# virajmehta/vae-training

Hardware: AMD Instinct MI355X
Metric: ELBO train-step samples/sec (higher is better)
Workload: dtype f32; 1 GPU; M: linear-padding dd3 pad9 (D=12) L=20 linear enc/dec -tdv eps=-1 lr=1e-3 (seed_linpadding_expts.sh:1); batch_per_gpu=65536, global_batch=65536, data_dim=12, latent_dim=20, params=533, parallelism=dp1, grad_exchange=none, launch=direct library call x2395 steps (arguments marshalled once), input_batches=48

## Files before the change

### include/vaek.h

```cpp
#ifndef VAEK_H
#define VAEK_H

#include <stddef.h>
#include <stdint.h>

#ifdef __cplusplus
extern "C" {
#endif

#define VAEK_VERSION 100
#define VAEK_MAX_HIDDEN 8

typedef enum vaek_status {
    VAEK_OK = 0,
    VAEK_ERR_INVALID = -1,
    VAEK_ERR_HIP = -2,
    VAEK_ERR_NO_DEVICE = -3,
    VAEK_ERR_WORKSPACE = -4,
    VAEK_ERR_COMM = -5
} vaek_status;

enum { VAEK_ACT_NONE = 0, VAEK_ACT_RELU = 1 };

enum { VAEK_F32 = 0, VAEK_BF16 = 1 };

typedef struct vaek_config {
    int32_t struct_size;
    int32_t batch;
    int32_t data_dim;
    int32_t latent_dim;
    int32_t n_enc_hidden;
    int32_t enc_hidden[VAEK_MAX_HIDDEN];
    int32_t n_dec_hidden;
    int32_t dec_hidden[VAEK_MAX_HIDDEN];
    int32_t sigmoid_decoder;
    int32_t tunable_eps;
    float   eps_cli;
    int32_t dtype;
    int32_t device;
    int32_t world;
    int32_t rank;
    int64_t global_batch;
    int32_t force_generic;
    int32_t reserved[7];
} vaek_config;

typedef struct vaek_ctx vaek_ctx;

int vaek_version(void);
const char* vaek_last_error(void);

int vaek_ctx_create(const vaek_config* cfg, vaek_ctx** out);
int vaek_ctx_destroy(vaek_ctx* ctx);
int vaek_param_count(const vaek_ctx* ctx, int64_t* P);
int vaek_grad_len(const vaek_ctx* ctx, int64_t* n);
int vaek_leaf_count(const vaek_ctx* ctx, int32_t* n_leaves);
int vaek_leaf_info(const vaek_ctx* ctx, int32_t leaf, char* name, int32_t name_cap,
                   int64_t* offset, int32_t* rows, int32_t* cols);
int vaek_workspace_bytes(const vaek_ctx* ctx, size_t* bytes);
int vaek_uses_fused_path(const vaek_ctx* ctx, int32_t* fused);
int vaek_train_step_path(const vaek_ctx* ctx, char* name, int32_t cap);

int vaek_dense_fwd(vaek_ctx* ctx, const float* x, const float* w, const float* b, float* y,
                   int32_t rows, int32_t n_in, int32_t n_out, int32_t act, void* stream);
int vaek_dense_bwd_dx(vaek_ctx* ctx, const float* dy, const float* w, const float* x_post, float* dx,
                      int32_t rows, int32_t n_in, int32_t n_out, int32_t act, int32_t accumulate, void* stream);
int vaek_dense_bwd_dw(vaek_ctx* ctx, const float* x, const float* dy, float* dwb,
                      int32_t rows, int32_t n_in, int32_t n_out, void* workspace, void* stream);
int vaek_elbo_fwd_bwd(vaek_ctx* ctx, const float* x, const float* x_hat_lin, const float* x_hat_sig,
                      const float* z2, const float* mu, const float* logvar_e, float eps,
                      float* d_lin, float* d_sig, float* out4, int32_t rows, int32_t data_dim,
                      int32_t latent_dim, int64_t batch_total, void* workspace, void* stream);
int vaek_elbo_fwd_bwd_dev(vaek_ctx* ctx, const float* x, const float* x_hat_lin, const float* x_hat_sig,
                          const float* z2, const float* mu, const float* logvar_e, const float* eps_param_dev, float eps_scale,
                          float* d_lin, float* d_sig, float* out4, int32_t rows, int32_t data_dim,
                          int32_t latent_dim, int64_t batch_total, void* workspace, void* stream);
int vaek_adam_step(vaek_ctx* ctx, float* params, const float* grads, float* m, float* v, int64_t n,
                   float lr, int32_t step, const int32_t* step_dev, float grad_scale, void* stream);

int vaek_train_step(vaek_ctx* ctx, float* params, float* grads, float* m, float* v, int32_t* step_dev,
                    const float* x, const float* z1, const float* z2, float lr,
                    void* workspace, void* stream);
int vaek_train_step_grads_only(vaek_ctx* ctx, const float* params, float* grads, int32_t* step_dev,
                               const float* x, const float* z1, const float* z2,
                               void* workspace, void* stream);
int vaek_train_step_apply(vaek_ctx* ctx, float* params, const float* grads, float* m, float* v,
                          const int32_t* step_dev, float lr, void* stream);
int vaek_bucket_count(const vaek_ctx* ctx, int32_t* n);
int vaek_bucket_info(const vaek_ctx* ctx, int32_t i, int64_t* offset, int64_t* count);
int vaek_train_step_grads_bucketed(vaek_ctx* ctx, const float* params, float* grads, int32_t* step_dev,
                                   const float* x, const float* z1, const float* z2, void* const* ready_events,
                                   void* workspace, void* stream);
int vaek_loss_eval(vaek_ctx* ctx, const float* params, const float* x, const float* z1, const float* z2,
                   float* out4, void* workspace, void* stream);
int vaek_forward(vaek_ctx* ctx, const float* params, const float* x, const float* z1, const float* z2,
                 int32_t sampling, float eps, float* x_hat, float* mu_out, int32_t rows,
                 void* workspace, void* stream);

int vaek_comm_buffer_bytes(const vaek_ctx* ctx, size_t* bytes);
int vaek_comm_create(vaek_ctx* ctx, uint8_t handle_out[64]);
int vaek_comm_init(vaek_ctx* ctx, const uint8_t* all_handles );
int vaek_comm_destroy(vaek_ctx* ctx);
int vaek_comm_allreduce(vaek_ctx* ctx, float* buf, int64_t n, void* stream);
int vaek_comm_status(vaek_ctx* ctx, int32_t* timed_out);

int vaek_make_batch(vaek_ctx* ctx, int32_t kind, const float* A, int32_t dd, int32_t did, int32_t pad, float var_added,
                    float* x, float* z1, float* z2, int32_t rows, int64_t row0, uint64_t seed,
                    const int32_t* step_dev, uint32_t step_host, uint32_t tag, void* stream);
int vaek_make_batch_next(vaek_ctx* ctx, int32_t kind, const float* A, int32_t dd, int32_t did, int32_t pad, float var_added,
                         float* x, float* z1, float* z2, int32_t rows, int64_t row0, uint64_t seed,
                         int32_t* counter , int32_t which, uint32_t tag, void* stream);
int vaek_train_step_gen(vaek_ctx* ctx, float* params, float* grads, float* m, float* v, int32_t* step_dev, const float* x,
                        const float* z1, const float* z2, float lr, void* workspace, int32_t kind, const float* A, int32_t dd,
                        int32_t did, int32_t pad, float var_added, float* x_next, float* z1_next, float* z2_next, int64_t row0,
                        uint64_t seed, int32_t* counter, int32_t which, uint32_t tag, void* stream);
int vaek_supports_train_steps(const vaek_ctx* ctx, int32_t* yes);
int vaek_train_steps(vaek_ctx* ctx, float* params, float* grads, float* m, float* v, int32_t* step_dev,
                     const float* const* xs, const float* const* z1s, const float* const* z2s, int32_t n_steps, float lr,
                     void* workspace, void* stream);
int vaek_train_steps_status(vaek_ctx* ctx, void* workspace, int32_t* gave_up);
int vaek_supports_train_steps_gen(const vaek_ctx* ctx, int32_t kind, int32_t* yes);
int vaek_train_steps_moment_len(const vaek_ctx* ctx, int64_t* len);
int vaek_train_steps_moments(vaek_ctx* ctx, const float* x, const float* z1, const float* z2, double* M, void* workspace, void* stream);
int vaek_train_steps_update(vaek_ctx* ctx, float* params, float* grads, float* m, float* v, int32_t* step_dev, const double* M, float lr,
                            void* workspace, void* stream);
int vaek_train_steps_gen(vaek_ctx* ctx, float* params, float* grads, float* m, float* v, int32_t* step_dev, int32_t kind, const float* A,
                         int32_t dd, int32_t did, int32_t pad, float var_added, int64_t row0, uint64_t seed, uint32_t tag, int32_t n_steps,
                         float lr, void* workspace, void* stream);
int vaek_supports_train_loop_gen(const vaek_ctx* ctx, int32_t kind, int32_t* yes);
int vaek_train_loop_gen(vaek_ctx* ctx, float* params, float* grads, float* m, float* v, int32_t* step_dev, int32_t kind, const float* A,
                        int32_t dd, int32_t did, int32_t pad, float var_added, int64_t row0, uint64_t seed, uint32_t tag, int32_t n_steps,
                        float lr, void* workspace, void* stream);
int vaek_train_loop_steps_per_launch(void);
typedef struct vaek_replicas {
    int32_t struct_size;
    int32_t n;
    int64_t state_stride;
    int64_t grads_stride;
    const uint64_t* seeds;
    const float* lrs;
    int64_t a_stride;
    float* loss_hist;
    int64_t loss_hist_cap;
} vaek_replicas;
int vaek_train_loop_max_replicas(void);
int vaek_train_loop_replicas_workspace_bytes(const vaek_ctx* ctx, int32_t n, size_t* bytes);
int vaek_train_loop_gen_replicas(vaek_ctx* ctx, float* params, float* grads, float* m, float* v, int32_t* step_dev,
                                 const vaek_replicas* rep, int32_t kind, const float* A, int32_t dd, int32_t did, int32_t pad,
                                 float var_added, int64_t row0, uint32_t tag, int32_t n_steps, float lr, void* workspace, void* stream);
typedef struct vaek_trajectory {
    int32_t struct_size;
    int32_t every;
    float*  buf;
    int64_t cap;
    int64_t record_stride;
    int64_t replica_stride;
} vaek_trajectory;
int vaek_trajectory_record_len(const vaek_ctx* ctx, int64_t* floats);
int vaek_train_loop_gen_traj(vaek_ctx* ctx, float* params, float* grads, float* m, float* v, int32_t* step_dev, int32_t kind, const float* A,
                             int32_t dd, int32_t did, int32_t pad, float var_added, int64_t row0, uint64_t seed, uint32_t tag, int32_t n_steps,
                             float lr, void* workspace, void* stream, const vaek_trajectory* traj);
int vaek_train_loop_gen_replicas_traj(vaek_ctx* ctx, float* params, float* grads, float* m, float* v, int32_t* step_dev,
                                      const vaek_replicas* rep, int32_t kind, const float* A, int32_t dd, int32_t did, int32_t pad,
                                      float var_added, int64_t row0, uint32_t tag, int32_t n_steps, float lr, void* workspace, void* stream,
                                      const vaek_trajectory* traj);
int vaek_supports_train_step_replicas(const vaek_ctx* ctx, int32_t* yes);
int vaek_train_step_max_replicas(void);
int vaek_train_step_replicas_workspace_bytes(const vaek_ctx* ctx, int32_t n, size_t* bytes);
int vaek_train_step_gen_replicas(vaek_ctx* ctx, float* params, float* grads, float* m, float* v, int32_t* step_dev,
                                 const vaek_replicas* rep, const float* x, const float* z1, const float* z2, float lr, void* workspace,
                                 int32_t kind, const float* A, int32_t dd, int32_t did, int32_t pad, float var_added, float* x_next,
                                 float* z1_next, float* z2_next, int64_t row0, int32_t* counter, int32_t which, uint32_t tag,
                                 void* stream);
int vaek_conv2d_forward_workspace(int32_t batch, int32_t height, int32_t width, int32_t c_in, int32_t c_out, int32_t transposed, size_t* bytes);
int vaek_conv2d_forward(const float* x, const float* w, const float* bias, const float* mask, float* y, int32_t batch, int32_t height,
                        int32_t width, int32_t c_in, int32_t c_out, int32_t relu, void* workspace, const void* x_bf16, void* y_bf16,
                        void* stream);
int vaek_to_bf16(const float* src, void* dst_bf16, int64_t n, void* stream);
int vaek_conv2d_transpose_forward(const float* y, const float* w, const float* bias, const float* mask, float* out, int32_t batch,
                                  int32_t height, int32_t width, int32_t c_in, int32_t c_out, int32_t relu, void* workspace,
                                  const void* y_bf16, void* out_bf16, void* stream);
int vaek_conv2d_weight_grad_workspace(int32_t batch, int32_t height, int32_t width, int32_t c_in, int32_t c_out, size_t* bytes);
int vaek_conv2d_weight_grad(const float* x, const float* dy, float* dw, float* dbias, void* workspace, int32_t batch, int32_t height,
                            int32_t width, int32_t c_in, int32_t c_out, const void* x_bf16, const void* dy_bf16, void* stream);
int vaek_conv2d_bias_grad(const float* dy, float* dbias, void* workspace, int64_t pixels, int32_t c, void* stream);
int vaek_conv2d_bias_grad_bf16(const void* dy_bf16, float* dbias, void* workspace, int64_t pixels, int32_t c, void* stream);
int vaek_dense_fwd_reparam(vaek_ctx* ctx, const float* x, const float* w, const float* b, float* mu, float* samples, const float* z1,
                           const float* logvar_e, int32_t rows, int32_t n_in, int32_t n_out, void* stream);
int vaek_reparam_bwd(vaek_ctx* ctx, float* d_samples, const float* mu, const float* z1, const float* logvar_e, float* d_logvar_e,
                     int32_t rows, int32_t latent_dim, int64_t batch_total, void* workspace, void* stream);
int vaek_rng_fill(vaek_ctx* ctx, float* normals, uint32_t* bits, int64_t n, uint64_t seed, uint32_t step, uint32_t tag,
                  void* stream);
int vaek_set_loss_history(vaek_ctx* ctx, float* buf, int64_t cap);

int vaek_microbench_copy(vaek_ctx* ctx, const void* src, void* dst, int64_t bytes, void* stream);
int vaek_microbench_mfma(vaek_ctx* ctx, int32_t kind, int32_t iters, int32_t waves_per_simd, float* scratch,
                         double* flops_out, void* stream);

int vaek_microbench_launch(vaek_ctx* ctx, int32_t kind, int32_t blocks, int32_t n, const int32_t* p, int32_t* out, void* stream);

int vaek_profile_begin(vaek_ctx* ctx, int32_t max_records);
int vaek_profile_report(vaek_ctx* ctx, char* buf, size_t cap);

#ifdef __cplusplus
}
#endif
#endif
```

### vae_training_amd/_lib.py

```python
from __future__ import annotations

import ctypes as C
import os

_HERE = os.path.dirname(os.path.abspath(__file__))
LIB_PATH = os.environ.get("VAEK_LIB_PATH") or os.path.join(_HERE, "csrc", "libvaek.so")
VAEK_MAX_HIDDEN = 8
VAEK_F32, VAEK_BF16 = 0, 1
VAEK_ACT_NONE, VAEK_ACT_RELU = 0, 1


class VaekError(RuntimeError):
    def __init__(self, code, msg):
        super().__init__(f"libvaek error {code}: {msg}")
        self.code = code


class VaekConfig(C.Structure):
    _fields_ = [
        ("struct_size", C.c_int32), ("batch", C.c_int32), ("data_dim", C.c_int32), ("latent_dim", C.c_int32),
        ("n_enc_hidden", C.c_int32), ("enc_hidden", C.c_int32 * VAEK_MAX_HIDDEN),
        ("n_dec_hidden", C.c_int32), ("dec_hidden", C.c_int32 * VAEK_MAX_HIDDEN),
        ("sigmoid_decoder", C.c_int32), ("tunable_eps", C.c_int32), ("eps_cli", C.c_float),
        ("dtype", C.c_int32), ("device", C.c_int32), ("world", C.c_int32), ("rank", C.c_int32),
        ("global_batch", C.c_int64), ("force_generic", C.c_int32), ("reserved", C.c_int32 * 7),
    ]


class VaekReplicas(C.Structure):
    _fields_ = [
        ("struct_size", C.c_int32), ("n", C.c_int32), ("state_stride", C.c_int64), ("grads_stride", C.c_int64),
        ("seeds", C.c_void_p), ("lrs", C.c_void_p), ("a_stride", C.c_int64), ("loss_hist", C.c_void_p), ("loss_hist_cap", C.c_int64),
    ]


class VaekTrajectory(C.Structure):
    _fields_ = [
        ("struct_size", C.c_int32), ("every", C.c_int32), ("buf", C.c_void_p), ("cap", C.c_int64), ("record_stride", C.c_int64),
        ("replica_stride", C.c_int64),
    ]


def trajectory_slot(t, every, cap):
    if t < 1 or t % every:
        return None
    return (t // every - 1) % cap


_vp, _i32, _i64, _f32 = C.c_void_p, C.c_int32, C.c_int64, C.c_float

SIGNATURES = {
    "vaek_version": (C.c_int, []),
    "vaek_last_error": (C.c_char_p, []),
    "vaek_ctx_create": (C.c_int, [C.POINTER(VaekConfig), C.POINTER(_vp)]),
    "vaek_ctx_destroy": (C.c_int, [_vp]),
    "vaek_param_count": (C.c_int, [_vp, C.POINTER(_i64)]),
    "vaek_grad_len": (C.c_int, [_vp, C.POINTER(_i64)]),
    "vaek_leaf_count": (C.c_int, [_vp, C.POINTER(_i32)]),
    "vaek_leaf_info": (C.c_int, [_vp, _i32, C.c_char_p, _i32, C.POINTER(_i64), C.POINTER(_i32), C.POINTER(_i32)]),
    "vaek_workspace_bytes": (C.c_int, [_vp, C.POINTER(C.c_size_t)]),
    "vaek_uses_fused_path": (C.c_int, [_vp, C.POINTER(_i32)]),
    "vaek_train_step_path": (C.c_int, [_vp, C.c_char_p, _i32]),
    "vaek_dense_fwd": (C.c_int, [_vp, _vp, _vp, _vp, _vp, _i32, _i32, _i32, _i32, _vp]),
    "vaek_dense_bwd_dx": (C.c_int, [_vp, _vp, _vp, _vp, _vp, _i32, _i32, _i32, _i32, _i32, _vp]),
    "vaek_dense_bwd_dw": (C.c_int, [_vp, _vp, _vp, _vp, _i32, _i32, _i32, _vp, _vp]),
    "vaek_elbo_fwd_bwd": (C.c_int, [_vp, _vp, _vp, _vp, _vp, _vp, _vp, _f32, _vp, _vp, _vp, _i32, _i32, _i32, _i64, _vp, _vp]),
    "vaek_elbo_fwd_bwd_dev": (C.c_int, [_vp, _vp, _vp, _vp, _vp, _vp, _vp, _vp, _f32, _vp, _vp, _vp, _i32, _i32, _i32, _i64, _vp, _vp]),
    "vaek_adam_step": (C.c_int, [_vp, _vp, _vp, _vp, _vp, _i64, _f32, _i32, _vp, _f32, _vp]),
    "vaek_train_step": (C.c_int, [_vp, _vp, _vp, _vp, _vp, _vp, _vp, _vp, _vp, _f32, _vp, _vp]),
    "vaek_train_step_grads_only": (C.c_int, [_vp, _vp, _vp, _vp, _vp, _vp, _vp, _vp, _vp]),
    "vaek_train_step_apply": (C.c_int, [_vp, _vp, _vp, _vp, _vp, _vp, _f32, _vp]),
    "vaek_bucket_count": (C.c_int, [_vp, C.POINTER(_i32)]),
    "vaek_bucket_info": (C.c_int, [_vp, _i32, C.POINTER(_i64), C.POINTER(_i64)]),
    "vaek_train_step_grads_bucketed": (C.c_int, [_vp, _vp, _vp, _vp, _vp, _vp, _vp, _vp, _vp, _vp]),
    "vaek_loss_eval": (C.c_int, [_vp, _vp, _vp, _vp, _vp, _vp, _vp, _vp]),
    "vaek_forward": (C.c_int, [_vp, _vp, _vp, _vp, _vp, _i32, _f32, _vp, _vp, _i32, _vp, _vp]),
    "vaek_comm_buffer_bytes": (C.c_int, [_vp, C.POINTER(C.c_size_t)]),
    "vaek_comm_create": (C.c_int, [_vp, _vp]),
    "vaek_comm_init": (C.c_int, [_vp, _vp]),
    "vaek_comm_status": (C.c_int, [_vp, C.POINTER(_i32)]),
    "vaek_comm_destroy": (C.c_int, [_vp]),
    "vaek_comm_allreduce": (C.c_int, [_vp, _vp, _i64, _vp]),
    "vaek_make_batch": (C.c_int, [_vp, _i32, _vp, _i32, _i32, _i32, _f32, _vp, _vp, _vp, _i32, _i64, C.c_uint64, _vp,
                                  C.c_uint32, C.c_uint32, _vp]),
    "vaek_make_batch_next": (C.c_int, [_vp, _i32, _vp, _i32, _i32, _i32, _f32, _vp, _vp, _vp, _i32, _i64, C.c_uint64, _vp,
                                       _i32, C.c_uint32, _vp]),
    "vaek_train_step_gen": (C.c_int, [_vp, _vp, _vp, _vp, _vp, _vp, _vp, _vp, _vp, _f32, _vp, _i32, _vp, _i32, _i32, _i32, _f32,
                                      _vp, _vp, _vp, _i64, C.c_uint64, _vp, _i32, C.c_uint32, _vp]),
    "vaek_supports_train_steps": (C.c_int, [_vp, C.POINTER(_i32)]),
    "vaek_train_steps": (C.c_int, [_vp, _vp, _vp, _vp, _vp, _vp, _vp, _vp, _vp, _i32, _f32, _vp, _vp]),
    "vaek_train_steps_status": (C.c_int, [_vp, _vp, C.POINTER(_i32)]),
    "vaek_supports_train_steps_gen": (C.c_int, [_vp, _i32, C.POINTER(_i32)]),
    "vaek_train_steps_moment_len": (C.c_int, [_vp, C.POINTER(_i64)]),
    "vaek_train_steps_moments": (C.c_int, [_vp, _vp, _vp, _vp, _vp, _vp, _vp]),
    "vaek_train_steps_update": (C.c_int, [_vp, _vp, _vp, _vp, _vp, _vp, _vp, _f32, _vp, _vp]),
    "vaek_train_steps_gen": (C.c_int, [_vp, _vp, _vp, _vp, _vp, _vp, _i32, _vp, _i32, _i32, _i32, _f32, C.c_int64, C.c_uint64, C.c_uint32, _i32,
                                       _f32, _vp, _vp]),
    "vaek_supports_train_loop_gen": (C.c_int, [_vp, _i32, C.POINTER(_i32)]),
    "vaek_train_loop_gen": (C.c_int, [_vp, _vp, _vp, _vp, _vp, _vp, _i32, _vp, _i32, _i32, _i32, _f32, C.c_int64, C.c_uint64, C.c_uint32, _i32,
                                      _f32, _vp, _vp]),
    "vaek_train_loop_steps_per_launch": (C.c_int, []),
    "vaek_train_loop_max_replicas": (C.c_int, []),
    "vaek_train_loop_replicas_workspace_bytes": (C.c_int, [_vp, _i32, C.POINTER(C.c_size_t)]),
    "vaek_train_loop_gen_replicas": (C.c_int, [_vp, _vp, _vp, _vp, _vp, _vp, C.POINTER(VaekReplicas), _i32, _vp, _i32, _i32, _i32, _f32,
                                               C.c_int64, C.c_uint32, _i32, _f32, _vp, _vp]),
    "vaek_trajectory_record_len": (C.c_int, [_vp, C.POINTER(_i64)]),
    "vaek_train_loop_gen_traj": (C.c_int, [_vp, _vp, _vp, _vp, _vp, _vp, _i32, _vp, _i32, _i32, _i32, _f32, C.c_int64, C.c_uint64, C.c_uint32, _i32,
                                           _f32, _vp, _vp, C.POINTER(VaekTrajectory)]),
    "vaek_train_loop_gen_replicas_traj": (C.c_int, [_vp, _vp, _vp, _vp, _vp, _vp, C.POINTER(VaekReplicas), _i32, _vp, _i32, _i32, _i32, _f32,
                                                    C.c_int64, C.c_uint32, _i32, _f32, _vp, _vp, C.POINTER(VaekTrajectory)]),
    "vaek_supports_train_step_replicas": (C.c_int, [_vp, C.POINTER(_i32)]),
    "vaek_train_step_max_replicas": (C.c_int, []),
    "vaek_train_step_replicas_workspace_bytes": (C.c_int, [_vp, _i32, C.POINTER(C.c_size_t)]),
    "vaek_train_step_gen_replicas": (C.c_int, [_vp, _vp, _vp, _vp, _vp, _vp, C.POINTER(VaekReplicas), _vp, _vp, _vp, _f32, _vp, _i32, _vp,
                                               _i32, _i32, _i32, _f32, _vp, _vp, _vp, _i64, _vp, _i32, C.c_uint32, _vp]),
    "vaek_conv2d_forward": (C.c_int, [_vp, _vp, _vp, _vp, _vp, _i32, _i32, _i32, _i32, _i32, _i32, _vp, _vp, _vp, _vp]),
    "vaek_to_bf16": (C.c_int, [_vp, _vp, C.c_int64, _vp]),
    "vaek_conv2d_forward_workspace": (C.c_int, [_i32, _i32, _i32, _i32, _i32, _i32, C.POINTER(C.c_size_t)]),
    "vaek_conv2d_bias_grad": (C.c_int, [_vp, _vp, _vp, C.c_int64, _i32, _vp]),
    "vaek_conv2d_bias_grad_bf16": (C.c_int, [_vp, _vp, _vp, C.c_int64, _i32, _vp]),
    "vaek_dense_fwd_reparam": (C.c_int, [_vp, _vp, _vp, _vp, _vp, _vp, _vp, _vp, _i32, _i32, _i32, _vp]),
    "vaek_reparam_bwd": (C.c_int, [_vp, _vp, _vp, _vp, _vp, _vp, _i32, _i32, C.c_int64, _vp, _vp]),
    "vaek_conv2d_transpose_forward": (C.c_int, [_vp, _vp, _vp, _vp, _vp, _i32, _i32, _i32, _i32, _i32, _i32, _vp, _vp, _vp, _vp]),
    "vaek_conv2d_weight_grad_workspace": (C.c_int, [_i32, _i32, _i32, _i32, _i32, C.POINTER(C.c_size_t)]),
    "vaek_conv2d_weight_grad": (C.c_int, [_vp, _vp, _vp, _vp, _vp, _i32, _i32, _i32, _i32, _i32, _vp, _vp, _vp]),
    "vaek_rng_fill": (C.c_int, [_vp, _vp, _vp, _i64, C.c_uint64, C.c_uint32, C.c_uint32, _vp]),
    "vaek_set_loss_history": (C.c_int, [_vp, _vp, _i64]),
    "vaek_microbench_copy": (C.c_int, [_vp, _vp, _vp, _i64, _vp]),
    "vaek_microbench_launch": (C.c_int, [_vp, _i32, _i32, _i32, _vp, _vp, _vp]),
    "vaek_microbench_mfma": (C.c_int, [_vp, _i32, _i32, _i32, _vp, C.POINTER(C.c_double), _vp]),
    "vaek_profile_begin": (C.c_int, [_vp, _i32]),
    "vaek_profile_report": (C.c_int, [_vp, C.c_char_p, C.c_size_t]),
}

_lib = None


def load():
    global _lib
    if _lib is not None:
        return _lib
    if not os.path.exists(LIB_PATH):
        raise RuntimeError(
            f"{LIB_PATH} is missing: build it with `make -C {os.path.dirname(LIB_PATH)}` or "
            "`python -c 'import __graft_entry__ as g; g.build()'`. vae_training_amd has no CPU/PyTorch fallback.")
    import torch
    lib = C.CDLL(LIB_PATH)
    for name, (res, args) in SIGNATURES.items():
        fn = getattr(lib, name)
        fn.restype, fn.argtypes = res, args
    _lib = lib
    return lib


def check(rc):
    if rc != 0:
        raise VaekError(rc, load().vaek_last_error().decode("utf-8", "replace"))
```

### vae_training_amd/csrc/api.hip

```cpp
#include <stdarg.h>
#include <string.h>

#include <algorithm>
#include <new>
#include <utility>

#include "vaek_internal.h"

namespace vaek {

static thread_local char g_err[512] = "";
thread_local Profiler* g_prof = nullptr;
void set_error(const char* fmt, ...) {
    va_list ap;
    va_start(ap, fmt);
    vsnprintf(g_err, sizeof(g_err), fmt, ap);
    va_end(ap);
}

static size_t align_up(size_t v, size_t a) { return (v + a - 1) / a * a; }
constexpr int kElboBlockSplits = 512;

static void add_net(vaek_ctx* c, Net& net, const char* name, int fan_in, const int* hidden, int n_hidden, int last) {
    int k = fan_in;
// ... 836 lines not shown
        return VAEK_ERR_INVALID;
    }
    if (rep->n < 1 || rep->n > resident_max_replicas()) {
        set_error("%s: %d replicas, need 1 .. %d (vaek_train_loop_max_replicas)", who, rep->n, resident_max_replicas());
        return VAEK_ERR_INVALID;
    }
    if (rep->state_stride < ctx->P || rep->grads_stride < ctx->P + kExtra) {
        set_error("%s: state_stride %lld < P = %lld or grads_stride %lld < grad_len = %lld", who, (long long)rep->state_stride,
                  (long long)ctx->P, (long long)rep->grads_stride, (long long)(ctx->P + kExtra));
        return VAEK_ERR_INVALID;
    }
    if (!rep->seeds) { set_error("%s: seeds is NULL", who); return VAEK_ERR_INVALID; }
    if (rep->a_stride < 0) { set_error("%s: a_stride %lld < 0", who, (long long)rep->a_stride); return VAEK_ERR_INVALID; }
    if (rep->loss_hist && rep->loss_hist_cap < 1) {
        set_error("%s: loss_hist given with loss_hist_cap %lld < 1", who, (long long)rep->loss_hist_cap);
        return VAEK_ERR_INVALID;
    }
    const size_t ws_bytes = resident_replicas_workspace_bytes(ctx, rep->n);
    if (ws_bytes && (!workspace || (reinterpret_cast<uintptr_t>(workspace) & 15))) {
        set_error("%s: this context stages its batches in memory: workspace must be a 16-byte aligned device "
                  "pointer of vaek_train_loop_replicas_workspace_bytes() = %zu bytes", who, ws_bytes);
        return VAEK_ERR_INVALID;
    }
    TrajArgs tj{};
    if (traj) { const int trc = check_trajectory(who, ctx, traj, true, &tj); if (trc) return trc; }
    BatchArgs gen;
    float* dummy = params;
    int rc = make_batch_args(ctx, kind, A, dd, did, pad, var_added, dummy, dummy, dummy, ctx->B, row0, 0, step_dev, 0, nullptr, 0, tag, &gen);
    if (rc) return rc;
    gen.x = gen.z1 = gen.z2 = nullptr;
    if (n_steps == 0) return VAEK_OK;
    return resident_train_loop_replicas(ctx, params, grads, m, v, step_dev, gen, rep->n, rep->state_stride, rep->grads_stride,
                                        reinterpret_cast<const unsigned long long*>(rep->seeds), rep->lrs, rep->a_stride, rep->loss_hist,
                                        rep->loss_hist_cap, n_steps, lr, workspace, (hipStream_t)stream, traj ? &tj : nullptr);
}

int vaek_train_loop_gen_replicas(vaek_ctx* ctx, float* params, float* grads, float* m, float* v, int32_t* step_dev,
                                 const vaek_replicas* rep, int32_t kind, const float* A, int32_t dd, int32_t did, int32_t pad,
                                 float var_added, int64_t row0, uint32_t tag, int32_t n_steps, float lr, void* workspace, void* stream) {
    return train_loop_gen_replicas_impl("vaek_train_loop_gen_replicas", ctx, params, grads, m, v, step_dev, rep, kind, A, dd, did, pad, var_added,
                                        row0, tag, n_steps, lr, workspace, stream, nullptr);
}

int vaek_train_loop_gen_replicas_traj(vaek_ctx* ctx, float* params, float* grads, float* m, float* v, int32_t* step_dev,
                                      const vaek_replicas* rep, int32_t kind, const float* A, int32_t dd, int32_t did, int32_t pad,
                                      float var_added, int64_t row0, uint32_t tag, int32_t n_steps, float lr, void* workspace, void* stream,
                                      const vaek_trajectory* traj) {
    return train_loop_gen_replicas_impl(traj ? "vaek_train_loop_gen_replicas_traj" : "vaek_train_loop_gen_replicas", ctx, params, grads, m, v,
                                        step_dev, rep, kind, A, dd, did, pad, var_added, row0, tag, n_steps, lr, workspace, stream, traj);
}

int vaek_train_loop_gen_traj(vaek_ctx* ctx, float* params, float* grads, float* m, float* v, int32_t* step_dev, int32_t kind, const float* A,
                             int32_t dd, int32_t did, int32_t pad, float var_added, int64_t row0, uint64_t seed, uint32_t tag, int32_t n_steps,
                             float lr, void* workspace, void* stream, const vaek_trajectory* traj) {
    if (!traj) return vaek_train_loop_gen(ctx, params, grads, m, v, step_dev, kind, A, dd, did, pad, var_added, row0, seed, tag, n_steps, lr,
                                          workspace, stream);
    ProfBind pb(ctx);
    if (!ctx || !params || !grads || !m || !v || !step_dev || n_steps < 0) { set_error("vaek_train_loop_gen_traj: invalid argument"); return VAEK_ERR_INVALID; }
    if (!ctx->resident) {
        set_error("vaek_train_loop_gen_traj: needs a context vaek_train_loop_gen covers (see vaek_supports_train_loop_gen)");
        return VAEK_ERR_INVALID;
    }
    TrajArgs tj{};
    int rc = check_trajectory("vaek_train_loop_gen_traj", ctx, traj, false, &tj);
    if (rc) return rc;
    if ((rc = check_ws(ctx, workspace))) return rc;
    BatchArgs gen;
    float* dummy = reinterpret_cast<float*>(workspace);
    if ((rc = make_batch_args(ctx, kind, A, dd, did, pad, var_added, dummy, dummy, dummy, ctx->B, row0, seed, step_dev, 0, nullptr, 0, tag, &gen))) return rc;
    gen.x = gen.z1 = gen.z2 = nullptr;
    if (n_steps == 0) return VAEK_OK;
    return resident_train_loop(ctx, params, grads, m, v, step_dev, gen, n_steps, lr, workspace, (hipStream_t)stream, &tj);
}

int vaek_supports_train_step_replicas(const vaek_ctx* ctx, int32_t* yes) {
    if (!ctx || !yes) { set_error("null argument"); return VAEK_ERR_INVALID; }
    *yes = ctx->mlp3 && ctx->cfg.world == 1 ? 1 : 0;
    return VAEK_OK;
}

int vaek_train_step_max_replicas(void) { return mlp3_max_replicas(); }

int vaek_train_step_replicas_workspace_bytes(const vaek_ctx* ctx, int32_t n, size_t* bytes) {
    if (!ctx || !bytes || n < 1 || n > mlp3_max_replicas()) {
        set_error("vaek_train_step_replicas_workspace_bytes: null argument, or n outside 1 .. %d", mlp3_max_replicas());
        return VAEK_ERR_INVALID;
    }
    *bytes = ctx->mlp3 && ctx->cfg.world == 1 ? mlp3_replicas_workspace_bytes(ctx, n) : 0;
    return VAEK_OK;
}

int vaek_train_step_gen_replicas(vaek_ctx* ctx, float* params, float* grads, float* m, float* v, int32_t* step_dev,
                                 const vaek_replicas* rep, const float* x, const float* z1, const float* z2, float lr, void* workspace,
                                 int32_t kind, const float* A, int32_t dd, int32_t did, int32_t pad, float var_added, float* x_next,
                                 float* z1_next, float* z2_next, int64_t row0, int32_t* counter, int32_t which, uint32_t tag, void* stream) {
    ProfBind pb(ctx);
    const char* const fn = "vaek_train_step_gen_replicas";
    if (!ctx || !params || !grads || !m || !v || !step_dev || !rep || !x || !z1 || !z2) {
        set_error("%s: null argument", fn);
        return VAEK_ERR_INVALID;
    }
    if (rep->struct_size != (int32_t)sizeof(vaek_replicas)) {
        set_error("%s: vaek_replicas.struct_size %d != %d (header / library mismatch)", fn, rep->struct_size, (int)sizeof(vaek_replicas));
        return VAEK_ERR_INVALID;
    }
    if (!ctx->mlp3 || ctx->cfg.world != 1) {
        set_error("%s: needs a single-GPU context whose train step path is \"mlp3\" (see vaek_supports_train_step_replicas)", fn);
        return VAEK_ERR_INVALID;
    }
    if (rep->n < 1 || rep->n > mlp3_max_replicas()) {
        set_error("%s: %d replicas, need 1 .. %d (vaek_train_step_max_replicas)", fn, rep->n, mlp3_max_replicas());
        return VAEK_ERR_INVALID;
    }
    if (rep->state_stride < ctx->P || rep->state_stride % 4 != 0) {
        set_error("%s: state_stride %lld must be >= P = %lld and a multiple of 4", fn, (long long)rep->state_stride, (long long)ctx->P);
        return VAEK_ERR_INVALID;
    }
    if (rep->grads_stride < ctx->P + kExtra) {
        set_error("%s: grads_stride %lld < grad_len = %lld", fn, (long long)rep->grads_stride, (long long)(ctx->P + kExtra));
        return VAEK_ERR_INVALID;
    }
    if (rep->loss_hist && rep->loss_hist_cap < 1) {
        set_error("%s: loss_hist given with loss_hist_cap %lld < 1", fn, (long long)rep->loss_hist_cap);
        return VAEK_ERR_INVALID;
    }
    if (rep->a_stride < 0) { set_error("%s: a_stride %lld < 0", fn, (long long)rep->a_stride); return VAEK_ERR_INVALID; }
    if (dd > 16 || did > 16) { set_error("%s: dd %d or did %d > 16", fn, dd, did); return VAEK_ERR_INVALID; }
    const int n_next = (x_next ? 1 : 0) + (z1_next ? 1 : 0) + (z2_next ? 1 : 0);
    if (n_next != 0 && n_next != 3) {
        set_error("%s: x_next, z1_next and z2_next must be all NULL (no draw) or all given", fn);
        return VAEK_ERR_INVALID;
    }
    if (!workspace || (reinterpret_cast<uintptr_t>(workspace) & 15)) {
        set_error("%s: workspace must be a 16-byte aligned device pointer of vaek_train_step_replicas_workspace_bytes() = %zu bytes", fn,
                  mlp3_replicas_workspace_bytes(ctx, rep->n));
        return VAEK_ERR_INVALID;
    }
    BatchArgs gen;
    if (n_next) {
        if (!rep->seeds || !counter) { set_error("%s: the drawing form needs seeds and counter", fn); return VAEK_ERR_INVALID; }
        if (x_next == x || z1_next == z1 || z2_next == z2) {
            set_error("%s: the next batch must not alias the current one", fn);
            return VAEK_ERR_INVALID;
        }
        int rc = make_batch_args(ctx, kind, A, dd, did, pad, var_added, x_next, z1_next, z2_next, ctx->B, row0, 0, nullptr, 0, counter, which,
                                 tag, &gen);
        if (rc) return rc;
    }
    return mlp3_train_step_replicas(ctx, params, grads, m, v, step_dev, x, z1, z2, lr, workspace, (hipStream_t)stream, n_next ? &gen : nullptr,
                                    rep->n, rep->state_stride, rep->grads_stride, reinterpret_cast<const unsigned long long*>(rep->seeds),
                                    rep->lrs, rep->a_stride, rep->loss_hist, rep->loss_hist_cap);
}

int vaek_train_steps_moment_len(const vaek_ctx* ctx, int64_t* len) {
    if (!ctx || !len) { set_error("null argument"); return VAEK_ERR_INVALID; }
    *len = ctx->lin.NO;
    return VAEK_OK;
}

int vaek_train_steps_moments(vaek_ctx* ctx, const float* x, const float* z1, const float* z2, double* M, void* workspace, void* stream) {
    ProfBind pb(ctx);
    if (!ctx || !x || !z1 || !z2 || !M) { set_error("vaek_train_steps_moments: null argument"); return VAEK_ERR_INVALID; }
    if (!ctx->lin.ok) { set_error("vaek_train_steps_moments: not a float32 linear VAE with L + 2 D + 1 <= 64"); return VAEK_ERR_INVALID; }
    if ((reinterpret_cast<uintptr_t>(x) | reinterpret_cast<uintptr_t>(z1) | reinterpret_cast<uintptr_t>(z2)) & 15) {
        set_error("vaek_train_steps_moments: batch pointers must be 16-byte aligned");
        return VAEK_ERR_INVALID;
    }
    int rc = check_ws(ctx, workspace);
    if (rc) return rc;
    return lin_moments(ctx, x, z1, z2, M, workspace, (hipStream_t)stream);
}

int vaek_train_steps_update(vaek_ctx* ctx, float* params, float* grads, float* m, float* v, int32_t* step_dev, const double* M, float lr,
                            void* workspace, void* stream) {
    ProfBind pb(ctx);
    if (!ctx || !params || !grads || !m || !v || !step_dev || !M) { set_error("vaek_train_steps_update: null argument"); return VAEK_ERR_INVALID; }
    if (!ctx->lin.ok) { set_error("vaek_train_steps_update: not a float32 linear VAE with L + 2 D + 1 <= 64"); return VAEK_ERR_INVALID; }
    int rc = check_ws(ctx, workspace);
    if (rc) return rc;
    return lin_update(ctx, params, grads, m, v, step_dev, M, lr, (hipStream_t)stream);
}

int vaek_train_steps_status(vaek_ctx* ctx, void* workspace, int32_t* gave_up) {
    if (!ctx || !workspace || !gave_up) { set_error("null argument"); return VAEK_ERR_INVALID; }
    int g = 0;
    const int rc = lin_steps_status(ctx, workspace, &g);
    *gave_up = g;
    return rc;
}

static void bucket_list(const vaek_ctx* c, std::vector<std::pair<int64_t, int64_t>>& out) {
    out.clear();
    if (c->fused) { out.push_back({0, c->P + kExtra}); return; }
    for (const Net* net : {&c->dec, &c->sig, &c->enc})
        for (int i = (int)net->layers.size() - 1; i >= 0; --i) {
            const auto& l = net->layers[i];
            out.push_back({l.w_off, (int64_t)(l.n_in + 1) * l.n_out});
        }
    out.push_back({c->off_epsp, c->P + kExtra - c->off_epsp});
}

int vaek_bucket_count(const vaek_ctx* ctx, int32_t* n) {
    if (!ctx || !n) { set_error("null argument"); return VAEK_ERR_INVALID; }
    std::vector<std::pair<int64_t, int64_t>> b;
    bucket_list(ctx, b);
    *n = (int32_t)b.size();
    return VAEK_OK;
}

int vaek_bucket_info(const vaek_ctx* ctx, int32_t i, int64_t* offset, int64_t* count) {
    if (!ctx || !offset || !count) { set_error("null argument"); return VAEK_ERR_INVALID; }
    std::vector<std::pair<int64_t, int64_t>> b;
    bucket_list(ctx, b);
    if (i < 0 || i >= (int32_t)b.size()) { set_error("bucket index out of range"); return VAEK_ERR_INVALID; }
    *offset = b[i].first; *count = b[i].second;
    return VAEK_OK;
}

int vaek_train_step_grads_bucketed(vaek_ctx* ctx, const float* params, float* grads, int32_t* step_dev, const float* x,
                                   const float* z1, const float* z2, void* const* ready_events, void* workspace, void* stream) {
    ProfBind pb(ctx);
    if (!ctx || !params || !grads || !step_dev || !x || !z1 || !z2 || !ready_events) { set_error("vaek_train_step_grads_bucketed: null argument"); return VAEK_ERR_INVALID; }
    int rc = check_ws(ctx, workspace);
    if (rc) return rc;
    hipStream_t st = (hipStream_t)stream;
    if (ctx->fused) {
        if ((rc = whole_step(ctx, const_cast<float*>(params), grads, nullptr, nullptr, step_dev, x, z1, z2, 0.f, false, false,
                             workspace, st)))
            return rc;
        VAEK_HIP_CHECK(hipEventRecord((hipEvent_t)ready_events[0], st));
        return VAEK_OK;
    }
    BucketSink sink{grads, ready_events, 0};
    if ((rc = generic_grads(ctx, params, step_dev, x, z1, z2, workspace, st, &sink))) return rc;
    if ((rc = generic_finalize(ctx, params, grads, nullptr, nullptr, nullptr, nullptr, 0.f, workspace, st, ctx->off_epsp))) return rc;
    VAEK_HIP_CHECK(hipEventRecord((hipEvent_t)ready_events[sink.next], st));
    return VAEK_OK;
}

int vaek_loss_eval(vaek_ctx* ctx, const float* params, const float* x, const float* z1, const float* z2, float* out4,
                   void* workspace, void* stream) {
    ProfBind pb(ctx);
    if (!ctx || !params || !x || !z1 || !z2 || !out4) { set_error("vaek_loss_eval: null argument"); return VAEK_ERR_INVALID; }
    int rc = check_ws(ctx, workspace);
    if (rc) return rc;
    hipStream_t st = (hipStream_t)stream;
    vaek_ctx* c = ctx;
    const bool sig = c->cfg.sigmoid_decoder != 0;
    if ((rc = convert_weights(c, params, workspace, st))) return rc;
    if ((rc = net_forward(c, c->enc, params, x, workspace, c->B, true, z1, st))) return rc;
    const float* samples = at<float>(workspace, c->ws_samples);
    if ((rc = net_forward(c, c->dec, params, samples, workspace, c->B, false, nullptr, st))) return rc;
    if (sig && (rc = net_forward(c, c->sig, params, samples, workspace, c->B, false, nullptr, st))) return rc;
    ElboArgs e{};
    e.x = x; e.y_lin = at<float>(workspace, c->dec.act_off.back());
    e.y_sig = sig ? at<float>(workspace, c->sig.act_off.back()) : nullptr;
    e.z2 = z2; e.mu = at<float>(workspace, c->enc.act_off.back());
    e.eps_param = c->off_eps >= 0 ? params + c->off_eps : nullptr; e.eps_cli = c->cfg.eps_cli;
    e.partial = at<float>(workspace, c->ws_epart);
    e.rows = c->B; e.D = c->D; e.L = c->L; e.S = c->Se; e.rows_per_split = c->rows_per_esplit;
    e.inv_bt = (float)(1.0 / (double)c->B);
    if ((rc = launch_elbo(e, st))) return rc;
    return launch_eval_out4(e.partial, c->Se, params, c->off_epsp, c->off_eps, c->L, c->D, c->cfg.eps_cli, (float)c->B,
                            e.inv_bt, out4, st);
}

int vaek_forward(vaek_ctx* ctx, const float* params, const float* x, const float* z1, const float* z2,
                 int32_t sampling, float eps, float* x_hat, float* mu_out, int32_t rows, void* workspace, void* stream) {
    ProfBind pb(ctx);
    if (!ctx || !params || !z1 || !z2 || !x_hat || (!sampling && !x) || rows <= 0) { set_error("vaek_forward: invalid argument"); return VAEK_ERR_INVALID; }
    if (rows > ctx->B) { set_error("vaek_forward: rows %d exceed this context's batch %d", rows, ctx->B); return VAEK_ERR_WORKSPACE; }
    int rc = check_ws(ctx, workspace);
    if (rc) return rc;
    hipStream_t st = (hipStream_t)stream;
    vaek_ctx* c = ctx;
    const bool sig = c->cfg.sigmoid_decoder != 0;
    const float* samples = z1;
    if ((rc = convert_weights(c, params, workspace, st))) return rc;
    if (!sampling) {
        if ((rc = net_forward(c, c->enc, params, x, workspace, rows, true, z1, st))) return rc;
        samples = at<float>(workspace, c->ws_samples);
        if (mu_out)
            VAEK_HIP_CHECK(hipMemcpyAsync(mu_out, at<float>(workspace, c->enc.act_off.back()),
                                          (size_t)rows * c->L * sizeof(float), hipMemcpyDeviceToDevice, st));
    } else if (mu_out) {
        VAEK_HIP_CHECK(hipMemsetAsync(mu_out, 0, (size_t)rows * c->L * sizeof(float), st));
    }
    if ((rc = net_forward(c, c->dec, params, samples, workspace, rows, false, nullptr, st))) return rc;
    if (sig && (rc = net_forward(c, c->sig, params, samples, workspace, rows, false, nullptr, st))) return rc;
    const float* eps_param = (!sampling && c->off_eps >= 0) ? params + c->off_eps : nullptr;
    const float eps_val = sampling ? eps : c->cfg.eps_cli;
    return launch_add_noise(at<float>(workspace, c->dec.act_off.back()),
                            sig ? at<float>(workspace, c->sig.act_off.back()) : nullptr, z2, eps_param, eps_val, x_hat,
                            (int64_t)rows * c->D, st);
}

int vaek_debug_set_stamps(vaek_ctx* ctx, unsigned long long* buf) {
    if (!ctx) return VAEK_ERR_INVALID;
    ctx->dbg_stamps = buf;
    return VAEK_OK;
}

int vaek_profile_begin(vaek_ctx* ctx, int32_t max_records) {
    if (!ctx || max_records <= 0) { set_error("vaek_profile_begin: invalid argument"); return VAEK_ERR_INVALID; }
    Profiler& p = ctx->prof;
    while ((int)p.ev.size() < 2 * max_records) {
// ... 40 lines not shown
```

### vae_training_amd/csrc/linear_moments.hip

```cpp
#include <stdlib.h>

#include <type_traits>

#include "comm_dev.h"
#include "rng_dev.h"
#include "vaek_internal.h"

namespace vaek {

using f32x4 = __attribute__((ext_vector_type(4))) float;
using d2 = __attribute__((ext_vector_type(2))) double;
typedef __attribute__((address_space(3))) void lds_void_t;
typedef const __attribute__((address_space(1))) void glb_void_t;

constexpr int LNT = 512, LNW = LNT / 64;
constexpr int kLinMaxPersist = 64;
constexpr int kLinCarry = 2, kLinSlots = kLinMaxPersist + kLinCarry;
struct LinWindow { int first, count; };
struct LinWindows { LinWindow stream, reduce, update; };
constexpr LinWindows lin_windows(int K, int j) {
    const int s0 = kLinMaxPersist * j, s1 = s0 + kLinMaxPersist < K ? s0 + kLinMaxPersist : K;
    const bool last = s1 == K;
    const int r0 = s0 >= 1 ? s0 - 1 : 0, u0 = s0 >= 2 ? s0 - 2 : 0;
    return LinWindows{{s0, s1 - s0}, {r0, (last ? K : s1 - 1) - r0}, {u0, (last ? K : s1 - 2) - u0}};
}
constexpr int lin_launches(int K) { return (K + kLinMaxPersist - 1) / kLinMaxPersist; }
constexpr bool lin_windows_ok(int K) {
    int s = 0, r = 0, u = 0;
    for (int j = 0; j < lin_launches(K); ++j) {
        const LinWindows w = lin_windows(K, j);
        if (w.stream.first != s || w.reduce.first != r || w.update.first != u) return false;
        if (w.stream.count < 1 || w.stream.count > kLinMaxPersist || w.reduce.count < 1 || w.update.count < 1) return false;
        s += w.stream.count; r += w.reduce.count; u += w.update.count;
        if (r > s || u > r || s - w.update.first > kLinSlots) return false;
    }
    return s == K && r == K && u == K;
}
static_assert(lin_windows_ok(1) && lin_windows_ok(2) && lin_windows_ok(64) && lin_windows_ok(65) && lin_windows_ok(66) && lin_windows_ok(128) &&
              lin_windows_ok(129) && lin_windows_ok(130) && lin_windows_ok(960), "launch windows of a vaek_train_steps call");
static_assert(lin_windows(64, 0).update.count == 64 && lin_windows(130, 1).update.first == 62 && lin_windows(130, 1).reduce.first == 63 &&
              lin_windows(130, 2).update.count == 4, "launch windows of a vaek_train_steps call");
constexpr int kLinReduceSets = 1;
constexpr int kLinReduceWgs = 24;

constexpr int kLinCommBanks = 4;
struct LinComm { unsigned long long* peer[kMaxWorld]; int world, rank, ng2; };

constexpr int kLinShards = 8, kLinShardStride = 32;
struct LinPtrs { const float* x[64]; const float* z1[64]; const float* z2[64]; };
struct LinArgs {
    int has_update, n_reduce, n_stream;
    int B, D, L, ntiles, T;
    const float* x; const float* z1; const float* z2; float* partial_out;
    const float* partial_in; double* M_out;
    const double* M_in;
    int persistent, n_steps, sets;
    int n_red, n_str, slot_upd, slot_red, slot_str;
    int d_red, d_str;
    float* partial_base; double* M_base;
    unsigned* cnt_stream; unsigned* cnt_reduce; unsigned* status;
    float* params; float* grads; float* m; float* v; int32_t* step_dev; float lr;
    float inv_bt, eps_cli, rows, rows_over_bt; int off_eps, P;
    float* loss_hist; long long loss_hist_cap;
    int stagger;
    LinComm comm;
};

#ifndef VAEK_LIN_ABL
#define VAEK_LIN_ABL 0
#endif
#ifdef VAEK_LIN_STAMPS
#ifdef VAEK_LIN_FOUR_BLOCK_TU
static __device__ unsigned long long* g_lin_stamp_buf = nullptr;
#else
__device__ unsigned long long* g_lin_stamp_buf = nullptr;
#endif
int lin_stamps_four(unsigned long long* buf);
#define LIN_STAMP(i)                                                                                         \
    do {                                                                                                     \
        if (VAEK_LIN_STAMPS == 2) break;          \
        __builtin_amdgcn_sched_barrier(0);                                                                   \
        unsigned long long _t;                                                                               \
        unsigned long long _r;                                                                               \
        asm volatile("s_waitcnt vmcnt(0) lgkmcnt(0)\n\ts_memtime %0\n\ts_memrealtime %1\n\ts_waitcnt lgkmcnt(0)" : "=s"(_t), "=s"(_r)::"memory"); \
        if (g_lin_stamp_buf && threadIdx.x == 0) { g_lin_stamp_buf[i] = _t; g_lin_stamp_buf[16 + (i)] = _r; } \
        __builtin_amdgcn_sched_barrier(0);                                                                   \
    } while (0)
#define LIN_NOW(v)                                                                                           \
    do {                                                                                                     \
        __builtin_amdgcn_sched_barrier(0);                                                                   \
        if (VAEK_LIN_STAMPS == 2) asm volatile("s_memrealtime %0\n\ts_waitcnt lgkmcnt(0)" : "=s"(v)::"memory");             \
        else asm volatile("s_waitcnt vmcnt(0) lgkmcnt(0)\n\ts_memrealtime %0\n\ts_waitcnt lgkmcnt(0)" : "=s"(v)::"memory"); \
        __builtin_amdgcn_sched_barrier(0);                                                                   \
    } while (0)
#define LIN_NOWQ(v)                                     \
    do {                                                                                                     \
        __builtin_amdgcn_sched_barrier(0);                                                                   \
        asm volatile("s_memrealtime %0\n\ts_waitcnt lgkmcnt(0)" : "=s"(v)::"memory");                        \
        __builtin_amdgcn_sched_barrier(0);                                                                   \
    } while (0)
#define LIN_PUT(i, v) do { if (g_lin_stamp_buf && threadIdx.x == 0) g_lin_stamp_buf[i] = (v); } while (0)
#define LIN_PUTMAX(i, v) do { if (g_lin_stamp_buf && threadIdx.x == 0) atomicMax(&g_lin_stamp_buf[i], (v)); } while (0)
#else
#define LIN_STAMP(i) do {} while (0)
#define LIN_NOW(v) do {} while (0)
#define LIN_NOWQ(v) do {} while (0)
#define LIN_PUT(i, v) do {} while (0)
#define LIN_PUTMAX(i, v) do {} while (0)
#endif

__device__ __forceinline__ void lin_glds16(const void* gsrc, void* lds_wave_base) {
    __builtin_amdgcn_global_load_lds((glb_void_t*)gsrc, (lds_void_t*)lds_wave_base, 16, 0, 0);
}
template <int N> __device__ __forceinline__ void lin_wait_vmcnt() { asm volatile("s_waitcnt vmcnt(%0)" ::"n"(N) : "memory"); }
__device__ __forceinline__ void lin_barrier() { asm volatile("s_waitcnt lgkmcnt(0)\n\ts_barrier" ::: "memory"); }
__device__ __forceinline__ void lin_wait_vmcnt_upto(int n) {
    switch (n) {
        case 1: lin_wait_vmcnt<1>(); break;   case 2: lin_wait_vmcnt<2>(); break;   case 3: lin_wait_vmcnt<3>(); break;
        case 4: lin_wait_vmcnt<4>(); break;   case 5: lin_wait_vmcnt<5>(); break;   case 6: lin_wait_vmcnt<6>(); break;
        case 7: lin_wait_vmcnt<7>(); break;   case 8: lin_wait_vmcnt<8>(); break;   case 9: lin_wait_vmcnt<9>(); break;
        case 10: lin_wait_vmcnt<10>(); break; case 11: lin_wait_vmcnt<11>(); break; case 12: lin_wait_vmcnt<12>(); break;
        case 13: lin_wait_vmcnt<13>(); break; case 14: lin_wait_vmcnt<14>(); break; case 15: lin_wait_vmcnt<15>(); break;
        case 16: lin_wait_vmcnt<16>(); break; case 17: lin_wait_vmcnt<17>(); break; case 18: lin_wait_vmcnt<18>(); break;
        case 19: lin_wait_vmcnt<19>(); break; case 20: lin_wait_vmcnt<20>(); break;
        default: lin_wait_vmcnt<0>(); break;
    }
}

__device__ __host__ constexpr int lin_blk(int NB, int b1, int b2) { return b1 * NB - b1 * (b1 - 1) / 2 + (b2 - b1); }

__device__ __forceinline__ void st_sc1(float* p, float v) { __hip_atomic_store(p, v, __ATOMIC_RELAXED, __HIP_MEMORY_SCOPE_AGENT); }
__device__ __forceinline__ void st_sc1(double* p, double v) { __hip_atomic_store(p, v, __ATOMIC_RELAXED, __HIP_MEMORY_SCOPE_AGENT); }
__device__ __forceinline__ float ld_sc1(const float* p) { return __hip_atomic_load(p, __ATOMIC_RELAXED, __HIP_MEMORY_SCOPE_AGENT); }
__device__ __forceinline__ double ld_sc1(const double* p) { return __hip_atomic_load(p, __ATOMIC_RELAXED, __HIP_MEMORY_SCOPE_AGENT); }

__device__ __forceinline__ void lin_wait_count(const unsigned* cnt, unsigned target, unsigned* status, unsigned tag) {
    if (threadIdx.x == 0) {
        unsigned spins = 0, seen;
        while ((seen = __hip_atomic_load(cnt, __ATOMIC_RELAXED, __HIP_MEMORY_SCOPE_AGENT)) < target) {
            __builtin_amdgcn_s_sleep(16);
            if ((++spins & 1023u) == 0) {
                if (__hip_atomic_load(status, __ATOMIC_RELAXED, __HIP_MEMORY_SCOPE_AGENT)) break;
                if (spins > (1u << 21)) {
                    unsigned expect = 0;
                    __hip_atomic_compare_exchange_strong(status, &expect, 0x80000000u | tag | (seen & 0xffffu), __ATOMIC_RELAXED,
                                                         __ATOMIC_RELAXED, __HIP_MEMORY_SCOPE_AGENT);
                    break;
                }
            }
        }
    }
    __syncthreads();
}

__device__ __forceinline__ void lin_wait_shards(const unsigned* cnt, unsigned target, unsigned* status, unsigned tag) {
    if (threadIdx.x == 0) {
        unsigned spins = 0, seen;
        for (;;) {
            unsigned v[kLinShards];
#pragma unroll
            for (int k = 0; k < kLinShards; ++k) v[k] = __hip_atomic_load(cnt + k * kLinShardStride, __ATOMIC_RELAXED, __HIP_MEMORY_SCOPE_AGENT);
            seen = 0;
#pragma unroll
            for (int k = 0; k < kLinShards; ++k) seen += v[k];
            if (seen >= target) break;
            __builtin_amdgcn_s_sleep(4);
            if ((++spins & 1023u) == 0) {
                if (__hip_atomic_load(status, __ATOMIC_RELAXED, __HIP_MEMORY_SCOPE_AGENT)) break;
                if (spins > (1u << 21)) {
                    unsigned expect = 0;
                    __hip_atomic_compare_exchange_strong(status, &expect, 0x80000000u | tag | (seen & 0xffffu), __ATOMIC_RELAXED,
                                                         __ATOMIC_RELAXED, __HIP_MEMORY_SCOPE_AGENT);
                    break;
                }
            }
        }
    }
    __syncthreads();
}

__device__ __forceinline__ double lin_sum_over_ranks(const LinComm& c, unsigned epoch, int o, double v, unsigned* status) {
    const unsigned long long bits = (unsigned long long)__double_as_longlong(v), tag = (unsigned long long)epoch << 32;
    const long long bank = (long long)(epoch & (kLinCommBanks - 1)) * c.world * c.ng2;
    for (int p = 0; p < c.world; ++p) {
        unsigned long long* q = c.peer[p] + bank + (long long)c.rank * c.ng2 + 2 * o;
        __hip_atomic_store(q, tag | (bits & 0xffffffffull), __ATOMIC_RELAXED, __HIP_MEMORY_SCOPE_SYSTEM);
        __hip_atomic_store(q + 1, tag | (bits >> 32), __ATOMIC_RELAXED, __HIP_MEMORY_SCOPE_SYSTEM);
    }
    const unsigned long long* own = c.peer[c.rank] + bank + 2 * o;
    double sum = 0.0;
    unsigned spins = 0;
    bool dead = false;
    for (int r = 0; r < c.world; ++r) {
        unsigned long long lo = 0, hi = 0;
        for (;;) {
            lo = __hip_atomic_load(own + (long long)r * c.ng2, __ATOMIC_RELAXED, __HIP_MEMORY_SCOPE_SYSTEM);
            hi = __hip_atomic_load(own + (long long)r * c.ng2 + 1, __ATOMIC_RELAXED, __HIP_MEMORY_SCOPE_SYSTEM);
            if (((unsigned)(lo >> 32) == epoch && (unsigned)(hi >> 32) == epoch) || dead) break;
            __builtin_amdgcn_s_sleep(8);
            if ((++spins & 1023u) == 0) {
                if (__hip_atomic_load(status, __ATOMIC_RELAXED, __HIP_MEMORY_SCOPE_AGENT)) dead = true;
                else if (spins > (1u << 21)) {
                    unsigned expect = 0;
                    __hip_atomic_compare_exchange_strong(status, &expect, 0x80000000u | (3u << 28) | ((unsigned)r << 16) | (epoch & 0xffffu),
                                                         __ATOMIC_RELAXED, __ATOMIC_RELAXED, __HIP_MEMORY_SCOPE_AGENT);
                    dead = true;
                }
            }
        }
        sum += __longlong_as_double((long long)((hi << 32) | (lo & 0xffffffffull)));
    }
    return sum;
}

struct LinTile {
    int nz1, nx, np, oX, oZ2, bytes;
    __device__ __host__ LinTile(int D, int L, int T) {
        nz1 = (L * 4 * T + 1023) >> 10; nx = (D * 4 * T + 1023) >> 10; np = nz1 + 2 * nx;
        oX = (nz1 << 10) + 80;
        oZ2 = oX + (nx << 10); bytes = (oZ2 + (nx << 10) + 255) & ~255;
    }
};

__device__ __forceinline__ void lin_issue_piece(const LinArgs& a, const LinTile& tl, const float* x, const float* z1, const float* z2,
                                                int tile, int p, char* slot, int lane) {
    const float* src; int cols, idx, lds_off;
    if (p < tl.nz1) { src = z1; cols = a.L; idx = p; lds_off = 0; }
    else if (p < tl.nz1 + tl.nx) { src = x; cols = a.D; idx = p - tl.nz1; lds_off = tl.oX; }
    else { src = z2; cols = a.D; idx = p - tl.nz1 - tl.nx; lds_off = tl.oZ2; }
    const long long tot = (long long)a.B * cols * 4, base = (long long)tile * a.T * cols * 4;
    const long long last = min(tot & ~15ll, base + (long long)a.T * cols * 4) - 16;
    long long off = base + idx * 1024 + lane * 16;
    off = off <= last ? off : last;
    lin_glds16(reinterpret_cast<const char*>(src) + off, slot + lds_off + idx * 1024);
}

struct LinTileSrc {
    const char *z1, *x, *z2; long long baseL, lastL, baseD, lastD; char* slot; bool on;
    __device__ __forceinline__ void prepare(const LinArgs& a, const float* px, const float* pz1, const float* pz2, int tile, char* slot_) {
        auto uni = [](const float* q) {
            const unsigned long long u = (unsigned long long)q;
            return reinterpret_cast<const char*>((unsigned long long)(unsigned)__builtin_amdgcn_readfirstlane((unsigned)u) |
                                                 ((unsigned long long)(unsigned)__builtin_amdgcn_readfirstlane((unsigned)(u >> 32)) << 32));
        };
        z1 = uni(pz1); x = uni(px); z2 = uni(pz2); slot = slot_; on = true;
        const long long rows = (long long)tile * a.T;
        const long long totL = (long long)a.B * a.L * 4, totD = (long long)a.B * a.D * 4;
        baseL = rows * a.L * 4; baseD = rows * a.D * 4;
        lastL = min(totL & ~15ll, baseL + (long long)a.T * a.L * 4) - 16;
        lastD = min(totD & ~15ll, baseD + (long long)a.T * a.D * 4) - 16;
    }
    __device__ __forceinline__ void issue(const LinTile& tl, int p, int lane) const {
        const char* src; long long base, last; int idx, lds_off;
        if (p < tl.nz1) { src = z1; base = baseL; last = lastL; idx = p; lds_off = 0; }
        else if (p < tl.nz1 + tl.nx) { src = x; base = baseD; last = lastD; idx = p - tl.nz1; lds_off = tl.oX; }
        else { src = z2; base = baseD; last = lastD; idx = p - tl.nz1 - tl.nx; lds_off = tl.oZ2; }
        long long off = base + idx * 1024 + lane * 16;
        off = off <= last ? off : last;
        lin_glds16(src + off, slot + lds_off + idx * 1024);
    }
#pragma clang diagnostic push
#pragma clang diagnostic ignored "-Winline-asm"
    __device__ __forceinline__ void issue_tile(const LinTile& tl, int lw, int NLW, int lane) const {
        auto region = [&](const char* src, long long base, long long last, int n, int lds_off) __attribute__((always_inline)) {
            const long long b2 = base <= last ? base : last;
            const char* sbase = src + b2;
            const unsigned lastrel = (unsigned)(last - b2), degenerate = base <= last ? 0xffffffffu : 0u;
            const unsigned m0_0 = (unsigned)(size_t)(lds_void_t*)(slot + lds_off);
            for (int idx = lw; idx < n; idx += NLW) {
                unsigned off = ((unsigned)idx * 1024u + (unsigned)lane * 16u) & degenerate;
                off = off <= lastrel ? off : lastrel;
                asm volatile("s_mov_b32 m0, %2\n\ts_nop 0\n\tglobal_load_lds_dwordx4 %0, %1" ::"v"(off), "s"(sbase), "s"(m0_0 + (unsigned)idx * 1024u) : "memory", "m0");
            }
        };
        region(z1, baseL, lastL, tl.nz1, 0);
        region(x, baseD, lastD, tl.nx, tl.oX);
        region(z2, baseD, lastD, tl.np - tl.nz1 - tl.nx, tl.oZ2);
    }
#pragma clang diagnostic pop
};

__device__ __forceinline__ void lin_fix_ragged(const LinArgs& a, const LinTile& tl, const float* x, const float* z1, const float* z2,
                                               int tile, char* slot, int t) {
    const int T = a.T;
    const long long row0 = (long long)tile * T;
    const int valid = (int)min((long long)T, (long long)a.B - row0), D = a.D, L = a.L;
    if (valid < T) {
        auto patch_tail = [&](const float* src, int cols, int lds_off) {
            const long long tot = (long long)a.B * cols * 4, full = tot & ~15ll, base = row0 * cols * 4;
            if (t < (int)((tot - full) / 4) && full >= base) reinterpret_cast<float*>(slot + lds_off)[(full - base) / 4 + t] = src[full / 4 + t];
        };
        patch_tail(z1, L, 0); patch_tail(x, D, tl.oX); patch_tail(z2, D, tl.oZ2);
        for (int e = valid * L + t; e < T * L; e += LNT) reinterpret_cast<float*>(slot)[e] = 0.f;
        for (int e = valid * D + t; e < T * D; e += LNT) { reinterpret_cast<float*>(slot + tl.oX)[e] = 0.f; reinterpret_cast<float*>(slot + tl.oZ2)[e] = 0.f; }
    }
    lin_barrier();
}
__device__ __forceinline__ void lin_write_vcol(float* v, int T, int valid, int t) {
    for (int r = t; r < T; r += LNT) v[r] = r < valid ? 1.f : 0.f;
}

__device__ __forceinline__ void st_sc1_x4(float* p, f32x4 v) {
    asm volatile("global_store_dwordx4 %0, %1, off sc1\n\ts_nop 1" ::"v"(p), "v"(v) : "memory");
}

constexpr int lin_scratch_bytes(int NB) { return LNW * (NB * (NB + 1) / 2) * 1024; }
constexpr int lin_ring_scratch_bytes(int NB) { return NB == 3 ? lin_scratch_bytes(NB) : lin_scratch_bytes(NB) / 2; }
constexpr int kLinCW = 4;
template <int NB, int JT, int CW, typename Hook>
__device__ __forceinline__ void lin_tile_products(const LinArgs& a, const LinTile& tl, const char* smem, int slot_off, int v_off, int c_off,
                                                  f32x4 (&acc)[NB * (NB + 1) / 2], int lane, int wave, Hook&& hook) {
    constexpr int NBLK = NB * (NB + 1) / 2;
    const int g = lane >> 4, D = a.D, L = a.L;
    int fb[NB], fs[NB];
#pragma unroll
    for (int u = 0; u < NB; ++u) {
        const int f = 16 * u + (lane & 15);
        if (f < L) { fb[u] = slot_off + f * 4; fs[u] = L * 4; }
        else if (f < L + D) { fb[u] = slot_off + tl.oX + (f - L) * 4; fs[u] = D * 4; }
        else if (f < L + 2 * D) { fb[u] = slot_off + tl.oZ2 + (f - L - D) * 4; fs[u] = D * 4; }
        else if (f == L + 2 * D) { fb[u] = v_off; fs[u] = 4; }
        else { fb[u] = c_off; fs[u] = 0; }
    }
#pragma unroll
    for (int k = 0; k < NBLK; ++k) acc[k] = f32x4{0.f, 0.f, 0.f, 0.f};
    const int J = JT ? JT : a.T / (4 * CW), wbase = (a.T / CW) * wave, jfull = J & ~3;
    auto products = [&](const float (&op)[NB]) __attribute__((always_inline)) {
        int k = 0;
#pragma unroll
        for (int b1 = 0; b1 < NB; ++b1)
#pragma unroll
            for (int b2 = b1; b2 < NB; ++b2, ++k) {
                if (VAEK_LIN_ABL & 2) acc[k][0] += op[b1] * op[b2];
                else acc[k] = __builtin_amdgcn_mfma_f32_16x16x4f32(op[b1], op[b2], acc[k], 0, 0, 0);
            }
    };
    if constexpr (JT > 0) {
        constexpr int JF = JT & ~3;
        int cur[NB], fs13[NB], tail[NB];
#pragma unroll
        for (int u = 0; u < NB; ++u) {
            cur[u] = fb[u] + (wbase + 4 * g) * fs[u]; fs13[u] = 13 * fs[u];
            tail[u] = fb[u] + (wbase + 4 * JF + (JT - JF) * g) * fs[u];
        }
        float op[JT][NB];
        auto fetch = [&](int j) __attribute__((always_inline)) {
#pragma unroll
            for (int u = 0; u < NB; ++u) {
                if (j == JF) cur[u] = tail[u];
                op[j][u] = *reinterpret_cast<const float*>(smem + cur[u]);
                cur[u] += (j < JF && (j & 3) == 3) ? fs13[u] : fs[u];
            }
        };
        fetch(0);
        if (JT > 1) fetch(1);
#pragma unroll
        for (int j = 0; j < JT; ++j) {
            if (j + 2 < JT) fetch(j + 2);
            hook(j);
            __builtin_amdgcn_sched_barrier(0);
            products(op[j]);
            __builtin_amdgcn_sched_barrier(0);
        }
    } else {
        float op[2][NB];
        auto fetch = [&](int set, int j) __attribute__((always_inline)) {
            const int sample = wbase + (j < jfull ? 16 * (j >> 2) + (j & 3) + 4 * g : 4 * jfull + (j - jfull) + (J - jfull) * g);
#pragma unroll
            for (int u = 0; u < NB; ++u) op[set][u] = *reinterpret_cast<const float*>(smem + fb[u] + sample * fs[u]);
        };
        fetch(0, 0);
        for (int j = 0; j < J; j += 2) {
            if (j + 1 < J) fetch(1, j + 1);
            hook(j);
            __builtin_amdgcn_sched_barrier(0);
            products(op[0]);
            __builtin_amdgcn_sched_barrier(0);
            if (j + 1 < J) {
                if (j + 2 < J) fetch(0, j + 2);
                hook(j + 1);
                __builtin_amdgcn_sched_barrier(0);
                products(op[1]);
                __builtin_amdgcn_sched_barrier(0);
            }
        }
    }
}

template <int NB, bool SC1, int CW>
__device__ __forceinline__ void lin_tile_combine(const f32x4 (&acc)[NB * (NB + 1) / 2], char* scratch, float* out, int t, int wave, int lane) {
    constexpr int NBLK = NB * (NB + 1) / 2;
    f32x4* scr = reinterpret_cast<f32x4*>(scratch);
    if (wave < CW) {
#pragma unroll
        for (int k = 0; k < NBLK; ++k) scr[(wave * NBLK + k) * 64 + lane] = acc[k];
    }
    lin_barrier();
    for (int q = t; q < NBLK * 64; q += LNT) {
        f32x4 sum = scr[q];
#pragma unroll
        for (int w = 1; w < CW; ++w) sum += scr[w * NBLK * 64 + q];
        if ((VAEK_LIN_ABL & 4) && sum[0] != 12345.f) continue;
        if (SC1) st_sc1_x4(out + 4 * q, sum); else *reinterpret_cast<f32x4*>(out + 4 * q) = sum;
    }
}
__device__ __forceinline__ void lin_img_coords(int e, int& blk, int& i, int& j) {
    blk = e >> 8; const int ln = (e >> 2) & 63; i = ((ln >> 4) << 2) + (e & 3); j = ln & 15;
}

template <bool SC1>
__device__ __forceinline__ void lin_reduce(const float* partial_in, double* M_out, int ntiles, char* smem, int rb, int no,
                                           const LinComm* cm = nullptr, unsigned epoch = 0, unsigned* status = nullptr) {
    double* sums = reinterpret_cast<double*>(smem);
    const int t = threadIdx.x, o = rb * 32 + (t & 31), rg = t >> 5;
    const int rpg = (ntiles + 15) / 16, r_lo = rg * rpg, r_hi = min(ntiles, r_lo + rpg);
    double s = 0.0;
    if (o < no)
        for (int r0 = r_lo; r0 < r_hi; r0 += 16) {
            float tv[16];
#pragma unroll
            for (int u = 0; u < 16; ++u) {
                const float* q = partial_in + (long long)min(r0 + u, r_hi - 1) * no + o;
                tv[u] = SC1 ? ld_sc1(q) : *q;
            }
#pragma unroll
            for (int u = 0; u < 16; ++u) s += r0 + u < r_hi ? (double)tv[u] : 0.0;
        }
    sums[rg * 32 + (t & 31)] = s;
    __syncthreads();
    if (t < 32 && o < no) {
        double tot = 0.0;
#pragma unroll
        for (int k = 0; k < 16; ++k) tot += sums[k * 32 + t];
        if (cm && cm->world > 1) tot = lin_sum_over_ranks(*cm, epoch, o, tot, status);
        if (SC1) st_sc1(M_out + o, tot); else M_out[o] = tot;
    }
}

__device__ __forceinline__ void lin_reduce_pair(const float* partial_in, double* M_out, int ntiles, char* smem, int rb0, int rb1, int no,
                                                const LinComm& cm, unsigned epoch, unsigned* status) {
    double* sums = reinterpret_cast<double*>(smem);
    const int t = threadIdx.x, q = t & 31, rg = t >> 5, o0 = rb0 * 32 + q, o1 = rb1 * 32 + q;
    const int rpg = (ntiles + 15) / 16, r_lo = rg * rpg, r_hi = min(ntiles, r_lo + rpg);
    double s0 = 0.0, s1 = 0.0;
    for (int r0 = r_lo; r0 < r_hi; r0 += 16) {
        float ta[16], tb[16];
#pragma unroll
        for (int u = 0; u < 16; ++u) {
            const float* row = partial_in + (long long)min(r0 + u, r_hi - 1) * no;
            ta[u] = ld_sc1(row + o0); tb[u] = ld_sc1(row + o1);
        }
#pragma unroll
        for (int u = 0; u < 16; ++u) { s0 += r0 + u < r_hi ? (double)ta[u] : 0.0; s1 += r0 + u < r_hi ? (double)tb[u] : 0.0; }
    }
    sums[rg * 32 + q] = s0; sums[512 + rg * 32 + q] = s1;
    __syncthreads();
    if (t < 64) {
        const int which = t >> 5;
        double tot = 0.0;
#pragma unroll
        for (int k = 0; k < 16; ++k) tot += sums[which * 512 + k * 32 + q];
        if (cm.world > 1) tot = lin_sum_over_ranks(cm, epoch, which ? o1 : o0, tot, status);
        st_sc1(M_out + (which ? o1 : o0), tot);
    }
}

constexpr int LKOUT = 4;
template <int NB, int DT, int LT>
struct LinUpd {
    static constexpr int NFP = 16 * NB, NBLK = NB * (NB + 1) / 2;
    int D, L, P, fone, off_be, off_wd, off_bd, off_epsp, off_eps;
    double *Mf, *SM, *P1, *G, *Wed, *Wdd, *bed, *bdd, *sd, *elv, *lvd, *dwd, *red, *epsv;
    float p[LKOUT], m[LKOUT], v[LKOUT];

    __device__ __forceinline__ void carve(const LinArgs& a, char* smem) {
        D = DT ? DT : a.D; L = LT ? LT : a.L; P = a.P; fone = L + 2 * D; off_eps = a.off_eps;
        off_be = D * L; off_wd = off_be + L; off_bd = off_wd + L * D; off_epsp = off_bd + D;
        Mf = reinterpret_cast<double*>(smem);
// ... 146 lines not shown
        LIN_STAMP(3);
        for (int e = t; e < L * NFP; e += LNT) {
            const int l = e / NFP, f = e % NFP;
            double s = 0.0;
#pragma unroll
            for (int d = 0; d < (DT ? DT : 32); ++d) if (DT || d < D) s += Wdd[l * D + d] * P1[d * NFP + f];
            G[e] = s;
        }
        for (int e = t; e < L * D; e += LNT) {
            const int l = e / D, d = e % D;
            double s = sd[l] * P1[d * NFP + l] + bed[l] * P1[d * NFP + fone];
#pragma unroll
            for (int dd = 0; dd < (DT ? DT : 32); ++dd) if (DT || dd < D) s += Wed[dd * L + l] * P1[d * NFP + L + dd];
            dwd[e] = s;
        }
        }
        __syncthreads();
        LIN_STAMP(4);
        double ssq = 0.0, musq = 0.0, z2r = 0.0, klc = 0.0;
        if constexpr (DT > 0 && LT > 0 && (DT % 2 == 0) && (LT % 2 == 0) && LT * (NFP / 2) <= LNT && LT * DT <= LNT / 2) {
            static_assert(DT * LT + LT + LT * DT + DT + LT + 1 + 3 <= LNT + 64, "wave 0 must own the scalar outputs");
            if (t < 64) {
                constexpr int NS = (LT * DT + 63) / 64, NM = (LT * (DT + 1) + 63) / 64;
                double wa[NS], da[NS], qw[NM], qs[NM], qd[NM], qm[NM];
#pragma unroll
                for (int j = 0; j < NS; ++j) { const int e = min(t + 64 * j, LT * DT - 1); wa[j] = Wdd[e]; da[j] = dwd[e]; }
#pragma unroll
                for (int j = 0; j < NM; ++j) {
                    const int e = min(t + 64 * j, LT * (DT + 1) - 1), l = e / (DT + 1), dd = e % (DT + 1), f = dd < DT ? LT + dd : fone;
                    qw[j] = dd < DT ? Wed[dd * LT + l] : bed[l]; qs[j] = SM[l * NFP + f]; qd[j] = sd[l]; qm[j] = Mf[l * NFP + f];
                }
                const int dq = min(t, DT - 1), lq = min(t, LT - 1);
                const double px = P1[dq * NFP + LT + dq], pz = P1[dq * NFP + LT + DT + dq], po = P1[dq * NFP + fone], bq = bdd[dq];
                const double lvq = lvd[lq], evq = elv[lq];
                __builtin_amdgcn_sched_barrier(0);
#pragma unroll
                for (int j = 0; j < NS; ++j) ssq += t + 64 * j < LT * DT ? wa[j] * da[j] : 0.0;
#pragma unroll
                for (int j = 0; j < NM; ++j) musq += t + 64 * j < LT * (DT + 1) ? qw[j] * (qs[j] - qd[j] * qm[j]) : 0.0;
                if (t < DT) { ssq += -px + sigma * pz + bq * po; z2r = pz; }
                if (t < LT) klc = 1.0 + lvq - evq;
#pragma unroll
                for (int o = 32; o > 0; o >>= 1) {
                    ssq += __shfl_xor(ssq, o, 64); musq += __shfl_xor(musq, o, 64);
                    z2r += __shfl_xor(z2r, o, 64); klc += __shfl_xor(klc, o, 64);
                }
            }
        } else {
        double p_ssq = 0.0, p_musq = 0.0, p_z2r = 0.0, p_klc = 0.0;
        for (int e = t; e < L * D; e += LNT) p_ssq += Wdd[e] * dwd[e];
        if (t < D) {
            p_ssq += -P1[t * NFP + L + t] + sigma * P1[t * NFP + L + D + t] + bdd[t] * P1[t * NFP + fone];
            p_z2r = P1[t * NFP + L + D + t];
        }
        for (int e = t; e < L * (D + 1); e += LNT) {
            const int l = e / (D + 1), dd = e % (D + 1);
            const int f = dd < D ? L + dd : fone;
            const double q = SM[l * NFP + f] - sd[l] * Mf[l * NFP + f];
            p_musq += (dd < D ? Wed[dd * L + l] : bed[l]) * q;
        }
        if (t < L) p_klc = 1.0 + lvd[t] - elv[t];
#pragma unroll
        for (int o = 32; o > 0; o >>= 1) {
            p_ssq += __shfl_xor(p_ssq, o, 64); p_musq += __shfl_xor(p_musq, o, 64);
            p_z2r += __shfl_xor(p_z2r, o, 64); p_klc += __shfl_xor(p_klc, o, 64);
        }
        if ((t & 63) == 0) { red[t >> 6] = p_ssq; red[LNW + (t >> 6)] = p_musq; red[2 * LNW + (t >> 6)] = p_z2r; red[3 * LNW + (t >> 6)] = p_klc; }
        __syncthreads();
#pragma unroll
        for (int w = 0; w < LNW; ++w) { ssq += red[w]; musq += red[LNW + w]; z2r += red[2 * LNW + w]; klc += red[3 * LNW + w]; }
        }
        LIN_STAMP(5);
        const double inv_bt = (double)a.inv_bt, rows = (double)a.rows, c0 = inv_var * inv_bt;
        const float bc1 = -expm1f((float)tstep * -0.10536051565782628f), bc2 = -expm1f((float)tstep * -0.0010005003335835335f);
#pragma unroll
        for (int k = 0; k < LKOUT; ++k) {
            const int idx = t + LNT * k;
            double gd = 0.0;
            if (idx < off_be) { const int d = idx / L, l = idx % L; gd = c0 * G[l * NFP + L + d] + (SM[l * NFP + L + d] - sd[l] * Mf[l * NFP + L + d]) * inv_bt; }
            else if (idx < off_wd) { const int l = idx - off_be; gd = c0 * G[l * NFP + fone] + (SM[l * NFP + fone] - sd[l] * Mf[l * NFP + fone]) * inv_bt; }
            else if (idx < off_bd) gd = c0 * dwd[idx - off_wd];
            else if (idx < off_epsp) gd = c0 * P1[(idx - off_bd) * NFP + fone];
            else if (idx < off_epsp + L) {
                const int l = idx - off_epsp;
                gd = 0.5 * sd[l] * c0 * G[l * NFP + l] - 0.5 * (1.0 - elv[l]) * (double)a.rows_over_bt;
            } else if (idx == off_eps) {
                gd = (double)a.eps_cli * (-0.5 * ssq * inv_var + 0.5 * rows * D + 0.5 * sigma * z2r * inv_var) * inv_bt;
            } else if (idx >= P && idx < P + 3) {
                const double dkl = (0.5 * musq - 0.5 * rows * klc) * inv_bt;
                const double mse = (0.5 * ssq * inv_var + 0.5 * rows * D * ((double)kLog2Pi + eps)) * inv_bt;
                gd = idx == P ? dkl + mse : (idx == P + 1 ? dkl : mse);
            }
            const float gf = (float)gd;
            gout[k] = gf;
            if (idx == P && a.loss_hist) a.loss_hist[(long long)(tstep - 1) % a.loss_hist_cap] = gf;
            if (idx < P) adam_apply_f(p[k], gf, m[k], v[k], a.lr, bc1, bc2);
        }
        LIN_STAMP(6);
    }
    __device__ __forceinline__ void store_state(const LinArgs& a, const float (&gout)[LKOUT], int tstep) {
        const int t = threadIdx.x;
#pragma unroll
        for (int k = 0; k < LKOUT; ++k) {
            const int idx = t + LNT * k;
            if (idx < P + kExtra) a.grads[idx] = gout[k];
            if (idx < P) { a.params[idx] = p[k]; a.m[idx] = m[k]; a.v[idx] = v[k]; }
        }
        if (t == 0) a.step_dev[0] = tstep;
    }
};

using d4 = __attribute__((ext_vector_type(4))) double;
template <int CTRL>
__device__ __forceinline__ double lin_dpp_add(double x) {
    const int lo = __builtin_amdgcn_update_dpp(0, __double2loint(x), CTRL, 0xf, 0xf, false);
    const int hi = __builtin_amdgcn_update_dpp(0, __double2hiint(x), CTRL, 0xf, 0xf, false);
    return x + __hiloint2double(hi, lo);
}
__device__ __forceinline__ double lin_wave_sum(double x) {
    x = lin_dpp_add<0xB1>(x);
    x = lin_dpp_add<0x4E>(x);
    x = lin_dpp_add<0x141>(x);
    x = lin_dpp_add<0x140>(x);
    double tot = 0.0;
#pragma unroll
    for (int r = 0; r < 4; ++r)
        tot += __hiloint2double(__builtin_amdgcn_readlane(__double2hiint(x), 16 * r), __builtin_amdgcn_readlane(__double2loint(x), 16 * r));
    return tot;
}
template <bool InLoop = false>
__device__ __forceinline__ double lin_exp(double x) {
    auto c = [](double v) __attribute__((always_inline)) { if constexpr (InLoop) asm volatile("" : "+s"(v)); return v; };
    const double k = rint(x * c(1.4426950408889634));
    double r = fma(-k, c(6.93147180369123816490e-01), x);
    r = fma(-k, c(1.90821492927058770002e-10), r);
    double p = c(1.0 / 6227020800.0);
    p = fma(p, r, c(1.0 / 479001600.0)); p = fma(p, r, c(1.0 / 39916800.0)); p = fma(p, r, c(1.0 / 3628800.0)); p = fma(p, r, c(1.0 / 362880.0));
    p = fma(p, r, c(1.0 / 40320.0)); p = fma(p, r, c(1.0 / 5040.0)); p = fma(p, r, c(1.0 / 720.0)); p = fma(p, r, c(1.0 / 120.0));
    p = fma(p, r, c(1.0 / 24.0)); p = fma(p, r, c(1.0 / 6.0)); p = fma(p, r, 0.5); p = fma(p, r, 1.0); p = fma(p, r, 1.0);
    return ldexp(p, (int)k);
}
__device__ __forceinline__ int lin_m_index(int NB, int r, int c) {
    const int br = r >> 4, bc = c >> 4;
    const int b1 = br <= bc ? br : bc, b2 = br <= bc ? bc : br, i = br <= bc ? (r & 15) : (c & 15), j = br <= bc ? (c & 15) : (r & 15);
    return lin_blk(NB, b1, b2) * 256 + (((i >> 2) * 16 + j) << 2) + (i & 3);
}
template <int NB, int DT, int LT>
struct LinUpdM {
    static constexpr int NFP = 16 * NB;
    static constexpr int KD = DT ? (DT + 3) / 4 : 4;
    static constexpr int RL1 = LT ? (LT > 16 ? (LT - 16 + 3) / 4 : 0) : 4;
    static constexpr int NM = 4 + RL1 + 2 * KD + 1;
    int D, L, P, fone, off_be, off_wd, off_bd, off_epsp, off_eps;
    double *Wed, *Wdd, *bed, *bdd, *sd, *elv, *lvd, *scal, *part, *P1s, *gq;
    float p[LKOUT], m[LKOUT], v[LKOUT];
    int mo[NM];

    static __host__ __device__ constexpr bool shape_ok(int D, int L) { return D <= 16 && L <= 32 && L + 2 * D + 1 <= NFP && NB == 3; }
    static __host__ size_t lds_bytes(int D, int L, int P) {
        return sizeof(double) * ((size_t)2 * D * L + 4 * L + D + 8 + 16 + 16 * NFP + (size_t)(P + kExtra + 7));
    }
    __device__ __forceinline__ void carve(const LinArgs& a, char* smem) {
        D = DT ? DT : a.D; L = LT ? LT : a.L; P = a.P; fone = L + 2 * D; off_eps = a.off_eps;
        off_be = D * L; off_wd = off_be + L; off_bd = off_wd + L * D; off_epsp = off_bd + D;
        Wed = reinterpret_cast<double*>(smem); Wdd = Wed + D * L; bed = Wdd + L * D; bdd = bed + L; sd = bdd + D; elv = sd + L; lvd = elv + L;
        scal = lvd + L; part = scal + 8; P1s = part + 16; gq = P1s + 16 * NFP;
    }
    __device__ __forceinline__ void load_state(const LinArgs& a) {
        const int t = threadIdx.x;
#pragma unroll
        for (int k = 0; k < LKOUT; ++k) {
            const int idx = min(t + LNT * k, P - 1);
            p[k] = a.params[idx]; m[k] = a.m[idx]; v[k] = a.v[idx];
        }
        if (off_eps < 0 && t == 0) { const double e = (double)a.eps_cli; scal[0] = e; scal[1] = lin_exp(0.5 * e); scal[2] = lin_exp(-e); }
        const int lane = t & 63, j = lane & 15, g = lane >> 4, f = min(16 * (t >> 6) + j, NFP - 1);
        int k = 0;
#pragma unroll
        for (int r = 0; r < 4; ++r) mo[k++] = lin_m_index(NB, g + 4 * r, f);
#pragma unroll
        for (int r = 0; r < RL1; ++r) mo[k++] = lin_m_index(NB, min(16 + g + 4 * r, NFP - 1), f);
#pragma unroll
        for (int r = 0; r < KD; ++r) mo[k++] = lin_m_index(NB, min(L + g + 4 * r, NFP - 1), f);
#pragma unroll
        for (int r = 0; r < KD; ++r) mo[k++] = lin_m_index(NB, min(L + D + g + 4 * r, NFP - 1), f);
        mo[k++] = lin_m_index(NB, fone, f);
    }
    __device__ __forceinline__ void fetch_M(const double* M_in, double (&r)[NM]) const {
#pragma unroll
        for (int k = 0; k < NM; ++k) r[k] = ld_sc1(M_in + mo[k]);
    }
    __device__ __forceinline__ void publish_params(const LinArgs& a) {
        const int t = threadIdx.x;
#pragma unroll
        for (int k = 0; k < LKOUT; ++k) {
            const int i = t + LNT * k;
            const double pv = (double)p[k];
            if (i < off_be) Wed[i] = pv;
            else if (i < off_wd) bed[i - off_be] = pv;
            else if (i < off_bd) Wdd[i - off_wd] = pv;
            else if (i < off_epsp) bdd[i - off_bd] = pv;
            else if (i < off_epsp + L || i == off_eps) {
                const bool is_eps = i == off_eps;
                const double e = is_eps ? pv * (double)a.eps_cli : pv, h = lin_exp(0.5 * e);
                if (is_eps) {
                    const double q = h * h;
                    double r = __builtin_amdgcn_rcp(q);
                    r = fma(fma(-q, r, 1.0), r, r); r = fma(fma(-q, r, 1.0), r, r);
                    scal[0] = e; scal[1] = h; scal[2] = r;
                }
                else { sd[i - off_epsp] = h; elv[i - off_epsp] = h * h; lvd[i - off_epsp] = pv; }
            }
        }
    }
    __device__ __forceinline__ void step(const LinArgs& a, int tstep, const double (&mreg)[NM], float (&gout)[LKOUT], const unsigned* next_cnt,
                                         unsigned per_set, const double* M_next, double (&mnext)[NM], bool& have_next) {
        const int t = threadIdx.x, wave = __builtin_amdgcn_readfirstlane(t >> 6), lane = t & 63, j = lane & 15, g = lane >> 4;
        LIN_STAMP(1);
        if (t == 64 * (NB + 2)) scal[4] = (next_cnt && __hip_atomic_load(next_cnt, __ATOMIC_RELAXED, __HIP_MEMORY_SCOPE_AGENT) >= per_set) ? 1.0 : 0.0;
        const double eps = scal[0], sigma = scal[1], inv_var = scal[2], inv_bt = (double)a.inv_bt, c0 = inv_var * inv_bt;
        d4 sm[2], p1;
        double musq_p = 0.0, ssq_p = 0.0, z2r_p = 0.0;
        const int f = 16 * wave + j;
        double awSMr[KD][2], awP1r[4 + (RL1 ? RL1 : 1)];
        auto awSM = [&](int kk, int lt) -> double& { return awSMr[kk][lt]; };
        auto awP1 = [&](int r) -> double& { return awP1r[r]; };
        if (wave < NB) {
#pragma unroll
            for (int kk = 0; kk < KD; ++kk)
#pragma unroll
                for (int lt = 0; lt < 2; ++lt) {
                    const int dd = 4 * kk + g, l = 16 * lt + j;
                    const double w1 = Wed[min(dd, D - 1) * L + min(l, L - 1)];
                    awSM(kk, lt) = (dd < D && l < L && (lt == 0 || RL1 > 0)) ? w1 : 0.0;
                }
#pragma unroll
            for (int r = 0; r < 4 + RL1; ++r) {
                const int l = (r < 4 ? 4 * r : 16 + 4 * (r - 4)) + g;
                const double w = Wdd[min(l, L - 1) * D + min(j, D - 1)];
                awP1(r) = (j < D && l < L) ? w : 0.0;
            }
        }
        __builtin_amdgcn_sched_barrier(0);
        if (wave < NB) {
            const double* Mz = mreg; const double* Mx = mreg + 4 + RL1; const double* Mz2 = Mx + KD; const double Mone = mreg[NM - 1];
#pragma unroll
            for (int lt = 0; lt < 2; ++lt)
#pragma unroll
                for (int r = 0; r < 4; ++r) {
                    const int l = 16 * lt + g + 4 * r;
                    const bool ok = l < L && (lt == 0 || r < RL1);
                    const double sv = sd[min(l, L - 1)], bv = bed[min(l, L - 1)];
                    const double slv = ok ? sv : 0.0, blv = ok ? bv : 0.0;
                    sm[lt][r] = (lt == 0 || r < RL1) ? slv * Mz[lt == 0 ? r : min(4 + r, 3 + RL1)] + blv * Mone : 0.0;
                }
#pragma unroll
            for (int kk = 0; kk < KD; ++kk) {
#pragma unroll
                for (int lt = 0; lt < 2; ++lt) {
                    if (lt == 1 && RL1 == 0) continue;
                    sm[lt] = __builtin_amdgcn_mfma_f64_16x16x4f64(awSM(kk, lt), Mx[kk], sm[lt], 0, 0, 0);
                }
            }
#pragma unroll
            for (int r = 0; r < 4; ++r) {
                const int d = g + 4 * r;
                p1[r] = (r < KD && d < D) ? -Mx[min(r, KD - 1)] + sigma * Mz2[min(r, KD - 1)] + bdd[min(d, D - 1)] * Mone : 0.0;
            }
#pragma unroll
            for (int r = 0; r < 4; ++r) p1 = __builtin_amdgcn_mfma_f64_16x16x4f64(awP1(r), sm[0][r], p1, 0, 0, 0);
#pragma unroll
            for (int r = 0; r < RL1; ++r) p1 = __builtin_amdgcn_mfma_f64_16x16x4f64(awP1(4 + r), sm[1][r], p1, 0, 0, 0);
#pragma unroll
            for (int r = 0; r < 4; ++r) P1s[(g + 4 * r) * NFP + f] = p1[r];
        } else if (wave == NB + 1) {
            const double kl = lane < L ? 1.0 + lvd[min(lane, L - 1)] - elv[min(lane, L - 1)] : 0.0;
            const double tot = lin_wave_sum(kl);
            if (lane == 0) {
                part[12] = tot;
                part[13] = (double)(-expm1f((float)tstep * -0.10536051565782628f)); part[14] = (double)(-expm1f((float)tstep * -0.0010005003335835335f));
            }
        }
        LIN_STAMP(2);
        __syncthreads();
        LIN_STAMP(3);
        have_next = scal[4] != 0.0;
        if (wave < NB) {
            if (have_next) fetch_M(M_next, mnext);
            double awGr[KD][2];
#pragma unroll
            for (int kk = 0; kk < KD; ++kk)
#pragma unroll
                for (int lt = 0; lt < 2; ++lt) {
                    const int dd = 4 * kk + g, l = 16 * lt + j;
                    const double w2 = Wdd[min(l, L - 1) * D + min(dd, D - 1)];
                    awGr[kk][lt] = (l < L && dd < D && (lt == 0 || RL1 > 0)) ? w2 : 0.0;
                }
            double sl[2][4], bl[2][4];
#pragma unroll
            for (int lt = 0; lt < 2; ++lt)
#pragma unroll
                for (int r = 0; r < 4; ++r) {
                    const int l = 16 * lt + g + 4 * r;
                    const bool ok = l < L && (lt == 0 || r < RL1);
                    const double sv = sd[min(l, L - 1)], bv = bed[min(l, L - 1)];
                    sl[lt][r] = ok ? sv : 0.0; bl[lt][r] = ok ? bv : 0.0;
                }
            __builtin_amdgcn_sched_barrier(0);
            d4 G[2];
            G[0] = d4{0.0, 0.0, 0.0, 0.0}; G[1] = d4{0.0, 0.0, 0.0, 0.0};
#pragma unroll
            for (int r = 0; r < KD; ++r) {
#pragma unroll
                for (int lt = 0; lt < 2; ++lt) {
                    if (lt == 1 && RL1 == 0) continue;
                    G[lt] = __builtin_amdgcn_mfma_f64_16x16x4f64(awGr[r][lt], p1[r], G[lt], 0, 0, 0);
                }
            }
            const double* Mz = mreg;
            const bool is_x = f >= L && f < L + D, is_z2 = f >= L + D && f < fone, is_one = f == fone, is_z1 = f < L;
            if (is_x || is_one) {
                const int base = is_x ? (f - L) * L : off_be;
#pragma unroll
                for (int lt = 0; lt < 2; ++lt)
#pragma unroll
                    for (int r = 0; r < 4; ++r) {
                        if (lt == 1 && r >= RL1) continue;
                        const int l = 16 * lt + g + 4 * r;
                        if (l < L) {
                            const double q = sm[lt][r] - sl[lt][r] * Mz[lt == 0 ? r : min(4 + r, 3 + RL1)];
                            gq[base + l] = c0 * G[lt][r] + q * inv_bt;
                            musq_p += (is_x ? Wed[base + l] : bl[lt][r]) * q;
                        }
                    }
            }
            if (is_one) {
#pragma unroll
                for (int r = 0; r < 4; ++r) {
                    const int d = g + 4 * r;
                    if (d < D) { gq[off_bd + d] = c0 * p1[r]; ssq_p += bdd[d] * p1[r]; }
                }
            }
            if (is_z1 && (j & 3) == g) {
                const int lt = f >> 4, r = j >> 2;
                double gll = 0.0;
#pragma unroll
                for (int q2 = 0; q2 < 2; ++q2)
#pragma unroll
                    for (int r2 = 0; r2 < 4; ++r2) gll = (q2 == lt && r2 == r) ? G[q2][r2] : gll;
                gq[off_epsp + f] = 0.5 * sd[f] * c0 * gll - 0.5 * (1.0 - elv[f]) * (double)a.rows_over_bt;
            }
            if (is_x || is_z2) {
                const int d = is_x ? f - L : f - L - D;
                if ((d & 3) == g) {
                    double pd = 0.0;
#pragma unroll
                    for (int r2 = 0; r2 < 4; ++r2) pd = (r2 == (d >> 2)) ? p1[r2] : pd;
                    if (is_x) ssq_p -= pd; else { ssq_p += sigma * pd; z2r_p += pd; }
                }
            }
            musq_p = lin_wave_sum(musq_p); ssq_p = lin_wave_sum(ssq_p); z2r_p = lin_wave_sum(z2r_p);
            if (lane == 0) { part[3 * wave] = ssq_p; part[3 * wave + 1] = musq_p; part[3 * wave + 2] = z2r_p; }
        } else if (wave == NB) {
            d4 C[2];
            double wsum = 0.0, avk[KD], p1l[2][4], p1o[4], dw_sr[2], dw_br[2], dw_wr[KD][2], dw_dr[2][4];
            auto dw_s = [&](int ct) -> double& { return dw_sr[ct]; };
            auto dw_b = [&](int ct) -> double& { return dw_br[ct]; };
            auto dw_w = [&](int kk, int ct) -> double& { return dw_wr[kk][ct]; };
            auto dw_d = [&](int ct, int r) -> double& { return dw_dr[ct][r]; };
#pragma unroll
            for (int ct = 0; ct < 2; ++ct) {
                const int l = 16 * ct + j, lc = min(l, L - 1);
                const double s_l = sd[lc], b_l = bed[lc];
                dw_s(ct) = l < L ? s_l : 0.0; dw_b(ct) = l < L ? b_l : 0.0;
#pragma unroll
                for (int kk = 0; kk < KD; ++kk) {
                    const int dd = 4 * kk + g;
                    const double w = Wed[min(dd, D - 1) * L + lc];
                    dw_w(kk, ct) = (dd < D && l < L) ? w : 0.0;
                }
#pragma unroll
                for (int r = 0; r < 4; ++r) dw_d(ct, r) = Wdd[lc * D + min(g + 4 * r, D - 1)];
            }
#pragma unroll
            for (int kk = 0; kk < KD; ++kk) avk[kk] = P1s[j * NFP + min(L + 4 * kk + g, NFP - 1)];
#pragma unroll
            for (int r = 0; r < 4; ++r) {
                p1o[r] = P1s[(g + 4 * r) * NFP + fone];
#pragma unroll
                for (int ct = 0; ct < 2; ++ct) p1l[ct][r] = P1s[(g + 4 * r) * NFP + min(16 * ct + j, L - 1)];
            }
            __builtin_amdgcn_sched_barrier(0);
#pragma unroll
            for (int ct = 0; ct < 2; ++ct) {
                if (ct == 1 && RL1 == 0) continue;
                const int l = 16 * ct + j;
#pragma unroll
                for (int r = 0; r < 4; ++r) C[ct][r] = dw_s(ct) * p1l[ct][r] + dw_b(ct) * p1o[r];
#pragma unroll
                for (int kk = 0; kk < KD; ++kk) C[ct] = __builtin_amdgcn_mfma_f64_16x16x4f64(avk[kk], dw_w(kk, ct), C[ct], 0, 0, 0);
#pragma unroll
                for (int r = 0; r < 4; ++r) {
                    const int d = g + 4 * r;
                    if (l < L && d < D) { gq[off_wd + l * D + d] = c0 * C[ct][r]; wsum += dw_d(ct, r) * C[ct][r]; }
                }
            }
            wsum = lin_wave_sum(wsum);
            if (lane == 0) part[9] = wsum;
        }
        LIN_STAMP(4);
        __syncthreads();
        LIN_STAMP(5);
        const double rows = (double)a.rows;
        const float bc1 = (float)part[13], bc2 = (float)part[14];
#pragma unroll
        for (int k = 0; k < LKOUT; ++k) {
            const int idx = t + LNT * k;
            if (LNT * k >= P + 3) break;
            double gd = 0.0;
            if (idx < P && idx != off_eps) gd = gq[idx];
            else if (idx == off_eps || (idx >= P && idx < P + 3)) {
                const double ssq = part[0] + part[3] + part[6] + part[9], musq = part[1] + part[4] + part[7], z2r = part[2] + part[5] + part[8], klc = part[12];
                if (idx == off_eps) gd = (double)a.eps_cli * (-0.5 * ssq * inv_var + 0.5 * rows * D + 0.5 * sigma * z2r * inv_var) * inv_bt;
                else {
                    const double dkl = (0.5 * musq - 0.5 * rows * klc) * inv_bt;
                    const double mse = (0.5 * ssq * inv_var + 0.5 * rows * D * ((double)kLog2Pi + eps)) * inv_bt;
                    gd = idx == P ? dkl + mse : (idx == P + 1 ? dkl : mse);
                }
            }
            const float gf = (float)gd;
            gout[k] = gf;
            if (idx == P && a.loss_hist) a.loss_hist[(long long)(tstep - 1) % a.loss_hist_cap] = gf;
            if (idx < P) adam_apply_f(p[k], gf, m[k], v[k], a.lr, bc1, bc2);
        }
        LIN_STAMP(6);
    }
    __device__ __forceinline__ void store_state(const LinArgs& a, const float (&gout)[LKOUT], int tstep) {
        const int t = threadIdx.x;
#pragma unroll
        for (int k = 0; k < LKOUT; ++k) {
            const int idx = t + LNT * k;
            if (idx < P + kExtra) a.grads[idx] = gout[k];
            if (idx < P) { a.params[idx] = p[k]; a.m[idx] = m[k]; a.v[idx] = v[k]; }
        }
        if (t == 0) a.step_dev[0] = tstep;
    }
};

template <int NB, int DT, int LT>
struct LinUpdMG {
    static constexpr int NFP = 16 * NB;
    static constexpr int KD = DT ? (DT + 3) / 4 : (NB == 3 ? 4 : 8);
    static constexpr int RL1 = LT ? (LT > 16 ? (LT - 16 + 3) / 4 : 0) : 4;
    static constexpr int NM = 4 + RL1 + 2 * KD + 1;
    static constexpr int PT = KD > 4 ? 2 : 1;
    static constexpr int NPART = NB == 3 ? 16 : 20;
    static constexpr bool PREFETCH = NB == 3;
    int D, L, P, fone, off_be, off_wd, off_bd, off_epsp, off_eps;
    double *Wed, *Wdd, *bed, *bdd, *sd, *elv, *lvd, *scal, *part, *P1s, *gq;
    float* pmv;
    __device__ __forceinline__ float& pk(int k) const { return pmv[k * LNT + threadIdx.x]; }
    __device__ __forceinline__ float& mk(int k) const { return pmv[(LKOUT + k) * LNT + threadIdx.x]; }
    __device__ __forceinline__ float& vk(int k) const { return pmv[(2 * LKOUT + k) * LNT + threadIdx.x]; }
    int* mos;

    static __host__ __device__ constexpr bool shape_ok(int D, int L) {
        return NB == 3 ? D <= 16 && L <= 32 && L + 2 * D + 1 <= NFP : NB == 4 && L <= 32 && L + 2 * D + 1 <= NFP && D <= 4 * KD;
    }
    static __host__ size_t lds_bytes(int D, int L, int P) {
        return sizeof(double) * ((size_t)2 * D * L + 4 * L + D + 8 + NPART + 16 * PT * NFP + (size_t)(P + kExtra + 7)) + sizeof(int) * NM * 64 * NB + sizeof(float) * 3 * LKOUT * LNT;
    }
    __device__ __forceinline__ void carve(const LinArgs& a, char* smem) {
        D = DT ? DT : a.D; L = LT ? LT : a.L; P = a.P; fone = L + 2 * D; off_eps = a.off_eps;
        off_be = D * L; off_wd = off_be + L; off_bd = off_wd + L * D; off_epsp = off_bd + D;
        Wed = reinterpret_cast<double*>(smem); Wdd = Wed + D * L; bed = Wdd + L * D; bdd = bed + L; sd = bdd + D; elv = sd + L; lvd = elv + L;
        scal = lvd + L; part = scal + 8; P1s = part + NPART; gq = P1s + 16 * PT * NFP; mos = reinterpret_cast<int*>(gq + P + kExtra + 7);
        pmv = reinterpret_cast<float*>(smem + sizeof(double) * (size_t)(gq + P + kExtra + 7 - Wed) + sizeof(int) * NM * 64 * NB);
    }
    __device__ __forceinline__ void load_state(const LinArgs& a) {
        const int t = threadIdx.x;
#pragma unroll
        for (int k = 0; k < LKOUT; ++k) {
            const int idx = min(t + LNT * k, P - 1);
            pk(k) = a.params[idx]; mk(k) = a.m[idx]; vk(k) = a.v[idx];
        }
        if (off_eps < 0 && t == 0) { const double e = (double)a.eps_cli; scal[0] = e; scal[1] = lin_exp<true>(0.5 * e); scal[2] = lin_exp<true>(-e); }
        if (t < 64 * NB) {
            const int lane = t & 63, j = lane & 15, g = lane >> 4, f = 16 * (t >> 6) + j;
            int k = 0;
            auto put = [&](int row) { mos[(k++) * 64 * NB + t] = lin_m_index(NB, row, f); };
#pragma unroll
            for (int r = 0; r < 4; ++r) put(g + 4 * r);
#pragma unroll
            for (int r = 0; r < RL1; ++r) put(min(16 + g + 4 * r, NFP - 1));
#pragma unroll
            for (int r = 0; r < KD; ++r) put(min(L + g + 4 * r, NFP - 1));
#pragma unroll
            for (int r = 0; r < KD; ++r) put(min(L + D + g + 4 * r, NFP - 1));
            put(fone);
        }
    }
    __device__ __forceinline__ void fetch_M(const double* M_in, double (&r)[NM]) const {
        const int* mt = mos + threadIdx.x;
        int o[NM];
#pragma unroll
        for (int k = 0; k < NM; ++k) o[k] = mt[k * 64 * NB];
#pragma unroll
        for (int k = 0; k < NM; ++k) r[k] = ld_sc1(M_in + o[k]);
    }
    __device__ __forceinline__ void publish_params(const LinArgs& a) {
        int t = threadIdx.x;
        if constexpr (NB == 4) asm volatile("" : "+v"(t));
#pragma unroll
        for (int k = 0; k < LKOUT; ++k) {
            const int i = t + LNT * k;
            const double pv = (double)pk(k);
            if (i < off_be) Wed[i] = pv;
            else if (i < off_wd) bed[i - off_be] = pv;
            else if (i < off_bd) Wdd[i - off_wd] = pv;
            else if (i < off_epsp) bdd[i - off_bd] = pv;
            else if (i < off_epsp + L || i == off_eps) {
                const bool is_eps = i == off_eps;
                const double e = is_eps ? pv * (double)a.eps_cli : pv, h = lin_exp<true>(0.5 * e);
                if (is_eps) {
                    const double q = h * h;
                    double r = __builtin_amdgcn_rcp(q);
                    r = fma(fma(-q, r, 1.0), r, r); r = fma(fma(-q, r, 1.0), r, r);
                    scal[0] = e; scal[1] = h; scal[2] = r;
                }
                else { sd[i - off_epsp] = h; elv[i - off_epsp] = h * h; lvd[i - off_epsp] = pv; }
            }
        }
    }
    __device__ __forceinline__ void step(const LinArgs& a, int tstep, const double (&mreg)[NM], float (&gout)[LKOUT], const unsigned* next_cnt,
                                         unsigned per_set, const double* M_next, double (&mnext)[NM], bool& have_next) {
        int t = threadIdx.x;
        if constexpr (NB == 4) asm volatile("" : "+v"(t));
        const int wave = __builtin_amdgcn_readfirstlane(t >> 6), lane = t & 63, j = lane & 15, g = lane >> 4;
        LIN_STAMP(1);
        if (PREFETCH && t == 64 * (NB + 2)) scal[4] = (next_cnt && __hip_atomic_load(next_cnt, __ATOMIC_RELAXED, __HIP_MEMORY_SCOPE_AGENT) >= per_set) ? 1.0 : 0.0;
        const double eps = scal[0], sigma = scal[1], inv_var = scal[2], inv_bt = (double)a.inv_bt, c0 = inv_var * inv_bt;
        d4 sm[2], p1;
        [[maybe_unused]] d4 p1b;
        auto p1row = [&](int r) -> double { return r < 4 ? p1[r & 3] : p1b[r & 3]; };
        double musq_p = 0.0, ssq_p = 0.0, z2r_p = 0.0;
        const int f = 16 * wave + j;
        double awSMr[KD][2], awP1r[PT][4 + (RL1 ? RL1 : 1)];
        auto awSM = [&](int kk, int lt) -> double& { return awSMr[kk][lt]; };
        auto awP1 = [&](int r) -> double& { return awP1r[0][r]; };
        if (wave < NB) {
#pragma unroll
            for (int kk = 0; kk < KD; ++kk)
#pragma unroll
                for (int lt = 0; lt < 2; ++lt) {
                    const int dd = 4 * kk + g, l = 16 * lt + j;
                    const double w1 = Wed[min(dd, D - 1) * L + min(l, L - 1)];
                    awSM(kk, lt) = (dd < D && l < L && (lt == 0 || RL1 > 0)) ? w1 : 0.0;
                }
#pragma unroll
            for (int r = 0; r < 4 + RL1; ++r) {
                const int l = (r < 4 ? 4 * r : 16 + 4 * (r - 4)) + g;
                const double w = Wdd[min(l, L - 1) * D + min(j, D - 1)];
                awP1(r) = (j < D && l < L) ? w : 0.0;
            }
        }
        __builtin_amdgcn_sched_barrier(0);
        if (wave < NB) {
            const double* Mz = mreg; const double* Mx = mreg + 4 + RL1; const double* Mz2 = Mx + KD; const double Mone = mreg[NM - 1];
#pragma unroll
            for (int lt = 0; lt < 2; ++lt)
#pragma unroll
                for (int r = 0; r < 4; ++r) {
                    const int l = 16 * lt + g + 4 * r;
                    const bool ok = l < L && (lt == 0 || r < RL1);
                    const double sv = sd[min(l, L - 1)], bv = bed[min(l, L - 1)];
                    const double slv = ok ? sv : 0.0, blv = ok ? bv : 0.0;
                    sm[lt][r] = (lt == 0 || r < RL1) ? slv * Mz[lt == 0 ? r : min(4 + r, 3 + RL1)] + blv * Mone : 0.0;
                }
#pragma unroll
            for (int kk = 0; kk < KD; ++kk) {
#pragma unroll
                for (int lt = 0; lt < 2; ++lt) {
                    if (lt == 1 && RL1 == 0) continue;
                    sm[lt] = __builtin_amdgcn_mfma_f64_16x16x4f64(awSM(kk, lt), Mx[kk], sm[lt], 0, 0, 0);
                }
            }
#pragma unroll
            for (int r = 0; r < 4; ++r) {
                const int d = g + 4 * r;
                p1[r] = (r < KD && d < D) ? -Mx[min(r, KD - 1)] + sigma * Mz2[min(r, KD - 1)] + bdd[min(d, D - 1)] * Mone : 0.0;
            }
#pragma unroll
            for (int r = 0; r < 4; ++r) p1 = __builtin_amdgcn_mfma_f64_16x16x4f64(awP1(r), sm[0][r], p1, 0, 0, 0);
#pragma unroll
            for (int r = 0; r < RL1; ++r) p1 = __builtin_amdgcn_mfma_f64_16x16x4f64(awP1(4 + r), sm[1][r], p1, 0, 0, 0);
#pragma unroll
            for (int r = 0; r < 4; ++r) P1s[(g + 4 * r) * NFP + f] = p1[r];
// ... 111 lines not shown
        } else if (wave == NB) {
            double wsum = 0.0;
#pragma unroll
            for (int dt = 0; dt < PT; ++dt) {
                d4 C[2];
                double avk[KD], p1l[2][4], p1o[4], dw_sr[2], dw_br[2], dw_wr[KD][2], dw_dr[2][4];
                auto dw_s = [&](int ct) -> double& { return dw_sr[ct]; };
                auto dw_b = [&](int ct) -> double& { return dw_br[ct]; };
                auto dw_w = [&](int kk, int ct) -> double& { return dw_wr[kk][ct]; };
                auto dw_d = [&](int ct, int r) -> double& { return dw_dr[ct][r]; };
                const int d0 = 16 * dt;
#pragma unroll
                for (int ct = 0; ct < 2; ++ct) {
                    const int l = 16 * ct + j, lc = min(l, L - 1);
                    const double s_l = sd[lc], b_l = bed[lc];
                    dw_s(ct) = l < L ? s_l : 0.0; dw_b(ct) = l < L ? b_l : 0.0;
#pragma unroll
                    for (int kk = 0; kk < KD; ++kk) {
                        const int dd = 4 * kk + g;
                        const double w = Wed[min(dd, D - 1) * L + lc];
                        dw_w(kk, ct) = (dd < D && l < L) ? w : 0.0;
                    }
#pragma unroll
                    for (int r = 0; r < 4; ++r) dw_d(ct, r) = Wdd[lc * D + min(d0 + g + 4 * r, D - 1)];
                }
#pragma unroll
                for (int kk = 0; kk < KD; ++kk) avk[kk] = P1s[(d0 + j) * NFP + min(L + 4 * kk + g, NFP - 1)];
#pragma unroll
                for (int r = 0; r < 4; ++r) {
                    p1o[r] = P1s[(d0 + g + 4 * r) * NFP + fone];
#pragma unroll
                    for (int ct = 0; ct < 2; ++ct) p1l[ct][r] = P1s[(d0 + g + 4 * r) * NFP + min(16 * ct + j, L - 1)];
                }
                __builtin_amdgcn_sched_barrier(0);
#pragma unroll
                for (int ct = 0; ct < 2; ++ct) {
                    if (ct == 1 && RL1 == 0) continue;
                    const int l = 16 * ct + j;
#pragma unroll
                    for (int r = 0; r < 4; ++r) C[ct][r] = dw_s(ct) * p1l[ct][r] + dw_b(ct) * p1o[r];
#pragma unroll
                    for (int kk = 0; kk < KD; ++kk) C[ct] = __builtin_amdgcn_mfma_f64_16x16x4f64(avk[kk], dw_w(kk, ct), C[ct], 0, 0, 0);
#pragma unroll
                    for (int r = 0; r < 4; ++r) {
                        const int d = d0 + g + 4 * r;
                        if (l < L && d < D) { gq[off_wd + l * D + d] = c0 * C[ct][r]; wsum += dw_d(ct, r) * C[ct][r]; }
                    }
                }
            }
            wsum = lin_wave_sum(wsum);
            if (lane == 0) part[3 * NB] = wsum;
        }
        LIN_STAMP(4);
        __syncthreads();
        LIN_STAMP(5);
        const double rows = (double)a.rows;
        const float bc1 = (float)part[3 * NB + 4], bc2 = (float)part[3 * NB + 5];
#pragma unroll
        for (int k = 0; k < LKOUT; ++k) {
            const int idx = t + LNT * k;
            if (LNT * k >= P + 3) break;
            double gd = 0.0;
            if (idx < P && idx != off_eps) gd = gq[idx];
            else if (idx == off_eps || (idx >= P && idx < P + 3)) {
                double ssq = part[0], musq = part[1], z2r = part[2];
#pragma unroll
                for (int w = 1; w < NB; ++w) { ssq += part[3 * w]; musq += part[3 * w + 1]; z2r += part[3 * w + 2]; }
                ssq += part[3 * NB];
                const double klc = part[3 * NB + 3];
                if (idx == off_eps) gd = (double)a.eps_cli * (-0.5 * ssq * inv_var + 0.5 * rows * D + 0.5 * sigma * z2r * inv_var) * inv_bt;
                else {
                    const double dkl = (0.5 * musq - 0.5 * rows * klc) * inv_bt;
                    const double mse = (0.5 * ssq * inv_var + 0.5 * rows * D * ((double)kLog2Pi + eps)) * inv_bt;
                    gd = idx == P ? dkl + mse : (idx == P + 1 ? dkl : mse);
                }
            }
            const float gf = (float)gd;
            gout[k] = gf;
            if (idx == P && a.loss_hist) a.loss_hist[(long long)(tstep - 1) % a.loss_hist_cap] = gf;
            if (idx < P) adam_apply_f(pk(k), gf, mk(k), vk(k), a.lr, bc1, bc2);
        }
        LIN_STAMP(6);
    }
    __device__ __forceinline__ void store_state(const LinArgs& a, const float (&gout)[LKOUT], int tstep) {
        const int t = threadIdx.x;
#pragma unroll
        for (int k = 0; k < LKOUT; ++k) {
            const int idx = t + LNT * k;
            if (idx < P + kExtra) a.grads[idx] = gout[k];
            if (idx < P) { a.params[idx] = pk(k); a.m[idx] = mk(k); a.v[idx] = vk(k); }
        }
        if (t == 0) a.step_dev[0] = tstep;
    }
};

template <int NB, int DT, int LT>
using LinUpdMFor = std::conditional_t<NB == 3, LinUpdM<NB, DT, LT>, LinUpdMG<NB, DT, LT>>;

template <int NB, int DT, int LT>
__global__ __launch_bounds__(LNT) void lin_step_kernel(const LinArgs a) {
    extern __shared__ __attribute__((aligned(16))) char lin_smem[];
    const int b = blockIdx.x, t = threadIdx.x;
    constexpr int NO = NB * (NB + 1) / 2 * 256;
    if (b < a.has_update) {
        LinUpd<NB, DT, LT> u;
        u.carve(a, lin_smem);
        LIN_STAMP(0);
        const int tstep = a.step_dev[0] + 1;
        u.load_state(a);
        u.publish_params();
        u.template expand_M<false>(a.M_in);
        __syncthreads();
        float g[LKOUT];
        u.step(a, tstep, g);
        u.store_state(a, g, tstep);
        LIN_STAMP(7);
    } else if (b < a.has_update + a.n_reduce) {
        lin_reduce<false>(a.partial_in, a.M_out, a.ntiles, lin_smem, b - a.has_update, NO);
    } else {
        const int tile = b - a.has_update - a.n_reduce;
        const int wave = __builtin_amdgcn_readfirstlane(t >> 6), lane = t & 63;
        const LinTile tl(a.D, a.L, a.T);
        const int stride = max(tl.bytes, lin_scratch_bytes(NB)), v_off = stride, c_off = v_off + 4 * a.T;
        for (int p = wave; p < tl.np; p += LNW) lin_issue_piece(a, tl, a.x, a.z1, a.z2, tile, p, lin_smem, lane);
        lin_write_vcol(reinterpret_cast<float*>(lin_smem + v_off), a.T, (int)min((long long)a.T, (long long)a.B - (long long)tile * a.T), t);
        if (t == 0) *reinterpret_cast<float*>(lin_smem + c_off) = 0.f;
        lin_wait_vmcnt<0>();
        lin_barrier();
        lin_fix_ragged(a, tl, a.x, a.z1, a.z2, tile, lin_smem, t);
        f32x4 acc[NB * (NB + 1) / 2];
        lin_tile_products<NB, 0, LNW>(a, tl, lin_smem, 0, v_off, c_off, acc, lane, wave, [](int) {});
        lin_barrier();
        lin_tile_combine<NB, false, LNW>(acc, lin_smem, a.partial_out + (long long)tile * NO, t, wave, lane);
    }
}

template <int NB, int DT, int LT, int JT, bool GEN>
__global__ __launch_bounds__(LNT, 2) void lin_persist_kernel(const LinArgs a, const std::conditional_t<GEN, BatchArgs, LinPtrs> src) {
    extern __shared__ __attribute__((aligned(16))) char lin_smem[];
    const int b = blockIdx.x, t = threadIdx.x, N = a.n_steps;
    constexpr int NO = NB * (NB + 1) / 2 * 256;
    const int per_set = a.n_reduce / a.sets;
    if (b < a.has_update) {
        LinUpdMFor<NB, DT, LT> u;
        u.carve(a, lin_smem);
        int tstep = a.step_dev[0];
        u.load_state(a);
        float g[LKOUT];
#pragma unroll
        for (int k = 0; k < LKOUT; ++k) g[k] = 0.f;
        constexpr int NM = LinUpdMFor<NB, DT, LT>::NM;
        double mreg[NM], mnext[NM];
        bool have_next = false;
        LIN_STAMP(10);
        int sl = a.slot_upd;
        for (int n = 0; n < N; ++n) {
            const int sl_next = sl + 1 == kLinSlots ? 0 : sl + 1;
            LIN_STAMP(0);
            u.publish_params(a);
            LIN_STAMP(9);
            if (!have_next) {
                lin_wait_count(a.cnt_reduce + sl, (unsigned)per_set, a.status, (1u << 28) | ((unsigned)n << 16));
                if (t < 64 * NB) u.fetch_M(a.M_base + (long long)sl * NO, mreg);
            } else {
                __syncthreads();
#pragma unroll
                for (int k = 0; k < NM; ++k) mreg[k] = mnext[k];
            }
            LIN_STAMP(8);
            ++tstep;
            u.step(a, tstep, mreg, g, n + 1 < N ? a.cnt_reduce + sl_next : nullptr, (unsigned)per_set, a.M_base + (long long)sl_next * NO, mnext, have_next);
            LIN_STAMP(7);
            { [[maybe_unused]] unsigned long long te = 0; LIN_NOWQ(te); LIN_PUT(64 + n, te); }
            sl = sl_next;
        }
        u.store_state(a, g, tstep);
        for (int k = t; k < N * kLinShards; k += LNT) {
            int s = a.slot_upd + k / kLinShards;
            s = s >= kLinSlots ? s - kLinSlots : s;
            __hip_atomic_store(a.cnt_stream + (s * kLinShards + k % kLinShards) * kLinShardStride, 0u, __ATOMIC_RELAXED, __HIP_MEMORY_SCOPE_AGENT);
        }
        for (int k = t; k < N; k += LNT) {
            int s = a.slot_upd + k;
            s = s >= kLinSlots ? s - kLinSlots : s;
            __hip_atomic_store(a.cnt_reduce + s, 0u, __ATOMIC_RELAXED, __HIP_MEMORY_SCOPE_AGENT);
        }
    } else if (b < a.has_update + a.n_reduce) {
        const int rb = b - a.has_update, set = rb / per_set, ro = rb % per_set;
        const int tstep0 = a.step_dev[0];
        [[maybe_unused]] unsigned long long r0 = 0, r1 = 0, r2 = 0, racc_w = 0, racc_r = 0;
        int sl = a.slot_red + set;
        sl = sl >= kLinSlots ? sl - kLinSlots : sl;
        for (int n = set; n < a.n_red; n += a.sets, sl = sl + a.sets >= kLinSlots ? sl + a.sets - kLinSlots : sl + a.sets) {
            LIN_NOWQ(r0);
            lin_wait_shards(a.cnt_stream + sl * kLinShards * kLinShardStride, (unsigned)a.ntiles, a.status, (2u << 28) | ((unsigned)n << 16));
            LIN_NOWQ(r1);
            for (int sub = ro; sub < NO / 32; sub += 2 * per_set) {
                if (sub != ro) __syncthreads();
                const float* pin = a.partial_base + (long long)sl * a.ntiles * NO;
                const unsigned epoch = (unsigned)(tstep0 + a.d_red + n + 1);
                if (sub + per_set < NO / 32)
                    lin_reduce_pair(pin, a.M_base + (long long)sl * NO, a.ntiles, lin_smem, sub, sub + per_set, NO, a.comm, epoch, a.status);
                else lin_reduce<true>(pin, a.M_base + (long long)sl * NO, a.ntiles, lin_smem, sub, NO, &a.comm, epoch, a.status);
            }
            lin_wait_vmcnt<0>();
            __syncthreads();
            LIN_NOWQ(r2);
            racc_w += r1 - r0; racc_r += r2 - r1;
            if (rb == 5) { LIN_PUT(40, racc_w); LIN_PUT(41, racc_r); }
            if (rb == 5 && n < 3) { LIN_PUT(56 + 2 * n, r1); LIN_PUT(57 + 2 * n, r2); }
            if (t == 0) __hip_atomic_fetch_add(a.cnt_reduce + sl, 1u, __ATOMIC_RELAXED, __HIP_MEMORY_SCOPE_AGENT);
            { [[maybe_unused]] unsigned long long te = 0; LIN_NOW(te); LIN_PUTMAX(136 + n, te); }
        }
    } else {
        const int sid = b - a.has_update - a.n_reduce, S = a.n_stream;
        { [[maybe_unused]] unsigned long long te = 0; LIN_NOWQ(te); if (sid == 0) LIN_PUT(50, te); if (sid == S / 2) LIN_PUT(51, te); if (sid == S - 1) LIN_PUT(52, te); }
        const int wave = __builtin_amdgcn_readfirstlane(t >> 6), lane = t & 63;
        const LinTile tl(a.D, a.L, a.T);
        const int stride = max(tl.bytes, lin_ring_scratch_bytes(NB));
        const int v_off = 3 * stride, vr_off = v_off + 4 * a.T, c_off = vr_off + 4 * a.T;
        const float** tab = reinterpret_cast<const float**>(lin_smem + c_off + 16);
        if constexpr (!GEN) {
            if (t < 3 * kLinMaxPersist) {
                const int which = t / kLinMaxPersist, n = t % kLinMaxPersist;
                tab[t] = n < a.n_str ? (which == 0 ? src.x : which == 1 ? src.z1 : src.z2)[n] : nullptr;
            }
        }
        [[maybe_unused]] float* const Amat = reinterpret_cast<float*>(lin_smem + c_off + 16);
        if constexpr (GEN) {
            if (src.kind == 0 && t < src.dd * src.did) Amat[t] = src.A[t];
        }
        const int valid_last = a.B - (a.ntiles - 1) * a.T;
        lin_write_vcol(reinterpret_cast<float*>(lin_smem + v_off), a.T, a.T, t);
        lin_write_vcol(reinterpret_cast<float*>(lin_smem + vr_off), a.T, valid_last, t);
        if (t == 0) { *reinterpret_cast<float*>(lin_smem + c_off) = 0.f; *reinterpret_cast<unsigned*>(lin_smem + c_off + 8) = 0u; }
        __syncthreads();
        const int per_batch = sid < a.ntiles ? (a.ntiles - sid + S - 1) / S : 0, items = a.n_str * per_batch;
        const bool loader = wave >= kLinCW;
        const int lw = wave - kLinCW;
        constexpr int NLW = LNW - kLinCW;
        auto share = [&](int n) { return lw < n ? (n - lw + NLW - 1) / NLW : 0; };
        const int npw = (GEN || !loader) ? 0 : share(tl.nz1) + share(tl.nx) + share(tl.np - tl.nz1 - tl.nx);
        const int sw = wave < (NO / 4 + 63) / 64 ? 1 : 0;
        struct Pos {
            int idx, n, r, slot, bs;
            __device__ __forceinline__ void advance(int per_batch) {
                ++idx; slot = slot == 2 ? 0 : slot + 1;
                if (++r == per_batch) { r = 0; ++n; bs = bs == kLinSlots - 1 ? 0 : bs + 1; }
            }
        };
        auto pos_tile = [&](const Pos& q) { return sid + q.r * S; };
        Pos p_cur{0, 0, 0, 0, a.slot_str}, p_load{0, 0, 0, 0, a.slot_str}, p_sig{0, 0, 0, 0, a.slot_str};
        LinTileSrc nxt;
        nxt.on = false;
        auto prepare = [&]() __attribute__((always_inline)) {
            if constexpr (!GEN) {
                nxt.on = false;
                if (p_load.idx < items) {
                    const int n = p_load.n;
                    nxt.prepare(a, tab[n], tab[kLinMaxPersist + n], tab[2 * kLinMaxPersist + n], pos_tile(p_load), lin_smem + p_load.slot * stride);
                }
                p_load.advance(per_batch);
            }
        };
        auto issue_pieces = [&]() __attribute__((always_inline)) {
            if constexpr (!GEN) { if (!(VAEK_LIN_ABL & 8) && nxt.on) nxt.issue_tile(tl, lw, NLW, lane); }
        };
        constexpr int GT = NLW * 64;
        [[maybe_unused]] const int gD = DT ? DT : a.D, gL = LT ? LT : a.L, nzb = (gL + gD + 3) / 4;
        [[maybe_unused]] const int nlat = a.T * nzb, xr = (a.T + GT - 1) / GT, npair = nlat / (2 * GT), rem = nlat - 2 * GT * npair;
        [[maybe_unused]] const int gen_rounds = xr + npair + (rem + GT - 1) / GT;
        [[maybe_unused]] const unsigned step0 = (unsigned)(a.step_dev[0] + a.d_str);
        [[maybe_unused]] int g_kind = 0, g_dd = 0, g_did = 0; [[maybe_unused]] float g_noise = 0.f; [[maybe_unused]] unsigned g_tag = 0;
        if constexpr (GEN) { g_kind = src.kind; g_dd = src.dd; g_did = src.did; g_noise = src.noise_std; g_tag = src.tag; }
        auto gen_round = [&](const Pos& q, int k, int gt) __attribute__((always_inline)) {
            if constexpr (GEN) {
                if (q.idx < items && k < gen_rounds) {
                    const uint2 key = make_uint2((unsigned)src.seed, (unsigned)(src.seed >> 32));
                    const long long row_lo = (long long)pos_tile(q) * a.T;
                    const unsigned step = step0 + (unsigned)q.n;
                    char* slot = lin_smem + q.slot * stride;
                    auto put = [&](int z, const float (&n4)[4]) __attribute__((always_inline)) {
                        const int r = z / nzb, q = z - r * nzb, c0 = 4 * q;
                        const bool live = row_lo + r < a.B;
                        const f32x4 v4 = live ? f32x4{n4[0], n4[1], n4[2], n4[3]} : f32x4{0.f, 0.f, 0.f, 0.f};
                        float* z1r = reinterpret_cast<float*>(slot) + r * gL;
                        float* z2r = reinterpret_cast<float*>(slot + tl.oZ2) + r * gD;
                        if (c0 + 3 < gL && gL % 4 == 0) *reinterpret_cast<f32x4*>(z1r + c0) = v4;
                        else if (c0 >= gL && (c0 - gL) + 3 < gD && gD % 4 == 0 && gL % 4 == 0) *reinterpret_cast<f32x4*>(z2r + (c0 - gL)) = v4;
                        else {
#pragma unroll
                            for (int c = 0; c < 4; ++c) {
                                if (c0 + c < gL) z1r[c0 + c] = v4[c];
                                else if (c0 + c < gL + gD) z2r[c0 + c - gL] = v4[c];
                            }
                        }
                    };
                    auto draw = [&](int z, float (&n4)[4]) __attribute__((always_inline)) {
                        const int r = z / nzb;
                        latent_block(src, step, src.row0 + row_lo + r, key, z - r * nzb, n4);
                    };
                    if (k >= xr && k < xr + npair) {
                        const int za = 2 * GT * (k - xr) + gt;
                        float na[4], nb[4];
                        draw(za, na); draw(za + GT, nb);
                        put(za, na); put(za + GT, nb);
                    } else if (k >= xr + npair) {
                        const int z = 2 * GT * npair + GT * (k - xr - npair) + gt;
                        if (z < nlat) {
                            float n4[4];
                            draw(z, n4);
                            put(z, n4);
                        }
                    } else {
                        const int row = gt + GT * k;
                        if (row < a.T) {
                            const long long lrow = row_lo + row, grow = src.row0 + lrow;
                            const bool live = lrow < a.B;
                            float nrm[16];
                            dataset_normals(src, step, grow, key, nrm);
                            float* xr_ = reinterpret_cast<float*>(slot + tl.oX) + row * gD;
                            float inv = 0.f;
                            if (g_kind == 2) {
                                float nsq = 0.f;
#pragma unroll
                                for (int d = 0; d < 16; ++d) if (d < g_dd) nsq = fmaf(nrm[d], nrm[d], nsq);
                                inv = 1.f / sqrtf(nsq);
                            }
                            for (int c0 = 0; c0 < gD; c0 += 4) {
                                float o[4] = {0.f, 0.f, 0.f, 0.f};
                                if (c0 < g_dd) {
#pragma unroll
                                    for (int c = 0; c < 4; ++c) {
                                        const int d = c0 + c;
                                        float v = 0.f;
                                        if (d < g_dd) {
                                            if (g_kind == 0) {
#pragma unroll
                                                for (int kk = 0; kk < 16; ++kk) if (kk < g_did) v = fmaf(Amat[d * g_did + kk], nrm[kk], v);
                                            } else {
#pragma unroll
                                                for (int kk = 0; kk < 16; ++kk) v = (kk == d) ? nrm[kk] : v;
                                                v *= inv;
                                            }
                                        }
                                        o[c] = v;
                                    }
                                }
                                if (g_kind == 0 && g_noise > 0.f) {
                                    float n4[4];
                                    normals4(philox4x32_10(make_uint4((unsigned)grow, (unsigned)((g_did + 3) / 4 + c0 / 4), step, g_tag), key), n4);
#pragma unroll
                                    for (int c = 0; c < 4; ++c) o[c] = fmaf(g_noise, n4[c], o[c]);
                                }
                                const f32x4 v4 = live ? f32x4{o[0], o[1], o[2], o[3]} : f32x4{0.f, 0.f, 0.f, 0.f};
                                if (gD % 4 == 0) *reinterpret_cast<f32x4*>(xr_ + c0) = v4;
                                else {
#pragma unroll
                                    for (int c = 0; c < 4; ++c) if (c0 + c < gD) xr_[c0 + c] = v4[c];
                                }
                            }
                        }
                    }
                }
            }
        };
        [[maybe_unused]] unsigned* const ticket = reinterpret_cast<unsigned*>(lin_smem + c_off + 8);
        auto gen_share = [&](const Pos& q0, const Pos& q1, int nitems) __attribute__((always_inline)) {
            if constexpr (GEN) {
                const unsigned units = (unsigned)gen_rounds * NLW, total = units * (unsigned)nitems;
#pragma unroll 1
                for (;;) {
                    unsigned u = 0;
                    if (lane == 0) u = __hip_atomic_fetch_add(ticket, 1u, __ATOMIC_RELAXED, __HIP_MEMORY_SCOPE_WORKGROUP);
                    u = (unsigned)__builtin_amdgcn_readfirstlane((int)u);
                    if (u >= total) break;
                    const bool second = u >= units;
                    const unsigned v = second ? u - units : u;
                    gen_round(second ? q1 : q0, (int)(v / NLW), (int)(v % NLW) * 64 + lane);
                }
            }
        };
        unsigned* const my_shard = a.cnt_stream + (b & (kLinShards - 1)) * kLinShardStride;
        auto signal = [&]() {
            if (t == 0) __hip_atomic_fetch_add(my_shard + p_sig.bs * kLinShards * kLinShardStride, 1u, __ATOMIC_RELAXED, __HIP_MEMORY_SCOPE_AGENT);
            p_sig.advance(per_batch);
        };
        if constexpr (GEN) {
            Pos q1 = p_load;
            q1.advance(per_batch);
            gen_share(p_load, q1, 2);
            p_load.advance(per_batch); p_load.advance(per_batch);
            lin_barrier();
            if (t == 0) *ticket = 0u;
        } else if (loader) {
            prepare();
            issue_pieces();
            prepare();
            issue_pieces();
        }
        [[maybe_unused]] unsigned long long s0 = 0, s1 = 0, s2 = 0, s3 = 0, s4 = 0, s5 = 0, s6 = 0, sacc_i = 0, sacc_l = 0, sacc_f = 0, sacc_m = 0, sacc_p = 0, sacc_b = 0;
        for (int i = 0; i < items; ++i) {
            LIN_NOWQ(s0);
            lin_wait_vmcnt_upto((i + 1 < items ? npw : 0) + (i >= 1 ? sw : 0));
            LIN_NOWQ(s1);
            lin_barrier();
            LIN_NOWQ(s2);
            if (i >= 3) signal();
            const int n = p_cur.n, tile = pos_tile(p_cur), slot_off = p_cur.slot * stride;
            char* slot = lin_smem + slot_off;
            const bool ragged = tile == a.ntiles - 1 && valid_last < a.T;
            if constexpr (!GEN) {
                if (ragged) lin_fix_ragged(a, tl, tab[n], tab[kLinMaxPersist + n], tab[2 * kLinMaxPersist + n], tile, slot, t);
            }
            LIN_NOWQ(s3);
            f32x4 acc[NB * (NB + 1) / 2];
            if (!loader) lin_tile_products<NB, JT, kLinCW>(a, tl, lin_smem, slot_off, ragged ? vr_off : v_off, c_off, acc, lane, wave, [](int) {});
            if constexpr (GEN) {
                gen_share(p_load, p_load, 1);
                p_load.advance(per_batch);
            } else if (loader && i > 0) {
                prepare();
                issue_pieces();
            }
            LIN_NOWQ(s5);
            lin_barrier();
            if constexpr (GEN) { if (t == 0) *ticket = 0u; }
            LIN_NOWQ(s6);
            lin_tile_combine<NB, true, kLinCW>(acc, slot, a.partial_base + ((long long)p_cur.bs * a.ntiles + tile) * NO, t, wave, lane);
            if (i == 0) {
                lin_wait_vmcnt<0>();
                lin_barrier();
                signal();
                if (sid == 0) { [[maybe_unused]] unsigned long long te = 0; LIN_NOWQ(te); LIN_PUT(53, te); }
                if constexpr (!GEN) {
                    if (loader) {
                        prepare();
                        issue_pieces();
                    }
                }
            }
            LIN_NOWQ(s4);
            if (i + 1 < items) { sacc_i += s1 - s0; sacc_l += s2 - s1; sacc_f += s3 - s2; sacc_m += s4 - s3; sacc_p += s5 - s3; sacc_b += s6 - s5; }
            if (sid == 7) { LIN_PUT(42, sacc_i); LIN_PUT(43, sacc_l); LIN_PUT(44, sacc_f); LIN_PUT(45, sacc_m); LIN_PUT(46, (unsigned long long)items); LIN_PUT(47, sacc_p); LIN_PUT(48, sacc_b); }
            p_cur.advance(per_batch);
        }
        lin_wait_vmcnt<0>();
        lin_barrier();
        if (items - 2 >= 1) signal();
        if (items - 1 >= 1) signal();
        { [[maybe_unused]] unsigned long long te = 0; LIN_NOWQ(te); LIN_PUTMAX(49, te); }
    }
}

constexpr unsigned kLinMagic = 0x4c494e33u;
#ifndef VAEK_LIN_FOUR_BLOCK_TU
__global__ void lin_init_kernel(unsigned* cnt, int n_words, unsigned* status) {
    for (int k = threadIdx.x; k < n_words; k += blockDim.x) cnt[k] = 0u;
    if (threadIdx.x == 0 && status[1] != kLinMagic) { status[0] = 0u; status[1] = kLinMagic; }
}
#endif

typedef void (*LinPersistKernel)(const LinArgs, const LinPtrs);
typedef void (*LinPersistGenKernel)(const LinArgs, const BatchArgs);
LinPersistKernel lin_persist_four(int which);
LinPersistGenKernel lin_persist_four_gen(int which);

#ifndef VAEK_LIN_FOUR_BLOCK_TU
constexpr size_t kLinMaxLds = 160 * 1024;
constexpr size_t kLinCntStreamBytes = (size_t)kLinSlots * kLinShards * kLinShardStride * 4, kLinCntBytes = kLinCntStreamBytes + 1024, kLinHeadBytes = kLinCntBytes + 256;
static_assert(kLinSlots * sizeof(unsigned) <= 1024, "cnt_reduce");

LinPlan lin_plan(const vaek_ctx* c) {
    LinPlan p{};
    const int D = c->D, L = c->L;
    p.ok = c->cfg.n_enc_hidden == 0 && c->cfg.n_dec_hidden == 0 && !c->cfg.sigmoid_decoder && c->cfg.dtype == VAEK_F32 &&
           L + 2 * D + 1 <= 64 && (long long)c->B * std::min(D, L) >= 8;
    if (!p.ok) return p;
    p.NB = (L + 2 * D + 1 + 15) / 16 <= 3 ? 3 : 4;
    p.NO = p.NB * (p.NB + 1) / 2 * 256;
    const auto slot_bytes = [&](int T) { return std::max((size_t)LinTile(D, L, T).bytes, (size_t)lin_scratch_bytes(p.NB)); };
    const auto ring_slot_bytes = [&](int T) { return std::max((size_t)LinTile(D, L, T).bytes, (size_t)lin_ring_scratch_bytes(p.NB)); };
    const auto ring_bytes = [&](int T) { return 3 * ring_slot_bytes(T) + 8 * (size_t)T + 16 + 3 * kLinMaxPersist * sizeof(void*) + 64; };
    const auto ksteps_ok = [&](int T) { return (LinTile(D, L, T).np + LNW - kLinCW - 1) / (LNW - kLinCW) <= 18; };
    const int smax = c->n_cu - 1 - kLinReduceSets * kLinReduceWgs;
    const bool upd_ok = p.NB == 3 ? LinUpdM<3, 0, 0>::shape_ok(D, L) : LinUpdMG<4, 0, 0>::shape_ok(D, L);
    p.T = 256;
    if (p.NB == 3) {
        if (smax >= 16 && c->B > 256 * smax) {
            const int T = 32 * (int)(((long long)c->B + 32ll * smax - 1) / (32ll * smax));
            if (T <= 512 && ksteps_ok(T) && ring_bytes(T) <= kLinMaxLds) p.T = T;
        }
    } else if (upd_ok && smax >= 16) {
        int T = 256;
        while (T > 32 && !(ksteps_ok(T) && ring_bytes(T) <= kLinMaxLds)) T -= 32;
        p.T = T;
    }
    p.ntiles = (c->B + p.T - 1) / p.T;
    const size_t upd = std::max(p.NB == 3 ? LinUpd<3, 0, 0>::lds_bytes(D, L) : LinUpd<4, 0, 0>::lds_bytes(D, L),
                                p.NB == 3 ? LinUpdM<3, 0, 0>::lds_bytes(D, L, (int)c->P) : LinUpdMG<4, 0, 0>::lds_bytes(D, L, (int)c->P));
    p.lds_step = std::max(slot_bytes(p.T) + 4 * (size_t)p.T + 16, std::max(upd, (size_t)2 * 16 * 32 * sizeof(double))) + 64;
    p.lds_persist = std::max(std::max(p.lds_step, ring_bytes(p.T)), (size_t)82 * 1024);
    p.persist = upd_ok && p.lds_persist <= kLinMaxLds && ksteps_ok(p.T) && smax >= 16;
    if (p.persist) {
        const int per = (p.ntiles + smax - 1) / smax;
        p.n_stream = (p.ntiles + per - 1) / per;
        p.n_reduce = kLinReduceSets * std::min(kLinReduceWgs, p.NO / 32);
    }
    p.which_persist = p.NB == 3 ? (D == 12 && L == 20 && p.T == 288 ? 0 : 1) : (D == 20 && L == 20 && p.T == 192 ? 3 : 2);
    p.which_step = D == 12 && L == 20 ? 2 : p.NB - 3;
    const int slots = p.persist ? kLinSlots : 2;
    p.M_off = kLinHeadBytes;
    p.partial_off = p.M_off + (size_t)slots * p.NO * sizeof(double) + 256;
    p.ws_bytes = (p.partial_off + (size_t)slots * p.ntiles * p.NO * sizeof(float) + 256 + 255) / 256 * 256;
    if (c->cfg.world > 1 && p.persist) p.comm_bytes = (size_t)kLinCommBanks * c->cfg.world * 2 * p.NO * sizeof(unsigned long long);
    return p;
}

bool lin_steps_supported(const vaek_ctx* c) {
    return c->lin.ok && (c->cfg.world == 1 || (c->lin.persist && c->comm.ready && c->comm.lin_bytes > 0));
}
bool lin_steps_gen_supported(const vaek_ctx* c, int kind) { return lin_steps_supported(c) && c->lin.persist && (kind == 0 || kind == 2); }

struct LinWs { float* partial; double* M; unsigned* cnt; unsigned* cnt_reduce; unsigned* status; };
static LinWs lin_ws(const vaek_ctx* c, void* ws) {
    char* base = static_cast<char*>(ws) + c->ws_lin;
    LinWs w;
    w.cnt = reinterpret_cast<unsigned*>(base); w.cnt_reduce = reinterpret_cast<unsigned*>(base + kLinCntStreamBytes);
    w.status = reinterpret_cast<unsigned*>(base + kLinCntBytes);
    w.M = reinterpret_cast<double*>(base + c->lin.M_off); w.partial = reinterpret_cast<float*>(base + c->lin.partial_off);
    return w;
}

typedef void (*LinStepKernel)(const LinArgs);
static const LinPersistKernel kLinPersist[] = {lin_persist_kernel<3, 12, 20, 18, false>, lin_persist_kernel<3, 0, 0, 0, false>,
                                                lin_persist_four(0), lin_persist_four(1)};
static const LinPersistGenKernel kLinPersistGen[] = {lin_persist_kernel<3, 12, 20, 18, true>, lin_persist_kernel<3, 0, 0, 0, true>,
                                                     lin_persist_four_gen(0), lin_persist_four_gen(1)};
static const LinStepKernel kLinStep[] = {lin_step_kernel<3, 0, 0>, lin_step_kernel<4, 0, 0>, lin_step_kernel<3, 12, 20>};
template <typename K, size_t N> static int lin_kernel(const K (&table)[N], int which, K* fn) {
    static thread_local PerDeviceOnce attr_set[N];
    if (attr_set[which].need()) {
        VAEK_HIP_CHECK(hipFuncSetAttribute((const void*)table[which], hipFuncAttributeMaxDynamicSharedMemorySize, (int)kLinMaxLds));
        attr_set[which].mark();
    }
    *fn = table[which];
    return VAEK_OK;
}

static void lin_fill_common(const vaek_ctx* c, LinArgs& a, float* params, float* grads, float* m, float* v, int32_t* step_dev, float lr) {
    a.B = c->B; a.D = c->D; a.L = c->L; a.T = c->lin.T; a.ntiles = c->lin.ntiles;
    a.params = params; a.grads = grads; a.m = m; a.v = v; a.step_dev = step_dev; a.lr = lr;
    const double rows = c->cfg.world > 1 ? (double)c->Bt : (double)c->B;
    a.inv_bt = (float)(1.0 / (double)c->Bt); a.eps_cli = c->cfg.eps_cli; a.rows = (float)rows;
    a.rows_over_bt = (float)(rows / (double)c->Bt); a.off_eps = (int)c->off_eps; a.P = (int)c->P;
    a.comm = LinComm{};
    a.comm.world = 1;
    if (c->cfg.world > 1 && c->comm.ready && c->comm.lin_bytes > 0) {
        a.comm.world = c->cfg.world; a.comm.rank = c->cfg.rank; a.comm.ng2 = 2 * c->lin.NO;
        for (int r = 0; r < c->cfg.world; ++r)
            a.comm.peer[r] = reinterpret_cast<unsigned long long*>(static_cast<char*>(c->comm.peers[r]) + c->comm.lin_off);
    }
    a.loss_hist = c->loss_hist; a.loss_hist_cap = c->loss_hist_cap;
    static const int stagger = getenv("VAEK_LIN_STAGGER") ? atoi(getenv("VAEK_LIN_STAGGER")) : 3;
    a.stagger = stagger;
}

static int lin_ensure_init(vaek_ctx* c, const LinWs& w, void* ws, hipStream_t st) {
    if (c->lin_ws_ready == ws) return VAEK_OK;
    hipStreamCaptureStatus cap = hipStreamCaptureStatusNone;
    VAEK_HIP_CHECK(hipStreamIsCapturing(st, &cap));
    hipLaunchKernelGGL(lin_init_kernel, dim3(1), dim3(1024), 0, st, w.cnt, (int)(kLinCntBytes / 4), w.status);
    VAEK_HIP_CHECK(hipGetLastError());
    c->lin_ws_issued = ws;
    c->lin_ws_ready = cap == hipStreamCaptureStatusNone ? ws : nullptr;
    return VAEK_OK;
}

static int lin_train_steps_impl(vaek_ctx* c, float* params, float* grads, float* m, float* v, int32_t* step_dev, const float* const* xs,
                                const float* const* z1s, const float* const* z2s, const BatchArgs* gen, int n_steps, float lr, void* ws, hipStream_t st) {
    const LinPlan& p = c->lin;
    const LinWs w = lin_ws(c, ws);
    static const char* env = getenv("VAEK_LIN_PERSIST");
    static const int roles = getenv("VAEK_LIN_ROLES") ? atoi(getenv("VAEK_LIN_ROLES")) : 7;
    const bool persistent = p.persist && (gen || c->cfg.world > 1 || !(env && atoi(env) == 0));
    if (gen && !persistent) { set_error("vaek_train_steps_gen: this context has no persistent form"); return VAEK_ERR_INVALID; }
    if (persistent) {
        LinPersistKernel fn = nullptr;
        LinPersistGenKernel fng = nullptr;
        if (int rc = gen ? lin_kernel(kLinPersistGen, p.which_persist, &fng) : lin_kernel(kLinPersist, p.which_persist, &fn)) return rc;
        if (int rc = lin_ensure_init(c, w, ws, st)) return rc;
        for (int j = 0; j < lin_launches(n_steps); ++j) {
            const LinWindows win = lin_windows(n_steps, j);
            const int s0 = win.stream.first, n = win.stream.count;
            LinArgs a{};
            lin_fill_common(c, a, params, grads, m, v, step_dev, lr);
            a.persistent = 1; a.n_steps = win.update.count; a.n_red = win.reduce.count; a.n_str = n;
            a.slot_upd = win.update.first % kLinSlots; a.slot_red = win.reduce.first % kLinSlots; a.slot_str = s0 % kLinSlots;
            a.d_red = win.reduce.first - win.update.first; a.d_str = s0 - win.update.first;
            a.sets = kLinReduceSets;
            a.has_update = 1; a.n_reduce = p.n_reduce; a.n_stream = p.n_stream;
            if (!(roles & 4)) a.has_update = 0;
            if (!(roles & 2)) { a.has_update = 0; a.n_reduce = 0; }
            if (!(roles & 1)) a.n_stream = 0;
            if (roles != 7) c->lin_ws_ready = nullptr;
            a.partial_base = w.partial; a.M_base = w.M;
            a.cnt_stream = w.cnt; a.cnt_reduce = w.cnt_reduce; a.status = w.status;
            const dim3 grid((unsigned)(a.has_update + a.n_reduce + a.n_stream));
            if (gen) {
                ProfScope ps("lin_moments_persistent_gen", st);
                launch_k(ps, fng, grid, dim3(LNT), p.lds_persist, st, a, *gen);
            } else {
                LinPtrs ptrs{};
                for (int i = 0; i < n; ++i) { ptrs.x[i] = xs[s0 + i]; ptrs.z1[i] = z1s[s0 + i]; ptrs.z2[i] = z2s[s0 + i]; }
                ProfScope ps("lin_moments_persistent", st);
                launch_k(ps, fn, grid, dim3(LNT), p.lds_persist, st, a, ptrs);
            }
        }
        VAEK_HIP_CHECK(hipGetLastError());
        return VAEK_OK;
    }
    LinStepKernel fn = nullptr;
    if (int rc = lin_kernel(kLinStep, p.which_step, &fn)) return rc;
    const size_t pstride = (size_t)p.ntiles * p.NO;
    for (int n = 0; n < n_steps + 2; ++n) {
        LinArgs a{};
        lin_fill_common(c, a, params, grads, m, v, step_dev, lr);
        a.has_update = (n >= 2 && (roles & 4)) ? 1 : 0;
        a.n_reduce = (n >= 1 && n <= n_steps && (roles & 2)) ? p.NO / 32 : 0;
        a.n_stream = (n < n_steps && (roles & 1)) ? p.ntiles : 0;
        if (a.has_update + a.n_reduce + a.n_stream == 0) continue;
        if (a.n_stream) { a.x = xs[n]; a.z1 = z1s[n]; a.z2 = z2s[n]; a.partial_out = w.partial + (n & 1) * pstride; }
        if (a.n_reduce) { a.partial_in = w.partial + ((n - 1) & 1) * pstride; a.M_out = w.M + ((n - 1) & 1) * p.NO; }
        a.M_in = w.M + (n & 1) * p.NO;
        ProfScope ps(a.n_stream ? "lin_moments_step" : "lin_moments_drain", st);
        launch_k(ps, fn, dim3((unsigned)(a.has_update + a.n_reduce + a.n_stream)), dim3(LNT), p.lds_step, st, a);
    }
    VAEK_HIP_CHECK(hipGetLastError());
    return VAEK_OK;
}

int lin_train_steps(vaek_ctx* c, float* params, float* grads, float* m, float* v, int32_t* step_dev, const float* const* xs,
                    const float* const* z1s, const float* const* z2s, int n_steps, float lr, void* ws, hipStream_t st) {
    return lin_train_steps_impl(c, params, grads, m, v, step_dev, xs, z1s, z2s, nullptr, n_steps, lr, ws, st);
}
int lin_train_steps_gen(vaek_ctx* c, float* params, float* grads, float* m, float* v, int32_t* step_dev, const BatchArgs& gen, int n_steps,
                        float lr, void* ws, hipStream_t st) {
    return lin_train_steps_impl(c, params, grads, m, v, step_dev, nullptr, nullptr, nullptr, &gen, n_steps, lr, ws, st);
}

int lin_moments(vaek_ctx* c, const float* x, const float* z1, const float* z2, double* M_out, void* ws, hipStream_t st) {
    const LinPlan& p = c->lin;
    LinStepKernel fn = nullptr;
    if (int rc = lin_kernel(kLinStep, p.which_step, &fn)) return rc;
    LinArgs a{};
    lin_fill_common(c, a, nullptr, nullptr, nullptr, nullptr, nullptr, 0.f);
    a.n_stream = p.ntiles; a.x = x; a.z1 = z1; a.z2 = z2; a.partial_out = lin_ws(c, ws).partial;
    { ProfScope ps("lin_moments_stream", st); launch_k(ps, fn, dim3((unsigned)p.ntiles), dim3(LNT), p.lds_step, st, a); }
    a.n_stream = 0; a.n_reduce = p.NO / 32; a.partial_in = a.partial_out; a.M_out = M_out;
    a.comm = LinComm{}; a.comm.world = 1;
    { ProfScope ps("lin_moments_reduce", st); launch_k(ps, fn, dim3((unsigned)a.n_reduce), dim3(LNT), p.lds_step, st, a); }
    VAEK_HIP_CHECK(hipGetLastError());
    return VAEK_OK;
}
int lin_update(vaek_ctx* c, float* params, float* grads, float* m, float* v, int32_t* step_dev, const double* M_in, float lr, hipStream_t st) {
    LinStepKernel fn = nullptr;
    if (int rc = lin_kernel(kLinStep, c->lin.which_step, &fn)) return rc;
    LinArgs a{};
    lin_fill_common(c, a, params, grads, m, v, step_dev, lr);
    a.has_update = 1; a.M_in = M_in;
    ProfScope ps("lin_moments_update", st);
    launch_k(ps, fn, dim3(1), dim3(LNT), c->lin.lds_step, st, a);
    VAEK_HIP_CHECK(hipGetLastError());
    return VAEK_OK;
}

int lin_steps_status(vaek_ctx* c, void* ws, int* gave_up) {
    *gave_up = 0;
    if (c->lin_ws_issued != ws) return VAEK_OK;
    const LinWs w = lin_ws(c, ws);
    unsigned s = 0;
    VAEK_HIP_CHECK(hipMemcpy(&s, w.status, sizeof(s), hipMemcpyDeviceToHost));
    *gave_up = (int)s;
    if (s) {
        VAEK_HIP_CHECK(hipMemset(w.status, 0, sizeof(unsigned)));
        c->lin_ws_ready = nullptr;
    }
    return VAEK_OK;
}

#endif

}

#if defined(VAEK_LIN_STAMPS) && !defined(VAEK_LIN_FOUR_BLOCK_TU)
extern "C" int vaek_debug_lin_stamps(unsigned long long* buf) {
    return hipMemcpyToSymbol(HIP_SYMBOL(vaek::g_lin_stamp_buf), &buf, sizeof(buf)) == hipSuccess ? vaek::lin_stamps_four(buf) : -2;
}
#endif
```

### vae_training_amd/csrc/vaek_internal.h

```cpp
#pragma once
#include <hip/hip_runtime.h>
#include <stdint.h>
#include <stdio.h>
#include <string>
#include <vector>

#include "../../include/vaek.h"

namespace vaek {

constexpr int kExtra = 4;
constexpr float kLog2Pi = 1.8378770664093453f;
constexpr float kAdamB1 = 0.9f, kAdamB2 = 0.999f, kAdamEps = 1e-8f;

void set_error(const char* fmt, ...);
#define VAEK_HIP_CHECK(expr)                                                              \
    do {                                                                                  \
        hipError_t _e = (expr);                                                           \
        if (_e != hipSuccess) {                                                           \
            vaek::set_error("%s failed: %s (%s:%d)", #expr, hipGetErrorString(_e), __FILE__, __LINE__); \
            return VAEK_ERR_HIP;                                                          \
        }                                                                                 \
    } while (0)

struct Leaf {
    std::string name;
    int64_t offset;
    int rows, cols;
};

enum class Kind : uint8_t {
    F32,
    BF16,
    FIRST_SK,
    FIRST16,
    HIDDEN16,
    LAST_SK,
    LAST16,
};
enum class Pos : uint8_t { FIRST, HIDDEN, LAST };

struct Layer {
    int n_in, n_out;
    int64_t w_off;
    bool relu;
    Kind kind = Kind::F32;
    int S, rows_per_split;
    int64_t w16_off = 0;
};

struct Net {
    std::vector<Layer> layers;
    std::vector<size_t> act_off;
};

struct Profiler {
    bool on = false;
    std::vector<hipEvent_t> ev;
    std::vector<const char*> label;
    int n = 0, cap = 0;
};
extern thread_local Profiler* g_prof;
struct ProfScope {
    int idx = -1;
    ProfScope(const char* label, hipStream_t) {
        Profiler* p = g_prof;
        if (p && p->on && p->n < p->cap) { idx = p->n++; p->label[idx] = label; }
    }
    hipEvent_t start() const { return g_prof->ev[2 * idx]; }
    hipEvent_t stop() const { return g_prof->ev[2 * idx + 1]; }
};
}
#include <hip/hip_ext.h>
namespace vaek {
template <typename K, typename... Args>
inline void launch_k(const ProfScope& ps, K kernel, dim3 grid, dim3 block, size_t shmem, hipStream_t st, Args... args) {
    if (ps.idx >= 0) hipExtLaunchKernelGGL(kernel, grid, block, shmem, st, ps.start(), ps.stop(), 0, args...);
    else hipLaunchKernelGGL(kernel, grid, block, shmem, st, args...);
}

struct Comm {
    bool ready = false;
    void* local = nullptr;
    size_t bytes = 0;
    int ng = 0;
    std::vector<void*> peers;
    uint32_t epoch = 0;
    size_t lin_off = 0, lin_bytes = 0;
};

struct LinPlan {
    bool ok = false;
    int NB = 0, NO = 0;
    int T = 0, ntiles = 0;
    bool persist = false;
    int n_stream = 0, n_reduce = 0;
    size_t lds_persist = 0, lds_step = 0;
    int which_persist = 0, which_step = 0;
    size_t M_off = 0, partial_off = 0, ws_bytes = 0;
    size_t comm_bytes = 0;
};

}

struct vaek_ctx {
    vaek_config cfg;
    int B, D, L;
    int64_t Bt;
    int64_t P;
    std::vector<vaek::Leaf> leaves;
    vaek::Net enc, dec, sig;
    int64_t off_epsp, off_eps;
    int S, rows_per_split, Se, rows_per_esplit;
    bool fused;
    bool mlp3 = false;
    bool resident = false;
    size_t ws_samples, ws_dsamp, ws_gbuf0, ws_gbuf1, ws_slabs, ws_epart, ws_epart_blk, ws_rpart, ws_eblk, ws_fused, ws_mlp3, ws_wb16, ws_sk16, ws_skpart, ws_lin, ws_lwd, ws_resident, ws_total;
    bool lwd = false; int lwd_rb = 0;
    int max_width;
    int n_cu;
    vaek::Comm comm;
    vaek::Profiler prof;
    unsigned long long* dbg_stamps = nullptr;
    float* loss_hist = nullptr;
    int64_t loss_hist_cap = 0;
    vaek::LinPlan lin;
    void* lin_ws_issued = nullptr;
    void* lin_ws_ready = nullptr;
};

namespace vaek {

struct ProfBind {
    explicit ProfBind(vaek_ctx* c) { g_prof = c ? &c->prof : nullptr; }
    ~ProfBind() { g_prof = nullptr; }
};

int launch_dense_fwd(const float* x, const float* w, const float* b, float* y, int rows, int n_in,
                     int n_out, bool relu, hipStream_t st);
int launch_dense_fwd_reparam(const float* x, const float* w, const float* b, float* mu, float* samples,
                             const float* z1, const float* lv, int rows, int n_in, int n_out, hipStream_t st);
int launch_dense_bwd_dx(const float* dy, const float* w, const float* x_post, float* dx, int rows,
                        int n_in, int n_out, bool relu, bool accumulate, hipStream_t st);
int launch_dense_bwd_dw(const float* x, const float* dy, float* slab0, int64_t slab_stride, int S,
                        int rows_per_split, int rows, int n_in, int n_out, hipStream_t st);

int launch_dense_fwd_bf16(const float* x, const float* w, const float* b, float* y, int rows, int n_in, int n_out,
                          bool relu, hipStream_t st);
int launch_dense_fwd_reparam_bf16(const float* x, const float* w, const float* b, float* mu, float* samples,
                                  const float* z1, const float* lv, int rows, int n_in, int n_out, hipStream_t st);
int launch_dense_bwd_dx_bf16(const float* dy, const float* w, const float* x_post, float* dx, int rows, int n_in,
                             int n_out, bool relu, bool accumulate, hipStream_t st);
int launch_dense_bwd_dw_bf16(const float* x, const float* dy, float* slab0, int64_t slab_stride, int S, int rows_per_split,
                             int rows, int n_in, int n_out, hipStream_t st);

int launch_dense_fwd_out16(const float* x, const float* w, const float* b, __bf16* y, int rows, int n_in, int n_out, bool relu,
                           hipStream_t st);
int launch_dense_fwd_in16(const __bf16* x, const float* w, const float* b, float* y, int rows, int n_in, int n_out, hipStream_t st);
int launch_dense_fwd_reparam_in16(const __bf16* x, const float* w, const float* b, float* mu, float* samples, const float* z1,
                                  const float* lv, int rows, int n_in, int n_out, hipStream_t st);
int launch_dense_fwd_elbo_in16(const __bf16* h, const float* w, const float* b, float* d_out, const float* x, const float* z2,
                               const float* eps_param, float eps_cli, float inv_bt, float* part, int rows, int n_in, int n_out,
                               int* bm, int* nbx, hipStream_t st);
int launch_dense_bwd_dx_out16(const float* dy, const float* w, const __bf16* x_post, __bf16* dx, int rows, int n_in, int n_out,
                              bool accumulate, hipStream_t st);
int launch_dense_bwd_dw_x16(const __bf16* x, const float* dy, float* slab0, int64_t slab_stride, int S, int rows_per_split,
                            int rows, int n_in, int n_out, hipStream_t st);
int launch_dense_bwd_dw_dy16(const float* x, const __bf16* dy, float* slab0, int64_t slab_stride, int S, int rows_per_split,
                             int rows, int n_in, int n_out, hipStream_t st);
int launch_dense_bwd_dx_in16(const __bf16* dy, const float* w, float* dx, int rows, int n_in, int n_out, bool accumulate,
                             hipStream_t st);
int launch_hs_fwd(const __bf16* x, const __bf16* wT, const float* b, __bf16* y, int rows, int n_in, int n_out, bool relu,
                  hipStream_t st);
int launch_hs_dx(const __bf16* dy, const __bf16* w16, const __bf16* x_post, __bf16* dx, int rows, int n_in, int n_out,
                 hipStream_t st);
int launch_hs_dw(const __bf16* x, const __bf16* dy, float* slab0, int64_t slab_stride, int S, int rows_per_split, int rows,
                 int n_in, int n_out, hipStream_t st);
int launch_cvt_weights(const float* params, __bf16* out, const int* K, const int* N, const int64_t* w_off, const int64_t* out_off,
                       int n, hipStream_t st);

bool sk_supported(int d, int H);
inline bool is_sk(Kind k) { return k == Kind::FIRST_SK || k == Kind::LAST_SK; }
inline int sk_d(const Layer& l) { return l.kind == Kind::FIRST_SK ? l.n_in : l.n_out; }
inline int sk_H(const Layer& l) { return l.kind == Kind::FIRST_SK ? l.n_out : l.n_in; }
bool sk_bwd_mfma_form(int rows, int H, int d, int S);
size_t sk_partial_bytes(int d, int H, int S);
int launch_sk_first_fwd(const float* x, const float* w, const float* b, __bf16* y, int rows, int d, int H, bool relu, hipStream_t st);
int launch_sk_last_fwd(const __bf16* h, const __bf16* wp, const float* b, float* y, int rows, int H, int d, hipStream_t st);
int launch_sk_last_fwd_reparam(const __bf16* h, const __bf16* wp, const float* b, float* mu, float* samples, const float* z1,
                               const float* lv, int rows, int H, int d, hipStream_t st);
int launch_sk_last_fwd_elbo(const __bf16* h, const __bf16* wp, const float* b, float* d_out, const float* x, const float* z2,
                            const float* eps_param, float eps_cli, float inv_bt, float* part, int rows, int H, int d, int* bm,
                            int* nbx, hipStream_t st);
int launch_sk_first_dx(const __bf16* dy, const __bf16* wp, float* dx, int rows, int H, int d, bool accumulate, hipStream_t st);
int launch_sk_last_bwd(const __bf16* h, const float* dy, const float* w, __bf16* dh, float* partial, float* slab0, int64_t slab_stride,
                       int S, int rows, int H, int d, hipStream_t st);
int launch_sk_first_bwd(const float* x, const __bf16* dy, float* partial, float* slab0, int64_t slab_stride, int S, int rows, int H,
                        int d, hipStream_t st);
int launch_sk_prep(const float* params, __bf16* out, const int* H, const int* d, const int* transposed, const int64_t* w_off,
                   const int64_t* out_off, int n, hipStream_t st);

inline bool b16_width(int n) { return n % 64 == 0; }
Kind dense_kind(int dtype, bool b16, Pos pos, int n_in, int n_out);
struct DenseW {
    const float* w; const float* b;
    const __bf16* w16;
};
enum class Epi : uint8_t { NONE, REPARAM, ELBO };
struct Epilogue {
    Epi kind;
    float* samples; const float* z1; const float* lv;
    const float* x; const float* z2; const float* eps_param; float eps_cli, inv_bt; float* part; int bm, nbx;
};
int prep_weights(const float* params, const Layer* const* ls, int n, __bf16* wb16, __bf16* sk16, hipStream_t st);
int dense_fwd(const Layer& l, const DenseW& p, const void* x, void* y, int rows, Epilogue* e, hipStream_t st);
int dense_dx(const Layer& l, const DenseW& p, const void* dy, const void* x_post, void* dx, int rows, bool relu, bool accumulate,
             hipStream_t st);
int dense_dw(const Layer& l, const DenseW& p, const void* x, const void* dy, void* dx, float* slab0, int64_t slab_stride, float* skpart,
             int rows, hipStream_t st);

struct ElboArgs {
    const float* x; const float* y_lin; const float* y_sig; const float* z2; const float* mu;
    const float* eps_param;
    float eps_cli;
    float* d_lin; float* d_sig;
    float* partial;
    int rows, D, L, S, rows_per_split;
    float inv_bt;
    int32_t* step_dev;
};
int launch_elbo(const ElboArgs& a, hipStream_t st);
int launch_elbo_reduce(const float* part, int bm, int nbx, const float* mu, float* partial, int rows, int L, int S,
                       int rows_per_split, int32_t* step_dev, hipStream_t st);
int launch_dense_fwd_elbo(const float* h, const float* w, const float* b, float* d_out, const float* x, const float* z2,
                          const float* eps_param, float eps_cli, float inv_bt, float* part, int rows, int n_in, int n_out,
                          int* bm, int* nbx, hipStream_t st);
int launch_reparam_bwd(float* dsamp, const float* mu, const float* z1, float* partial,
                       int rows, int L, int S, int rows_per_split, float inv_bt, hipStream_t st);
struct FinalizeArgs {
    const float* slabs; int64_t slab_stride; int S;
    int nseg; int seg_end[32]; int seg_S[32];
    const float* epart; const float* rpart; int Se;
    int64_t P, off_epsp, off_eps; int L, D;
    const float* params;
    float eps_cli; float rows_over_bt; float inv_bt; float rows;
    float* grads;
    float* params_rw; float* m; float* v; const int32_t* step_dev; float lr;
// ... 133 lines not shown
```

### vae_training_amd/engine.py

```python
from __future__ import annotations

import ctypes as C
from collections import OrderedDict

import torch

from . import _lib, layout


def _ptr(t):
    if t is None:
        return None
    assert t.is_cuda and t.is_contiguous(), "libvaek takes contiguous device tensors"
    return C.c_void_p(t.data_ptr())


def _stream():
    return C.c_void_p(torch.cuda.current_stream().cuda_stream)


def _f32(t, device):
    if not torch.is_tensor(t):
        t = torch.as_tensor(t)
    return t.to(device=device, dtype=torch.float32).contiguous()
# ... 86 lines not shown
        assert counter.dtype == torch.int32 and counter.numel() == 2 and counter.is_cuda
        _lib.check(self.lib.vaek_train_step_gen(self.h, _ptr(params), _ptr(grads), _ptr(m), _ptr(v), _ptr(step_dev),
                                                _ptr(cur[0]), _ptr(cur[1]), _ptr(cur[2]), float(lr), _ptr(self.workspace),
                                                int(kind), _ptr(A), int(dd), int(did), int(pad), float(var_added),
                                                _ptr(nxt[0]), _ptr(nxt[1]), _ptr(nxt[2]), int(row0), int(seed) & (2**64 - 1),
                                                _ptr(counter), int(which), int(tag), _stream()))

    def supports_train_steps(self):
        f = C.c_int32()
        _lib.check(self.lib.vaek_supports_train_steps(self.h, C.byref(f)))
        return bool(f.value)

    def train_steps(self, params, grads, m, v, step_dev, batches, lr):
        n = len(batches)
        arr = lambda k: (C.c_void_p * n)(*[C.c_void_p(b[k].data_ptr()) for b in batches])
        for b in batches:
            assert all(t.is_cuda and t.is_contiguous() and t.dtype == torch.float32 for t in b)
        xs, z1s, z2s = arr(0), arr(1), arr(2)
        _lib.check(self.lib.vaek_train_steps(self.h, _ptr(params), _ptr(grads), _ptr(m), _ptr(v), _ptr(step_dev), xs, z1s, z2s, n,
                                             float(lr), _ptr(self.workspace), _stream()))

    def supports_train_steps_gen(self, kind):
        f = C.c_int32()
        _lib.check(self.lib.vaek_supports_train_steps_gen(self.h, int(kind), C.byref(f)))
        return bool(f.value)

    def train_steps_gen(self, params, grads, m, v, step_dev, n_steps, lr, kind, A, dd, did, pad, var_added, seed, tag=0, row0=0):
        _lib.check(self.lib.vaek_train_steps_gen(self.h, _ptr(params), _ptr(grads), _ptr(m), _ptr(v), _ptr(step_dev), int(kind), _ptr(A),
                                                 int(dd), int(did), int(pad), float(var_added), int(row0), int(seed) & (2**64 - 1), int(tag),
                                                 int(n_steps), float(lr), _ptr(self.workspace), _stream()))

    def supports_train_loop_gen(self, kind):
        f = C.c_int32()
        _lib.check(self.lib.vaek_supports_train_loop_gen(self.h, int(kind), C.byref(f)))
        return bool(f.value)

    @property
    def train_loop_steps_per_launch(self):
        return int(self.lib.vaek_train_loop_steps_per_launch())

    @property
    def trajectory_record_len(self):
        n = C.c_int64()
        _lib.check(self.lib.vaek_trajectory_record_len(self.h, C.byref(n)))
        return int(n.value)

    @staticmethod
    def _trajectory(trajectory):
        if not isinstance(trajectory, dict):
            trajectory = dict(buf=trajectory[0], every=trajectory[1])
        buf = trajectory["buf"]
        assert buf is None or buf.dtype == torch.float32
        tj = _lib.VaekTrajectory()
        tj.struct_size = int(trajectory.get("struct_size", C.sizeof(_lib.VaekTrajectory)))
        tj.every = int(trajectory["every"])
        tj.buf = _ptr(buf)
        shape = (1, 1, 1) if buf is None else tuple(buf.shape)
        tj.cap = int(trajectory["cap"]) if "cap" in trajectory else shape[-2]
        tj.record_stride = int(trajectory["record_stride"]) if "record_stride" in trajectory else shape[-1]
        tj.replica_stride = int(trajectory["replica_stride"]) if "replica_stride" in trajectory else tj.cap * tj.record_stride
        return tj

    def train_loop_gen(self, params, grads, m, v, step_dev, n_steps, lr, kind, A, dd, did, pad, var_added, seed, tag=0, row0=0,
                       trajectory=None):
        if trajectory is not None:
            tj = self._trajectory(trajectory)
            _lib.check(self.lib.vaek_train_loop_gen_traj(self.h, _ptr(params), _ptr(grads), _ptr(m), _ptr(v), _ptr(step_dev), int(kind), _ptr(A),
                                                         int(dd), int(did), int(pad), float(var_added), int(row0), int(seed) & (2**64 - 1),
                                                         int(tag), int(n_steps), float(lr), _ptr(self.workspace), _stream(), C.byref(tj)))
            return
        _lib.check(self.lib.vaek_train_loop_gen(self.h, _ptr(params), _ptr(grads), _ptr(m), _ptr(v), _ptr(step_dev), int(kind), _ptr(A),
                                                int(dd), int(did), int(pad), float(var_added), int(row0), int(seed) & (2**64 - 1), int(tag),
                                                int(n_steps), float(lr), _ptr(self.workspace), _stream()))

    @property
    def train_loop_max_replicas(self):
        return int(self.lib.vaek_train_loop_max_replicas())

    def train_loop_replicas_workspace(self, n):
        b = C.c_size_t()
        _lib.check(self.lib.vaek_train_loop_replicas_workspace_bytes(self.h, int(n), C.byref(b)))
        return int(b.value)

    def train_loop_gen_replicas(self, params, grads, m, v, step_dev, n_steps, lr, kind, A, dd, did, pad, var_added, seeds, lrs=None,
                                a_stride=0, loss_hist=None, workspace=None, tag=0, row0=0, n=None, state_stride=None, grads_stride=None,
                                loss_hist_cap=None, trajectory=None):
        rep = _lib.VaekReplicas()
        rep.struct_size = C.sizeof(_lib.VaekReplicas)
        rep.n = int(params.shape[0] if n is None else n)
        rep.state_stride = int(params.shape[1] if state_stride is None else state_stride)
        rep.grads_stride = int(grads.shape[1] if grads_stride is None else grads_stride)
        assert seeds is None or seeds.dtype == torch.int64
        assert lrs is None or lrs.dtype == torch.float32
        rep.seeds, rep.lrs = _ptr(seeds), _ptr(lrs)
        rep.a_stride = int(a_stride)
        rep.loss_hist = _ptr(loss_hist)
        rep.loss_hist_cap = int((0 if loss_hist is None else loss_hist.shape[-1]) if loss_hist_cap is None else loss_hist_cap)
        args = (self.h, _ptr(params), _ptr(grads), _ptr(m), _ptr(v), _ptr(step_dev), C.byref(rep), int(kind), _ptr(A), int(dd), int(did),
                int(pad), float(var_added), int(row0), int(tag), int(n_steps), float(lr), _ptr(workspace), _stream())
        if trajectory is not None:
            tj = self._trajectory(trajectory)
            _lib.check(self.lib.vaek_train_loop_gen_replicas_traj(*args, C.byref(tj)))
            return
        _lib.check(self.lib.vaek_train_loop_gen_replicas(*args))

    def supports_train_step_replicas(self):
        f = C.c_int32()
        _lib.check(self.lib.vaek_supports_train_step_replicas(self.h, C.byref(f)))
        return bool(f.value)

    @property
    def train_step_max_replicas(self):
        return int(self.lib.vaek_train_step_max_replicas())

    def train_step_replicas_workspace(self, n):
        b = C.c_size_t()
        _lib.check(self.lib.vaek_train_step_replicas_workspace_bytes(self.h, int(n), C.byref(b)))
        return int(b.value)

    def train_step_gen_replicas(self, params, grads, m, v, step_dev, cur, lr, kind, A, dd, did, pad, var_added, nxt, seeds, counter,
                                which, lrs=None, a_stride=0, loss_hist=None, workspace=None, tag=0, row0=0, n=None, state_stride=None,
                                grads_stride=None, loss_hist_cap=None):
        rep = _lib.VaekReplicas()
        rep.struct_size = C.sizeof(_lib.VaekReplicas)
        rep.n = int(params.shape[0] if n is None else n)
        rep.state_stride = int(params.shape[1] if state_stride is None else state_stride)
        rep.grads_stride = int(grads.shape[1] if grads_stride is None else grads_stride)
        assert seeds is None or seeds.dtype == torch.int64
        assert lrs is None or lrs.dtype == torch.float32
        assert counter is None or (counter.dtype == torch.int32 and counter.is_cuda)
        rep.seeds, rep.lrs = _ptr(seeds), _ptr(lrs)
        rep.a_stride = int(a_stride)
        rep.loss_hist = _ptr(loss_hist)
        rep.loss_hist_cap = int((0 if loss_hist is None else loss_hist.shape[-1]) if loss_hist_cap is None else loss_hist_cap)
        nxt = (None, None, None) if nxt is None else nxt
        _lib.check(self.lib.vaek_train_step_gen_replicas(self.h, _ptr(params), _ptr(grads), _ptr(m), _ptr(v), _ptr(step_dev), C.byref(rep),
                                                         _ptr(cur[0]), _ptr(cur[1]), _ptr(cur[2]), float(lr), _ptr(workspace), int(kind),
                                                         _ptr(A), int(dd), int(did), int(pad), float(var_added), _ptr(nxt[0]), _ptr(nxt[1]),
                                                         _ptr(nxt[2]), int(row0), _ptr(counter), int(which), int(tag), _stream()))

    def plan_train_steps(self, params, grads, m, v, step_dev, batches, lr):
        n = len(batches)
        for b in batches:
            assert all(t.is_cuda and t.is_contiguous() and t.dtype == torch.float32 for t in b)
        arr = lambda k: (C.c_void_p * n)(*[C.c_void_p(b[k].data_ptr()) for b in batches])
        keep = (params, grads, m, v, step_dev, list(batches))
        args = (self.h, _ptr(params), _ptr(grads), _ptr(m), _ptr(v), _ptr(step_dev), arr(0), arr(1), arr(2), n, C.c_float(lr), _ptr(self.workspace))
        fn, check = self.lib.vaek_train_steps, _lib.check

        def run(_keep=keep):
            check(fn(*args, _stream()))
        return run

    def moment_len(self):
        return self._moment_len

    def moments(self, x, z1, z2, M):
        assert M.dtype == torch.float64 and M.numel() >= self.moment_len()
        _lib.check(self.lib.vaek_train_steps_moments(self.h, _ptr(x), _ptr(z1), _ptr(z2), _ptr(M), _ptr(self.workspace), _stream()))

    def moments_update(self, params, grads, m, v, step_dev, M, lr):
        _lib.check(self.lib.vaek_train_steps_update(self.h, _ptr(params), _ptr(grads), _ptr(m), _ptr(v), _ptr(step_dev), _ptr(M), float(lr),
                                                    _ptr(self.workspace), _stream()))

    def train_steps_gave_up(self):
        f = C.c_int32()
        _lib.check(self.lib.vaek_train_steps_status(self.h, _ptr(self.workspace), C.byref(f)))
        self.train_steps_status_word = f.value & 0xffffffff
        return f.value != 0

    def grads_only(self, params, grads, step_dev, x, z1, z2):
        _lib.check(self.lib.vaek_train_step_grads_only(self.h, _ptr(params), _ptr(grads), _ptr(step_dev), _ptr(x),
                                                       _ptr(z1), _ptr(z2), _ptr(self.workspace), _stream()))

    def buckets(self):
        n = C.c_int32()
        _lib.check(self.lib.vaek_bucket_count(self.h, C.byref(n)))
        out = []
        for i in range(n.value):
            off, cnt = C.c_int64(), C.c_int64()
            _lib.check(self.lib.vaek_bucket_info(self.h, i, C.byref(off), C.byref(cnt)))
            out.append((off.value, cnt.value))
        return out

    def grads_bucketed(self, params, grads, step_dev, x, z1, z2, events):
        arr = (C.c_void_p * len(events))(*[C.c_void_p(e.cuda_event) for e in events])
        _lib.check(self.lib.vaek_train_step_grads_bucketed(self.h, _ptr(params), _ptr(grads), _ptr(step_dev), _ptr(x), _ptr(z1),
                                                           _ptr(z2), arr, _ptr(self.workspace), _stream()))

    def apply(self, params, grads, m, v, step_dev, lr):
        _lib.check(self.lib.vaek_train_step_apply(self.h, _ptr(params), _ptr(grads), _ptr(m), _ptr(v),
                                                  _ptr(step_dev), float(lr), _stream()))

    def loss_eval(self, params, x, z1, z2):
        out = torch.empty(4, dtype=torch.float32, device=self.device)
        _lib.check(self.lib.vaek_loss_eval(self.h, _ptr(params), _ptr(x), _ptr(z1), _ptr(z2), _ptr(out),
                                           _ptr(self.workspace), _stream()))
        return out

    def forward(self, params, x, z1, z2, sampling=False, eps=0.0, want_mu=True):
        rows = z1.shape[0]
        x_hat = torch.empty(rows, self.D, dtype=torch.float32, device=self.device)
        mu = torch.empty(rows, self.L, dtype=torch.float32, device=self.device) if want_mu else None
        _lib.check(self.lib.vaek_forward(self.h, _ptr(params), _ptr(x), _ptr(z1), _ptr(z2), int(bool(sampling)),
                                         float(eps), _ptr(x_hat), _ptr(mu), rows, _ptr(self.workspace), _stream()))
        return x_hat, mu

    def make_batch(self, kind, A, dd, did, pad, var_added, rows, seed, step_dev=None, step=0, tag=0, row0=0,
                   want_x=True, want_z=True, out=None, counter=None, which=0):
        if out is None:
            Dx = dd + pad + (1 if kind == 1 else 0)
            x = torch.empty(rows, Dx, dtype=torch.float32, device=self.device) if want_x else None
            z1 = torch.empty(rows, self.L, dtype=torch.float32, device=self.device) if want_z else None
            z2 = torch.empty(rows, self.D, dtype=torch.float32, device=self.device) if want_z else None
        else:
            x, z1, z2 = out
        if counter is not None:
            assert counter.dtype == torch.int32 and counter.numel() == 2 and counter.is_cuda
            _lib.check(self.lib.vaek_make_batch_next(self.h, int(kind), _ptr(A), int(dd), int(did), int(pad), float(var_added),
                                                     _ptr(x), _ptr(z1), _ptr(z2), int(rows), int(row0),
                                                     int(seed) & (2**64 - 1), _ptr(counter), int(which), int(tag), _stream()))
            return x, z1, z2
        _lib.check(self.lib.vaek_make_batch(self.h, int(kind), _ptr(A), int(dd), int(did), int(pad), float(var_added),
                                            _ptr(x), _ptr(z1), _ptr(z2), int(rows), int(row0), int(seed) & (2**64 - 1),
                                            _ptr(step_dev), int(step), int(tag), _stream()))
        return x, z1, z2

    def rng_fill(self, n, seed, step=0, tag=0, bits=False):
        out_n = torch.empty(n, dtype=torch.float32, device=self.device)
        out_u = torch.empty(n, dtype=torch.int32, device=self.device) if bits else None
        _lib.check(self.lib.vaek_rng_fill(self.h, _ptr(out_n), _ptr(out_u), int(n), int(seed) & (2**64 - 1), int(step),
                                          int(tag), _stream()))
        return (out_n, out_u) if bits else out_n

    def set_loss_history(self, buf):
        self._loss_hist = buf
        _lib.check(self.lib.vaek_set_loss_history(self.h, _ptr(buf), 0 if buf is None else buf.numel()))

    def profile_begin(self, max_records=4096):
        _lib.check(self.lib.vaek_profile_begin(self.h, int(max_records)))

    def profile_report(self):
        import json
        buf = C.create_string_buffer(8192)
        _lib.check(self.lib.vaek_profile_report(self.h, buf, 8192))
        return json.loads(buf.value.decode())

    def measure_peaks(self, copy_bytes=1 << 30, reps=5):
        src = torch.empty(copy_bytes, dtype=torch.uint8, device=self.device).random_(0, 255)
        dst = torch.empty_like(src)
        scratch = torch.zeros(16, dtype=torch.float32, device=self.device)
        flops = C.c_double()
        st = _stream()
        plan = [("microbench_mfma_f32", 0, 20000, 1), ("microbench_mfma_bf16", 1, 40000, 1)]
        for _ in range(2):
            _lib.check(self.lib.vaek_microbench_copy(self.h, _ptr(src), _ptr(dst), copy_bytes, st))
            for _, kind, iters, wps in plan:
                _lib.check(self.lib.vaek_microbench_mfma(self.h, kind, iters, wps, _ptr(scratch), C.byref(flops), st))
        torch.cuda.synchronize()
        self.profile_begin(64)
        fl = {}
        for _ in range(reps):
            _lib.check(self.lib.vaek_microbench_copy(self.h, _ptr(src), _ptr(dst), copy_bytes, st))
            for name, kind, iters, wps in plan:
                _lib.check(self.lib.vaek_microbench_mfma(self.h, kind, iters, wps, _ptr(scratch), C.byref(flops), st))
                fl[name] = flops.value
        torch.cuda.synchronize()
        rep = self.profile_report()
        out = {"hbm_copy_GBps": 2.0 * copy_bytes * rep["microbench_stream_copy"]["count"] / (rep["microbench_stream_copy"]["total_ms"] * 1e-3) / 1e9}
        for name, _, _, _ in plan:
            out[name.replace("microbench_", "") + "_TFLOPs"] = fl[name] * rep[name]["count"] / (rep[name]["total_ms"] * 1e-3) / 1e12
        return out

    def measure_launch_floor(self, n=100, reps=20):
        import time
        launch = lambda k: _lib.check(self.lib.vaek_microbench_launch(self.h, 0, 1, k, None, None, _stream()))
        launch(4)
        torch.cuda.synchronize()
        side = torch.cuda.Stream(device=self.device)
        side.wait_stream(torch.cuda.current_stream())
        with torch.cuda.stream(side):
            g = torch.cuda.CUDAGraph()
            with torch.cuda.graph(g, stream=side):
                launch(n)
        torch.cuda.current_stream().wait_stream(side)
        g.replay()
        torch.cuda.synchronize()
        t0 = time.perf_counter()
        for _ in range(reps):
            g.replay()
        torch.cuda.synchronize()
        return (time.perf_counter() - t0) / (n * reps) * 1e6

    def dense_fwd(self, x, w, b, relu=False):
        rows, n_in = x.shape
        n_out = w.shape[1]
        y = torch.empty(rows, n_out, dtype=torch.float32, device=self.device)
        _lib.check(self.lib.vaek_dense_fwd(self.h, _ptr(x), _ptr(w), _ptr(b), _ptr(y), rows, n_in, n_out,
                                           int(relu), _stream()))
        return y

    def dense_fwd_reparam(self, x, w, b, z1, logvar_e):
        rows, n_in = x.shape
        n_out = w.shape[1]
        mu = torch.empty(rows, n_out, dtype=torch.float32, device=self.device)
        samples = torch.empty_like(mu)
# ... 47 lines not shown
```

Before: 18.63 billion samples/s.

## Group tiles into partial images and keep multiple batches in flight

Stream workgroups now accumulate G consecutive tiles into one partial image before combining, which cuts the number of partial images reducers must read and wait on. The slot ring and launch windows are generalised so F batches can be in flight between stream, reduce and update stages. The update workgroup also moves the loss reduction into a dedicated wave and moves the next-counter poll off the critical path. This adds complexity in the slot and window bookkeeping, and a larger workspace.

```diff
diff --git a/include/vaek.h b/include/vaek.h
--- a/include/vaek.h
+++ b/include/vaek.h
@@ -115,6 +115,7 @@
                         int32_t did, int32_t pad, float var_added, float* x_next, float* z1_next, float* z2_next, int64_t row0,
                         uint64_t seed, int32_t* counter, int32_t which, uint32_t tag, void* stream);
 int vaek_supports_train_steps(const vaek_ctx* ctx, int32_t* yes);
+int vaek_train_steps_plan(const vaek_ctx* ctx, int32_t* plan);
 int vaek_train_steps(vaek_ctx* ctx, float* params, float* grads, float* m, float* v, int32_t* step_dev,
                      const float* const* xs, const float* const* z1s, const float* const* z2s, int32_t n_steps, float lr,
                      void* workspace, void* stream);
diff --git a/vae_training_amd/_lib.py b/vae_training_amd/_lib.py
--- a/vae_training_amd/_lib.py
+++ b/vae_training_amd/_lib.py
@@ -88,6 +88,7 @@
     "vaek_train_step_gen": (C.c_int, [_vp, _vp, _vp, _vp, _vp, _vp, _vp, _vp, _vp, _f32, _vp, _i32, _vp, _i32, _i32, _i32, _f32,
                                       _vp, _vp, _vp, _i64, C.c_uint64, _vp, _i32, C.c_uint32, _vp]),
     "vaek_supports_train_steps": (C.c_int, [_vp, C.POINTER(_i32)]),
+    "vaek_train_steps_plan": (C.c_int, [_vp, C.POINTER(_i32)]),
     "vaek_train_steps": (C.c_int, [_vp, _vp, _vp, _vp, _vp, _vp, _vp, _vp, _vp, _i32, _f32, _vp, _vp]),
     "vaek_train_steps_status": (C.c_int, [_vp, _vp, C.POINTER(_i32)]),
     "vaek_supports_train_steps_gen": (C.c_int, [_vp, _i32, C.POINTER(_i32)]),
diff --git a/vae_training_amd/csrc/api.hip b/vae_training_amd/csrc/api.hip
--- a/vae_training_amd/csrc/api.hip
+++ b/vae_training_amd/csrc/api.hip
@@ -1012,6 +1012,13 @@
                                     rep->lrs, rep->a_stride, rep->loss_hist, rep->loss_hist_cap);
 }
 
+int vaek_train_steps_plan(const vaek_ctx* ctx, int32_t* plan) {
+    if (!ctx || !plan) { set_error("null argument"); return VAEK_ERR_INVALID; }
+    const LinPlan& p = ctx->lin;
+    plan[0] = p.T; plan[1] = p.ntiles; plan[2] = p.ok ? p.G : 0; plan[3] = p.n_img; plan[4] = p.ok ? p.F : 0;
+    return VAEK_OK;
+}
+
 int vaek_train_steps_moment_len(const vaek_ctx* ctx, int64_t* len) {
     if (!ctx || !len) { set_error("null argument"); return VAEK_ERR_INVALID; }
     *len = ctx->lin.NO;
diff --git a/vae_training_amd/csrc/linear_moments.hip b/vae_training_amd/csrc/linear_moments.hip
--- a/vae_training_amd/csrc/linear_moments.hip
+++ b/vae_training_amd/csrc/linear_moments.hip
@@ -15,31 +15,40 @@
 
 constexpr int LNT = 512, LNW = LNT / 64;
 constexpr int kLinMaxPersist = 64;
-constexpr int kLinCarry = 2, kLinSlots = kLinMaxPersist + kLinCarry;
+constexpr int kLinMaxF = 4;
+constexpr int lin_slots(int F) { return kLinMaxPersist + F + 1; }
+constexpr int kLinSlots = lin_slots(kLinMaxF);
 struct LinWindow { int first, count; };
 struct LinWindows { LinWindow stream, reduce, update; };
-constexpr LinWindows lin_windows(int K, int j) {
+constexpr LinWindows lin_windows(int K, int j, int F) {
     const int s0 = kLinMaxPersist * j, s1 = s0 + kLinMaxPersist < K ? s0 + kLinMaxPersist : K;
     const bool last = s1 == K;
-    const int r0 = s0 >= 1 ? s0 - 1 : 0, u0 = s0 >= 2 ? s0 - 2 : 0;
-    return LinWindows{{s0, s1 - s0}, {r0, (last ? K : s1 - 1) - r0}, {u0, (last ? K : s1 - 2) - u0}};
+    const int r0 = s0 >= F ? s0 - F : 0, u0 = s0 >= F + 1 ? s0 - F - 1 : 0;
+    return LinWindows{{s0, s1 - s0}, {r0, (last ? K : s1 - F) - r0}, {u0, (last ? K : s1 - F - 1) - u0}};
 }
 constexpr int lin_launches(int K) { return (K + kLinMaxPersist - 1) / kLinMaxPersist; }
-constexpr bool lin_windows_ok(int K) {
+constexpr bool lin_windows_ok(int K, int F) {
     int s = 0, r = 0, u = 0;
     for (int j = 0; j < lin_launches(K); ++j) {
-        const LinWindows w = lin_windows(K, j);
+        const LinWindows w = lin_windows(K, j, F);
         if (w.stream.first != s || w.reduce.first != r || w.update.first != u) return false;
         if (w.stream.count < 1 || w.stream.count > kLinMaxPersist || w.reduce.count < 1 || w.update.count < 1) return false;
         s += w.stream.count; r += w.reduce.count; u += w.update.count;
-        if (r > s || u > r || s - w.update.first > kLinSlots) return false;
+        if (r > s || u > r || s - w.update.first > lin_slots(F)) return false;
     }
     return s == K && r == K && u == K;
 }
-static_assert(lin_windows_ok(1) && lin_windows_ok(2) && lin_windows_ok(64) && lin_windows_ok(65) && lin_windows_ok(66) && lin_windows_ok(128) &&
-              lin_windows_ok(129) && lin_windows_ok(130) && lin_windows_ok(960), "launch windows of a vaek_train_steps call");
-static_assert(lin_windows(64, 0).update.count == 64 && lin_windows(130, 1).update.first == 62 && lin_windows(130, 1).reduce.first == 63 &&
-              lin_windows(130, 2).update.count == 4, "launch windows of a vaek_train_steps call");
+constexpr bool lin_windows_ok_all(int F) {
+    for (int K : {1, 2, 3, 4, 5, 63, 64, 65, 66, 67, 68, 69, 70, 127, 128, 129, 130, 131, 132, 133, 134, 192, 193, 960}) if (!lin_windows_ok(K, F)) return false;
+    return true;
+}
+static_assert(lin_windows_ok_all(1) && lin_windows_ok_all(2) && lin_windows_ok_all(3) && lin_windows_ok_all(4), "launch windows of a vaek_train_steps call");
+static_assert(lin_slots(1) == 66 && lin_windows(64, 0, 1).update.count == 64 && lin_windows(130, 0, 1).reduce.count == 63 && lin_windows(130, 0, 1).update.count == 62 &&
+              lin_windows(130, 1, 1).update.first == 62 && lin_windows(130, 1, 1).reduce.first == 63 && lin_windows(130, 1, 1).reduce.count == 64 &&
+              lin_windows(130, 1, 1).update.count == 64 && lin_windows(130, 2, 1).reduce.first == 127 && lin_windows(130, 2, 1).update.first == 126 &&
+              lin_windows(130, 2, 1).update.count == 4, "one batch in flight: the windows of the launch-per-step shift");
+static_assert(lin_windows(960, 1, 4).reduce.first == 60 && lin_windows(960, 1, 4).update.first == 59 && lin_windows(960, 14, 4).update.count == 69 &&
+              lin_windows(960, 0, 4).update.count == 59, "four batches in flight");
 constexpr int kLinReduceSets = 1;
 constexpr int kLinReduceWgs = 24;
 
@@ -51,6 +60,7 @@
 struct LinArgs {
     int has_update, n_reduce, n_stream;
     int B, D, L, ntiles, T;
+    int G, n_img, nslots;
     const float* x; const float* z1; const float* z2; float* partial_out;
     const float* partial_in; double* M_out;
     const double* M_in;
@@ -309,7 +319,7 @@
 constexpr int kLinCW = 4;
 template <int NB, int JT, int CW, typename Hook>
 __device__ __forceinline__ void lin_tile_products(const LinArgs& a, const LinTile& tl, const char* smem, int slot_off, int v_off, int c_off,
-                                                  f32x4 (&acc)[NB * (NB + 1) / 2], int lane, int wave, Hook&& hook) {
+                                                  f32x4 (&acc)[NB * (NB + 1) / 2], int lane, int wave, Hook&& hook, bool zero = true) {
     constexpr int NBLK = NB * (NB + 1) / 2;
     const int g = lane >> 4, D = a.D, L = a.L;
     int fb[NB], fs[NB];
@@ -322,8 +332,10 @@
         else if (f == L + 2 * D) { fb[u] = v_off; fs[u] = 4; }
         else { fb[u] = c_off; fs[u] = 0; }
     }
-#pragma unroll
-    for (int k = 0; k < NBLK; ++k) acc[k] = f32x4{0.f, 0.f, 0.f, 0.f};
+    if (zero) {
+#pragma unroll
+        for (int k = 0; k < NBLK; ++k) acc[k] = f32x4{0.f, 0.f, 0.f, 0.f};
+    }
     const int J = JT ? JT : a.T / (4 * CW), wbase = (a.T / CW) * wave, jfull = J & ~3;
     auto products = [&](const float (&op)[NB]) __attribute__((always_inline)) {
         int k = 0;
@@ -776,19 +788,21 @@
     static constexpr int RL1 = LT ? (LT > 16 ? (LT - 16 + 3) / 4 : 0) : 4;
     static constexpr int NM = 4 + RL1 + 2 * KD + 1;
     int D, L, P, fone, off_be, off_wd, off_bd, off_epsp, off_eps;
-    double *Wed, *Wdd, *bed, *bdd, *sd, *elv, *lvd, *scal, *part, *P1s, *gq;
+    double *Wed, *Wdd, *bed, *bdd, *sd, *elv, *lvd, *scal, *part, *P1s, *gq, *mq;
     float p[LKOUT], m[LKOUT], v[LKOUT];
     int mo[NM];
 
     static __host__ __device__ constexpr bool shape_ok(int D, int L) { return D <= 16 && L <= 32 && L + 2 * D + 1 <= NFP && NB == 3; }
     static __host__ size_t lds_bytes(int D, int L, int P) {
-        return sizeof(double) * ((size_t)2 * D * L + 4 * L + D + 8 + 16 + 16 * NFP + (size_t)(P + kExtra + 7));
+        return sizeof(double) * ((size_t)2 * D * L + 4 * L + D + 8 + 16 + 16 * NFP + (size_t)(P + kExtra + 7) + 64 * NB);
     }
     __device__ __forceinline__ void carve(const LinArgs& a, char* smem) {
         D = DT ? DT : a.D; L = LT ? LT : a.L; P = a.P; fone = L + 2 * D; off_eps = a.off_eps;
         off_be = D * L; off_wd = off_be + L; off_bd = off_wd + L * D; off_epsp = off_bd + D;
         Wed = reinterpret_cast<double*>(smem); Wdd = Wed + D * L; bed = Wdd + L * D; bdd = bed + L; sd = bdd + D; elv = sd + L; lvd = elv + L;
-        scal = lvd + L; part = scal + 8; P1s = part + 16; gq = P1s + 16 * NFP;
+        scal = lvd + L; part = scal + 8;
+        mq = part + 16;
+        P1s = mq + 64 * NB; gq = P1s + 16 * NFP;
     }
     __device__ __forceinline__ void load_state(const LinArgs& a) {
         const int t = threadIdx.x;
@@ -798,6 +812,7 @@
             p[k] = a.params[idx]; m[k] = a.m[idx]; v[k] = a.v[idx];
         }
         if (off_eps < 0 && t == 0) { const double e = (double)a.eps_cli; scal[0] = e; scal[1] = lin_exp(0.5 * e); scal[2] = lin_exp(-e); }
+        if (t < kExtra) gq[P + t] = 0.0;
         const int lane = t & 63, j = lane & 15, g = lane >> 4, f = min(16 * (t >> 6) + j, NFP - 1);
         int k = 0;
 #pragma unroll
@@ -841,7 +856,6 @@
                                          unsigned per_set, const double* M_next, double (&mnext)[NM], bool& have_next) {
         const int t = threadIdx.x, wave = __builtin_amdgcn_readfirstlane(t >> 6), lane = t & 63, j = lane & 15, g = lane >> 4;
         LIN_STAMP(1);
-        if (t == 64 * (NB + 2)) scal[4] = (next_cnt && __hip_atomic_load(next_cnt, __ATOMIC_RELAXED, __HIP_MEMORY_SCOPE_AGENT) >= per_set) ? 1.0 : 0.0;
         const double eps = scal[0], sigma = scal[1], inv_var = scal[2], inv_bt = (double)a.inv_bt, c0 = inv_var * inv_bt;
         d4 sm[2], p1;
         double musq_p = 0.0, ssq_p = 0.0, z2r_p = 0.0;
@@ -903,6 +917,7 @@
             if (lane == 0) {
                 part[12] = tot;
                 part[13] = (double)(-expm1f((float)tstep * -0.10536051565782628f)); part[14] = (double)(-expm1f((float)tstep * -0.0010005003335835335f));
+                scal[4] = (next_cnt && __hip_atomic_load(next_cnt, __ATOMIC_RELAXED, __HIP_MEMORY_SCOPE_AGENT) >= per_set) ? 1.0 : 0.0;
             }
         }
         LIN_STAMP(2);
@@ -983,8 +998,9 @@
                     if (is_x) ssq_p -= pd; else { ssq_p += sigma * pd; z2r_p += pd; }
                 }
             }
-            musq_p = lin_wave_sum(musq_p); ssq_p = lin_wave_sum(ssq_p); z2r_p = lin_wave_sum(z2r_p);
-            if (lane == 0) { part[3 * wave] = ssq_p; part[3 * wave + 1] = musq_p; part[3 * wave + 2] = z2r_p; }
+            mq[64 * wave + lane] = musq_p;
+            ssq_p = lin_wave_sum(ssq_p); z2r_p = lin_wave_sum(z2r_p);
+            if (lane == 0) { part[3 * wave] = ssq_p; part[3 * wave + 2] = z2r_p; }
         } else if (wave == NB) {
             d4 C[2];
             double wsum = 0.0, avk[KD], p1l[2][4], p1o[4], dw_sr[2], dw_br[2], dw_wr[KD][2], dw_dr[2][4];
@@ -1036,6 +1052,22 @@
         __syncthreads();
         LIN_STAMP(5);
         const double rows = (double)a.rows;
+        if (wave == NB + 2) {
+            double mu[NB];
+#pragma unroll
+            for (int w = 0; w < NB; ++w) mu[w] = lin_wave_sum(mq[64 * w + lane]);
+            if (lane < 3) {
+                double musq = mu[0];
+#pragma unroll
+                for (int w = 1; w < NB; ++w) musq += mu[w];
+                const double ssq = part[0] + part[3] + part[6] + part[9], klc = part[12];
+                const double dkl = (0.5 * musq - 0.5 * rows * klc) * inv_bt;
+                const double mse = (0.5 * ssq * inv_var + 0.5 * rows * D * ((double)kLog2Pi + eps)) * inv_bt;
+                const float gf = (float)(lane == 0 ? dkl + mse : (lane == 1 ? dkl : mse));
+                gq[P + lane] = (double)gf;
+                if (lane == 0 && a.loss_hist) a.loss_hist[(long long)(tstep - 1) % a.loss_hist_cap] = gf;
+            }
+        }
         const float bc1 = (float)part[13], bc2 = (float)part[14];
 #pragma unroll
         for (int k = 0; k < LKOUT; ++k) {
@@ -1043,18 +1075,12 @@
             if (LNT * k >= P + 3) break;
             double gd = 0.0;
             if (idx < P && idx != off_eps) gd = gq[idx];
-            else if (idx == off_eps || (idx >= P && idx < P + 3)) {
-                const double ssq = part[0] + part[3] + part[6] + part[9], musq = part[1] + part[4] + part[7], z2r = part[2] + part[5] + part[8], klc = part[12];
-                if (idx == off_eps) gd = (double)a.eps_cli * (-0.5 * ssq * inv_var + 0.5 * rows * D + 0.5 * sigma * z2r * inv_var) * inv_bt;
-                else {
-                    const double dkl = (0.5 * musq - 0.5 * rows * klc) * inv_bt;
-                    const double mse = (0.5 * ssq * inv_var + 0.5 * rows * D * ((double)kLog2Pi + eps)) * inv_bt;
-                    gd = idx == P ? dkl + mse : (idx == P + 1 ? dkl : mse);
-                }
+            else if (idx == off_eps) {
+                const double ssq = part[0] + part[3] + part[6] + part[9], z2r = part[2] + part[5] + part[8];
+                gd = (double)a.eps_cli * (-0.5 * ssq * inv_var + 0.5 * rows * D + 0.5 * sigma * z2r * inv_var) * inv_bt;
             }
             const float gf = (float)gd;
             gout[k] = gf;
-            if (idx == P && a.loss_hist) a.loss_hist[(long long)(tstep - 1) % a.loss_hist_cap] = gf;
             if (idx < P) adam_apply_f(p[k], gf, m[k], v[k], a.lr, bc1, bc2);
         }
         LIN_STAMP(6);
@@ -1064,9 +1090,9 @@
 #pragma unroll
         for (int k = 0; k < LKOUT; ++k) {
             const int idx = t + LNT * k;
-            if (idx < P + kExtra) a.grads[idx] = gout[k];
-            if (idx < P) { a.params[idx] = p[k]; a.m[idx] = m[k]; a.v[idx] = v[k]; }
-        }
+            if (idx < P) { a.grads[idx] = gout[k]; a.params[idx] = p[k]; a.m[idx] = m[k]; a.v[idx] = v[k]; }
+        }
+        if (t < kExtra) a.grads[P + t] = (float)gq[P + t];
         if (t == 0) a.step_dev[0] = tstep;
     }
 };
@@ -1484,10 +1510,11 @@
         constexpr int NM = LinUpdMFor<NB, DT, LT>::NM;
         double mreg[NM], mnext[NM];
         bool have_next = false;
+        [[maybe_unused]] unsigned long long prefetched = 0;
         LIN_STAMP(10);
         int sl = a.slot_upd;
         for (int n = 0; n < N; ++n) {
-            const int sl_next = sl + 1 == kLinSlots ? 0 : sl + 1;
+            const int sl_next = sl + 1 == a.nslots ? 0 : sl + 1;
             LIN_STAMP(0);
             u.publish_params(a);
             LIN_STAMP(9);
@@ -1504,17 +1531,20 @@
             u.step(a, tstep, mreg, g, n + 1 < N ? a.cnt_reduce + sl_next : nullptr, (unsigned)per_set, a.M_base + (long long)sl_next * NO, mnext, have_next);
             LIN_STAMP(7);
             { [[maybe_unused]] unsigned long long te = 0; LIN_NOWQ(te); LIN_PUT(64 + n, te); }
+            if (have_next) ++prefetched;
             sl = sl_next;
         }
+        LIN_PUT(54, prefetched); LIN_PUT(55, (unsigned long long)N);
+        __syncthreads();
         u.store_state(a, g, tstep);
         for (int k = t; k < N * kLinShards; k += LNT) {
             int s = a.slot_upd + k / kLinShards;
-            s = s >= kLinSlots ? s - kLinSlots : s;
+            s = s >= a.nslots ? s - a.nslots : s;
             __hip_atomic_store(a.cnt_stream + (s * kLinShards + k % kLinShards) * kLinShardStride, 0u, __ATOMIC_RELAXED, __HIP_MEMORY_SCOPE_AGENT);
         }
         for (int k = t; k < N; k += LNT) {
             int s = a.slot_upd + k;
-            s = s >= kLinSlots ? s - kLinSlots : s;
+            s = s >= a.nslots ? s - a.nslots : s;
             __hip_atomic_store(a.cnt_reduce + s, 0u, __ATOMIC_RELAXED, __HIP_MEMORY_SCOPE_AGENT);
         }
     } else if (b < a.has_update + a.n_reduce) {
@@ -1522,18 +1552,18 @@
         const int tstep0 = a.step_dev[0];
         [[maybe_unused]] unsigned long long r0 = 0, r1 = 0, r2 = 0, racc_w = 0, racc_r = 0;
         int sl = a.slot_red + set;
-        sl = sl >= kLinSlots ? sl - kLinSlots : sl;
-        for (int n = set; n < a.n_red; n += a.sets, sl = sl + a.sets >= kLinSlots ? sl + a.sets - kLinSlots : sl + a.sets) {
+        sl = sl >= a.nslots ? sl - a.nslots : sl;
+        for (int n = set; n < a.n_red; n += a.sets, sl = sl + a.sets >= a.nslots ? sl + a.sets - a.nslots : sl + a.sets) {
             LIN_NOWQ(r0);
-            lin_wait_shards(a.cnt_stream + sl * kLinShards * kLinShardStride, (unsigned)a.ntiles, a.status, (2u << 28) | ((unsigned)n << 16));
+            lin_wait_shards(a.cnt_stream + sl * kLinShards * kLinShardStride, (unsigned)a.n_img, a.status, (2u << 28) | ((unsigned)n << 16));
             LIN_NOWQ(r1);
             for (int sub = ro; sub < NO / 32; sub += 2 * per_set) {
                 if (sub != ro) __syncthreads();
-                const float* pin = a.partial_base + (long long)sl * a.ntiles * NO;
+                const float* pin = a.partial_base + (long long)sl * a.n_img * NO;
                 const unsigned epoch = (unsigned)(tstep0 + a.d_red + n + 1);
                 if (sub + per_set < NO / 32)
-                    lin_reduce_pair(pin, a.M_base + (long long)sl * NO, a.ntiles, lin_smem, sub, sub + per_set, NO, a.comm, epoch, a.status);
-                else lin_reduce<true>(pin, a.M_base + (long long)sl * NO, a.ntiles, lin_smem, sub, NO, &a.comm, epoch, a.status);
+                    lin_reduce_pair(pin, a.M_base + (long long)sl * NO, a.n_img, lin_smem, sub, sub + per_set, NO, a.comm, epoch, a.status);
+                else lin_reduce<true>(pin, a.M_base + (long long)sl * NO, a.n_img, lin_smem, sub, NO, &a.comm, epoch, a.status);
             }
             lin_wait_vmcnt<0>();
             __syncthreads();
@@ -1565,24 +1595,46 @@
         const int valid_last = a.B - (a.ntiles - 1) * a.T;
         lin_write_vcol(reinterpret_cast<float*>(lin_smem + v_off), a.T, a.T, t);
         lin_write_vcol(reinterpret_cast<float*>(lin_smem + vr_off), a.T, valid_last, t);
-        if (t == 0) { *reinterpret_cast<float*>(lin_smem + c_off) = 0.f; *reinterpret_cast<unsigned*>(lin_smem + c_off + 8) = 0u; }
+        if (t == 0) {
+            *reinterpret_cast<float*>(lin_smem + c_off) = 0.f;
+            *reinterpret_cast<unsigned*>(lin_smem + c_off + 8) = 0u; *reinterpret_cast<unsigned*>(lin_smem + c_off + 12) = 0u;
+        }
         __syncthreads();
-        const int per_batch = sid < a.ntiles ? (a.ntiles - sid + S - 1) / S : 0, items = a.n_str * per_batch;
         const bool loader = wave >= kLinCW;
         const int lw = wave - kLinCW;
         constexpr int NLW = LNW - kLinCW;
         auto share = [&](int n) { return lw < n ? (n - lw + NLW - 1) / NLW : 0; };
         const int npw = (GEN || !loader) ? 0 : share(tl.nz1) + share(tl.nx) + share(tl.np - tl.nz1 - tl.nx);
         const int sw = wave < (NO / 4 + 63) / 64 ? 1 : 0;
+        struct Walk { int G, n_img, glast, dn, ds, nslots; };
+        const Walk walk{a.G, a.n_img, a.ntiles - (a.n_img - 1) * a.G, S / a.n_img, S % a.n_img, a.nslots};
         struct Pos {
-            int idx, n, r, slot, bs;
-            __device__ __forceinline__ void advance(int per_batch) {
+            int idx, n, s, k, gc, slot, bs;
+            __device__ __forceinline__ void next_super(const Walk& w) {
+                k = 0; s += w.ds; n += w.dn; bs += w.dn;
+                if (s >= w.n_img) { s -= w.n_img; ++n; ++bs; }
+                if (bs >= w.nslots) bs -= w.nslots;
+                gc = s == w.n_img - 1 ? w.glast : w.G;
+            }
+            __device__ __forceinline__ void advance(const Walk& w) {
                 ++idx; slot = slot == 2 ? 0 : slot + 1;
-                if (++r == per_batch) { r = 0; ++n; bs = bs == kLinSlots - 1 ? 0 : bs + 1; }
-            }
+                if (++k == gc) next_super(w);
+            }
+            __device__ __forceinline__ bool first() const { return k == 0; }
+            __device__ __forceinline__ bool last() const { return k == gc - 1; }
         };
-        auto pos_tile = [&](const Pos& q) { return sid + q.r * S; };
-        Pos p_cur{0, 0, 0, 0, a.slot_str}, p_load{0, 0, 0, 0, a.slot_str}, p_sig{0, 0, 0, 0, a.slot_str};
+        auto pos_tile = [&](const Pos& q) { return q.s * walk.G + q.k; };
+        Pos p_cur;
+        {
+            const int n0 = sid / walk.n_img, s0 = sid - n0 * walk.n_img;
+            int bs0 = a.slot_str + n0;
+            bs0 = bs0 >= walk.nslots ? bs0 - walk.nslots : bs0;
+            p_cur = Pos{0, n0, s0, 0, s0 == walk.n_img - 1 ? walk.glast : walk.G, 0, bs0};
+        }
+        Pos p_load = p_cur, p_sig = p_cur;
+        int items = 0;
+        for (Pos q = p_cur; q.n < a.n_str; q.next_super(walk)) items += q.gc;
+        const int first_end = items > 0 ? p_cur.gc - 1 : -1;
         LinTileSrc nxt;
         nxt.on = false;
         auto prepare = [&]() __attribute__((always_inline)) {
@@ -1592,7 +1644,7 @@
                     const int n = p_load.n;
                     nxt.prepare(a, tab[n], tab[kLinMaxPersist + n], tab[2 * kLinMaxPersist + n], pos_tile(p_load), lin_smem + p_load.slot * stride);
                 }
-                p_load.advance(per_batch);
+                p_load.advance(walk);
             }
         };
         auto issue_pieces = [&]() __attribute__((always_inline)) {
@@ -1697,8 +1749,8 @@
                 }
             }
         };
-        [[maybe_unused]] unsigned* const ticket = reinterpret_cast<unsigned*>(lin_smem + c_off + 8);
-        auto gen_share = [&](const Pos& q0, const Pos& q1, int nitems) __attribute__((always_inline)) {
+        [[maybe_unused]] unsigned* const tickets = reinterpret_cast<unsigned*>(lin_smem + c_off + 8);
+        auto gen_share = [&](const Pos& q0, const Pos& q1, int nitems, unsigned* ticket) __attribute__((always_inline)) {
             if constexpr (GEN) {
                 const unsigned units = (unsigned)gen_rounds * NLW, total = units * (unsigned)nitems;
 #pragma unroll 1
@@ -1716,15 +1768,14 @@
         unsigned* const my_shard = a.cnt_stream + (b & (kLinShards - 1)) * kLinShardStride;
         auto signal = [&]() {
             if (t == 0) __hip_atomic_fetch_add(my_shard + p_sig.bs * kLinShards * kLinShardStride, 1u, __ATOMIC_RELAXED, __HIP_MEMORY_SCOPE_AGENT);
-            p_sig.advance(per_batch);
+            p_sig.next_super(walk);
         };
         if constexpr (GEN) {
             Pos q1 = p_load;
-            q1.advance(per_batch);
-            gen_share(p_load, q1, 2);
-            p_load.advance(per_batch); p_load.advance(per_batch);
+            q1.advance(walk);
+            gen_share(p_load, q1, 2, tickets + 1);
+            p_load.advance(walk); p_load.advance(walk);
             lin_barrier();
-            if (t == 0) *ticket = 0u;
         } else if (loader) {
             prepare();
             issue_pieces();
@@ -1732,55 +1783,62 @@
             issue_pieces();
         }
         [[maybe_unused]] unsigned long long s0 = 0, s1 = 0, s2 = 0, s3 = 0, s4 = 0, s5 = 0, s6 = 0, sacc_i = 0, sacc_l = 0, sacc_f = 0, sacc_m = 0, sacc_p = 0, sacc_b = 0;
+        bool sig2 = false, sig1 = false;
+        f32x4 acc[NB * (NB + 1) / 2];
         for (int i = 0; i < items; ++i) {
             LIN_NOWQ(s0);
-            lin_wait_vmcnt_upto((i + 1 < items ? npw : 0) + (i >= 1 ? sw : 0));
+            lin_wait_vmcnt_upto((i + 1 < items ? npw : 0) + (sig1 ? sw : 0));
             LIN_NOWQ(s1);
             lin_barrier();
             LIN_NOWQ(s2);
-            if (i >= 3) signal();
+            if (sig2) signal();
+            if constexpr (GEN) { if (t == 0) tickets[(i + 1) & 1] = 0u; }
             const int n = p_cur.n, tile = pos_tile(p_cur), slot_off = p_cur.slot * stride;
+            const bool ends = p_cur.last(), early = i == first_end;
             char* slot = lin_smem + slot_off;
             const bool ragged = tile == a.ntiles - 1 && valid_last < a.T;
             if constexpr (!GEN) {
                 if (ragged) lin_fix_ragged(a, tl, tab[n], tab[kLinMaxPersist + n], tab[2 * kLinMaxPersist + n], tile, slot, t);
             }
             LIN_NOWQ(s3);
-            f32x4 acc[NB * (NB + 1) / 2];
-            if (!loader) lin_tile_products<NB, JT, kLinCW>(a, tl, lin_smem, slot_off, ragged ? vr_off : v_off, c_off, acc, lane, wave, [](int) {});
+            if (!loader) lin_tile_products<NB, JT, kLinCW>(a, tl, lin_smem, slot_off, ragged ? vr_off : v_off, c_off, acc, lane, wave, [](int) {}, p_cur.first());
             if constexpr (GEN) {
-                gen_share(p_load, p_load, 1);
-                p_load.advance(per_batch);
-            } else if (loader && i > 0) {
+                gen_share(p_load, p_load, 1, tickets + (i & 1));
+                p_load.advance(walk);
+            } else if (loader && !early) {
                 prepare();
                 issue_pieces();
             }
             LIN_NOWQ(s5);
-            lin_barrier();
-            if constexpr (GEN) { if (t == 0) *ticket = 0u; }
-            LIN_NOWQ(s6);
-            lin_tile_combine<NB, true, kLinCW>(acc, slot, a.partial_base + ((long long)p_cur.bs * a.ntiles + tile) * NO, t, wave, lane);
-            if (i == 0) {
-                lin_wait_vmcnt<0>();
+            if (ends) {
                 lin_barrier();
-                signal();
-                if (sid == 0) { [[maybe_unused]] unsigned long long te = 0; LIN_NOWQ(te); LIN_PUT(53, te); }
-                if constexpr (!GEN) {
-                    if (loader) {
-                        prepare();
-                        issue_pieces();
+                LIN_NOWQ(s6);
+                lin_tile_combine<NB, true, kLinCW>(acc, slot, a.partial_base + ((long long)p_cur.bs * a.n_img + p_cur.s) * NO, t, wave, lane);
+                if (early) {
+                    lin_wait_vmcnt<0>();
+                    lin_barrier();
+                    signal();
+                    if (sid == 0) { [[maybe_unused]] unsigned long long te = 0; LIN_NOWQ(te); LIN_PUT(53, te); }
+                    if constexpr (!GEN) {
+                        if (loader) {
+                            prepare();
+                            issue_pieces();
+                        }
                     }
                 }
+            } else {
+                LIN_NOWQ(s6);
             }
             LIN_NOWQ(s4);
             if (i + 1 < items) { sacc_i += s1 - s0; sacc_l += s2 - s1; sacc_f += s3 - s2; sacc_m += s4 - s3; sacc_p += s5 - s3; sacc_b += s6 - s5; }
             if (sid == 7) { LIN_PUT(42, sacc_i); LIN_PUT(43, sacc_l); LIN_PUT(44, sacc_f); LIN_PUT(45, sacc_m); LIN_PUT(46, (unsigned long long)items); LIN_PUT(47, sacc_p); LIN_PUT(48, sacc_b); }
-            p_cur.advance(per_batch);
+            sig2 = sig1; sig1 = ends && !early;
+            p_cur.advance(walk);
         }
         lin_wait_vmcnt<0>();
         lin_barrier();
-        if (items - 2 >= 1) signal();
-        if (items - 1 >= 1) signal();
+        if (sig2) signal();
+        if (sig1) signal();
         { [[maybe_unused]] unsigned long long te = 0; LIN_NOWQ(te); LIN_PUTMAX(49, te); }
     }
 }
@@ -1829,6 +1887,7 @@
         p.T = T;
     }
     p.ntiles = (c->B + p.T - 1) / p.T;
+    p.G = 1; p.n_img = p.ntiles; p.F = 1;
     const size_t upd = std::max(p.NB == 3 ? LinUpd<3, 0, 0>::lds_bytes(D, L) : LinUpd<4, 0, 0>::lds_bytes(D, L),
                                 p.NB == 3 ? LinUpdM<3, 0, 0>::lds_bytes(D, L, (int)c->P) : LinUpdMG<4, 0, 0>::lds_bytes(D, L, (int)c->P));
     p.lds_step = std::max(slot_bytes(p.T) + 4 * (size_t)p.T + 16, std::max(upd, (size_t)2 * 16 * 32 * sizeof(double))) + 64;
@@ -1838,13 +1897,18 @@
         const int per = (p.ntiles + smax - 1) / smax;
         p.n_stream = (p.ntiles + per - 1) / per;
         p.n_reduce = kLinReduceSets * std::min(kLinReduceWgs, p.NO / 32);
+        if (p.NB == 3) p.G = p.ntiles >= 64 ? 4 : p.ntiles >= 32 ? 2 : 1;
+        p.n_img = (p.ntiles + p.G - 1) / p.G;
+        p.F = (p.n_stream + p.n_img - 1) / p.n_img;
+        if (p.F > kLinMaxF) { p.G = 1; p.n_img = p.ntiles; p.F = (p.n_stream + p.n_img - 1) / p.n_img; }
     }
     p.which_persist = p.NB == 3 ? (D == 12 && L == 20 && p.T == 288 ? 0 : 1) : (D == 20 && L == 20 && p.T == 192 ? 3 : 2);
     p.which_step = D == 12 && L == 20 ? 2 : p.NB - 3;
-    const int slots = p.persist ? kLinSlots : 2;
+    const int slots = p.persist ? lin_slots(p.F) : 2;
+    const size_t images = std::max(p.persist ? (size_t)slots * p.n_img : (size_t)0, (size_t)2 * p.ntiles);
     p.M_off = kLinHeadBytes;
     p.partial_off = p.M_off + (size_t)slots * p.NO * sizeof(double) + 256;
-    p.ws_bytes = (p.partial_off + (size_t)slots * p.ntiles * p.NO * sizeof(float) + 256 + 255) / 256 * 256;
+    p.ws_bytes = (p.partial_off + images * p.NO * sizeof(float) + 256 + 255) / 256 * 256;
     if (c->cfg.world > 1 && p.persist) p.comm_bytes = (size_t)kLinCommBanks * c->cfg.world * 2 * p.NO * sizeof(unsigned long long);
     return p;
 }
@@ -1923,12 +1987,14 @@
         if (int rc = gen ? lin_kernel(kLinPersistGen, p.which_persist, &fng) : lin_kernel(kLinPersist, p.which_persist, &fn)) return rc;
         if (int rc = lin_ensure_init(c, w, ws, st)) return rc;
         for (int j = 0; j < lin_launches(n_steps); ++j) {
-            const LinWindows win = lin_windows(n_steps, j);
+            const int nslots = lin_slots(p.F);
+            const LinWindows win = lin_windows(n_steps, j, p.F);
             const int s0 = win.stream.first, n = win.stream.count;
             LinArgs a{};
             lin_fill_common(c, a, params, grads, m, v, step_dev, lr);
             a.persistent = 1; a.n_steps = win.update.count; a.n_red = win.reduce.count; a.n_str = n;
-            a.slot_upd = win.update.first % kLinSlots; a.slot_red = win.reduce.first % kLinSlots; a.slot_str = s0 % kLinSlots;
+            a.G = p.G; a.n_img = p.n_img; a.nslots = nslots;
+            a.slot_upd = win.update.first % nslots; a.slot_red = win.reduce.first % nslots; a.slot_str = s0 % nslots;
             a.d_red = win.reduce.first - win.update.first; a.d_str = s0 - win.update.first;
             a.sets = kLinReduceSets;
             a.has_update = 1; a.n_reduce = p.n_reduce; a.n_stream = p.n_stream;
diff --git a/vae_training_amd/csrc/vaek_internal.h b/vae_training_amd/csrc/vaek_internal.h
--- a/vae_training_amd/csrc/vaek_internal.h
+++ b/vae_training_amd/csrc/vaek_internal.h
@@ -93,6 +93,7 @@
     bool ok = false;
     int NB = 0, NO = 0;
     int T = 0, ntiles = 0;
+    int G = 1, n_img = 0, F = 1;
     bool persist = false;
     int n_stream = 0, n_reduce = 0;
     size_t lds_persist = 0, lds_step = 0;
diff --git a/vae_training_amd/engine.py b/vae_training_amd/engine.py
--- a/vae_training_amd/engine.py
+++ b/vae_training_amd/engine.py
@@ -262,6 +262,11 @@
             check(fn(*args, _stream()))
         return run
 
+    def train_steps_plan(self):
+        plan = (C.c_int32 * 5)()
+        _lib.check(self.lib.vaek_train_steps_plan(self.h, plan))
+        return dict(zip(("T", "tiles", "G", "images", "in_flight"), (int(x) for x in plan)))
+
     def moment_len(self):
         return self._moment_len
 
```

Measured after the change: 18.56 billion samples/s. No clear change (-0.4%).
